# emolch/kiwi

Measured on AMD Instinct MI355X. Metric: trial-source misfit evals/s, higher is better.
Workload: dtype f32

## Files before the change

### kiwi_amd/csrc/kiwi_accum.hip

```cpp
#include "kiwi_accum_api.hpp"

#if KIWI_ARITH == 0
#define KIWI_ARITH_NS exact
#elif KIWI_ARITH == 1
#define KIWI_ARITH_NS fused
#else
#error "KIWI_ARITH: 0 (exact) or 1 (fused)"
#endif

namespace kiwi {
namespace KIWI_ARITH_NS {

#include "kiwi_accum.inc"

#define KIWI_COMMON_ARGS a.G, a.span, a.pitch, a.recs, a.cent_ofs, a.isrc0, a.nrec, a.recv, a.syn, a.syn_stride

#if KIWI_FAMILY == 1
void launch_direct(const AccumArgs &a, dim3 grid)
{
    if (a.ng == 10) hipLaunchKernelGGL(accumulate_kernel<10>, grid, dim3(256), 0, a.stream, KIWI_COMMON_ARGS, a.synrow);
    else            hipLaunchKernelGGL(accumulate_kernel<8>, grid, dim3(256), 0, a.stream, KIWI_COMMON_ARGS, a.synrow);
}
#endif

#if KIWI_FAMILY == 2
template <int NG, int T, bool COMPACT>
static void grouped_tc(const AccumArgs &a, dim3 grid, int ntiles, const int *runs, int pairsel, const int *mate, const int *mate4)
{
#define KIWI_G(FV, RV) hipLaunchKernelGGL((accumulate_grouped_kernel<NG, T, FV, RV, COMPACT>), grid, dim3(T), 0, a.stream, KIWI_COMMON_ARGS, ntiles, \
                                          a.tab, a.coefs, runs, a.fp, a.pairflag, pairsel, mate, mate4, a.synrow, a.fam_ofs, a.fam_list)
    if (a.fuse) { if (runs) KIWI_G(true, true); else KIWI_G(true, false); }
    else        { if (runs) KIWI_G(false, true); else KIWI_G(false, false); }
#undef KIWI_G
}
template <int NG, int T>
static void grouped_t(const AccumArgs &a, dim3 grid, int ntiles, const int *runs, int pairsel, const int *mate, const int *mate4)
{
    if (a.compact) grouped_tc<NG, T, true>(a, grid, ntiles, runs, pairsel, mate, mate4);
    else           grouped_tc<NG, T, false>(a, grid, ntiles, runs, pairsel, mate, mate4);
}
void launch_grouped(const AccumArgs &a, dim3 grid, int T, int ntiles, const int *runs, int pairsel, const int *mate, const int *mate4)
{
    if (a.ng == 10) {
        if (T == 64) grouped_t<10, 64>(a, grid, ntiles, runs, pairsel, mate, mate4);
        else if (T == 128) grouped_t<10, 128>(a, grid, ntiles, runs, pairsel, mate, mate4);
        else grouped_t<10, 256>(a, grid, ntiles, runs, pairsel, mate, mate4);
    } else {
        if (T == 64) grouped_t<8, 64>(a, grid, ntiles, runs, pairsel, mate, mate4);
        else if (T == 128) grouped_t<8, 128>(a, grid, ntiles, runs, pairsel, mate, mate4);
        else grouped_t<8, 256>(a, grid, ntiles, runs, pairsel, mate, mate4);
    }
}
#endif

#if KIWI_FAMILY == 3
template <int NG, int NS, bool COMPACT>
static void multi_t(const AccumArgs &a, dim3 grid, int ntiles, const int *mate, const int *wider)
{
    if (a.fuse) hipLaunchKernelGGL((accumulate_multi_kernel<NG, true, NS, COMPACT>), grid, dim3(256), 0, a.stream, KIWI_COMMON_ARGS, ntiles, a.tab, a.coefs, a.fp,
                                   a.pairflag, mate, wider);
    else        hipLaunchKernelGGL((accumulate_multi_kernel<NG, false, NS, COMPACT>), grid, dim3(256), 0, a.stream, KIWI_COMMON_ARGS, ntiles, a.tab, a.coefs, a.fp,
                                   a.pairflag, mate, wider);
}
template <int NG, int NS>
static void multi_c(const AccumArgs &a, dim3 grid, int ntiles, const int *mate, const int *wider)
{
    if (a.compact) multi_t<NG, NS, true>(a, grid, ntiles, mate, wider); else multi_t<NG, NS, false>(a, grid, ntiles, mate, wider);
}
void launch_multi(const AccumArgs &a, dim3 grid, int NS, int ntiles, const int *mate, const int *wider)
{
    if (a.ng == 10) { if (NS == 4) multi_c<10, 4>(a, grid, ntiles, mate, wider); else multi_c<10, 2>(a, grid, ntiles, mate, wider); }
    else            { if (NS == 4) multi_c<8, 4>(a, grid, ntiles, mate, wider); else multi_c<8, 2>(a, grid, ntiles, mate, wider); }
}
#endif

#if KIWI_FAMILY == 4
template <int NG, bool COMPACT>
static void cell_t(const AccumArgs &a, dim3 grid, int ntiles, bool per_wave)
{
#define KIWI_C(KERNEL) hipLaunchKernelGGL(KERNEL, grid, dim3(256), 0, a.stream, KIWI_COMMON_ARGS, ntiles, a.tab, a.coefs, a.fp, a.pairflag, a.synrow, \
                                          a.fam_ofs, a.fam_list)
    if (per_wave) { if (a.fuse) KIWI_C((accumulate_cellw_kernel<NG, true, COMPACT>)); else KIWI_C((accumulate_cellw_kernel<NG, false, COMPACT>)); }
    else          { if (a.fuse) KIWI_C((accumulate_cell_kernel<NG, 256, 2, 0, true, COMPACT>)); else KIWI_C((accumulate_cell_kernel<NG, 256, 2, 0, false, COMPACT>)); }
#undef KIWI_C
}
template <int NG>
static void cell_c(const AccumArgs &a, dim3 grid, int ntiles, bool per_wave)
{
    if (a.compact) cell_t<NG, true>(a, grid, ntiles, per_wave); else cell_t<NG, false>(a, grid, ntiles, per_wave);
}
void launch_cell(const AccumArgs &a, dim3 grid, int ntiles) { if (a.ng == 10) cell_c<10>(a, grid, ntiles, false); else cell_c<8>(a, grid, ntiles, false); }
void launch_cellw(const AccumArgs &a, dim3 grid, int ntiles) { if (a.ng == 10) cell_c<10>(a, grid, ntiles, true); else cell_c<8>(a, grid, ntiles, true); }
int cellw_range() { return kCellwRange; }
#endif

}
}
```

### kiwi_amd/csrc/kiwi_accum.inc

```


typedef float f4u __attribute__((ext_vector_type(4), aligned(4)));
typedef float f2u __attribute__((ext_vector_type(2), aligned(4)));

#if defined(KIWI_EXPLICIT_FMA)
#ifndef KIWI_CELLW_AHEAD
#define KIWI_CELLW_AHEAD 3
#endif
template <class V> __device__ __forceinline__ V kiwi_mad(V acc, float w, V v)
{
    V ws;
    for (int k = 0; k < (int)(sizeof(V) / sizeof(float)); k++) ws[k] = w;
    return __builtin_elementwise_fma(ws, v, acc);
}
template <class V> __device__ __forceinline__ V kiwi_madv(V acc, V w, V v) { return __builtin_elementwise_fma(w, v, acc); }
#else
template <class V> __device__ __forceinline__ V kiwi_mad(V acc, float w, V v) { return acc + w * v; }
template <class V> __device__ __forceinline__ V kiwi_madv(V acc, V w, V v) { return acc + w * v; }
#endif

typedef int v4i_t __attribute__((ext_vector_type(4)));
typedef int v2i_t __attribute__((ext_vector_type(2)));
__device__ __forceinline__ __amdgpu_buffer_rsrc_t gf_rsrc(const float *base)
{
// ... 195 lines not shown
    int q = kRowPad + l;
    q = min(max(q, 0), pitch - 4);
    return *(const f4u *)(rowp + q);
}


template <bool BLEND, bool FAST, int N>
__device__ __forceinline__ void build_batch(float *__restrict__ tile0, int lds_tile, const int (&igs)[N], int p, int jb,
                                            const float *__restrict__ G, int pitch, int ta, int tb, const GeoRec &g)
{
    const int j = jb + p;
    f4u v[N][BLEND ? 4 : 1];
#pragma unroll
    for (int q = 0; q < N; q++) {
#pragma unroll
        for (int k = 0; k < (BLEND ? 4 : 1); k++) {
            const int base = REC_I(ta, 4 * igs[q] + k);
            if constexpr (FAST) {
                v[q][k] = buf_load4(gf_rsrc(G), p, base + jb);
            } else {
                const int lo = REC_I(tb, 4 * igs[q] + k);
                const int idx = min(max(base + j, lo), lo + pitch - 4);
                v[q][k] = *(const f4u *)(G + (size_t)(unsigned)idx);
            }
        }
    }
#pragma unroll
    for (int q = 0; q < N; q++) {
        f4u b;
        if constexpr (BLEND) {
            b = g.w[0] * v[q][0];
            b = b + g.w[1] * v[q][1];
            b = b + g.w[2] * v[q][2];
            b = b + g.w[3] * v[q][3];
        } else {
            b = v[q][0];
        }
        *(float4 *)(tile0 + igs[q] * lds_tile + p) = make_float4(b.x, b.y, b.z, b.w);
    }
}

template <bool BLEND, bool FAST>
__device__ __forceinline__ void pair_issue(f4u (&v)[2][BLEND ? 4 : 1], int ig0, int p, int jb, const float *__restrict__ G,
                                           int pitch, int ta, int tb)
{
    const int j = jb + p;
#pragma unroll
    for (int q = 0; q < 2; q++) {
#pragma unroll
        for (int k = 0; k < (BLEND ? 4 : 1); k++) {
            const int base = REC_I(ta, 4 * (ig0 + q) + k);
            if constexpr (FAST) {
                v[q][k] = buf_load4(gf_rsrc(G), p, base + jb);
            } else {
                const int lo = REC_I(tb, 4 * (ig0 + q) + k);
                const int idx = min(max(base + j, lo), lo + pitch - 4);
                v[q][k] = *(const f4u *)(G + (size_t)(unsigned)idx);
            }
        }
    }
}

template <bool BLEND>
__device__ __forceinline__ void pair_finish(const f4u (&v)[2][BLEND ? 4 : 1], float *__restrict__ tile0, int lds_tile, int ig0, int p,
                                            const GeoRec &g)
{
#pragma unroll
    for (int q = 0; q < 2; q++) {
        f4u b;
        if constexpr (BLEND) {
            b = g.w[0] * v[q][0];
            b = b + g.w[1] * v[q][1];
            b = b + g.w[2] * v[q][2];
            b = b + g.w[3] * v[q][3];
        } else {
            b = v[q][0];
        }
        *(float4 *)(tile0 + (ig0 + q) * lds_tile + p) = make_float4(b.x, b.y, b.z, b.w);
    }
}

struct HaloRegs { f4u v[4]; };

template <bool BLEND, bool FAST>
__device__ __forceinline__ HaloRegs halo_issue(bool active, int ig, int ph, int jb, const float *__restrict__ G, int pitch,
                                               int ta, int tb)
{
    HaloRegs h;
#pragma unroll
    for (int k = 0; k < (BLEND ? 4 : 1); k++) {
        const int base = __shfl(ta, 4 * ig + k, 64);
        int idx = base + jb + ph;
        if constexpr (!FAST) {
            const int lo = __shfl(tb, 4 * ig + k, 64);
            idx = min(max(idx, lo), lo + pitch - 4);
        }
        h.v[k] = f4u{ 0.f, 0.f, 0.f, 0.f };
        if (active) h.v[k] = *(const f4u *)(G + (size_t)(unsigned)idx);
    }
    return h;
}

template <bool BLEND>
__device__ __forceinline__ void halo_finish(bool active, const HaloRegs &h, float *__restrict__ tile0, int lds_tile, int ig, int ph,
                                            const GeoRec &g)
{
    f4u b;
    if constexpr (BLEND) {
        b = g.w[0] * h.v[0];
        b = kiwi_mad(b, g.w[1], h.v[1]);
        b = kiwi_mad(b, g.w[2], h.v[2]);
        b = kiwi_mad(b, g.w[3], h.v[3]);
    } else {
        b = h.v[0];
    }
    if (active) *(float4 *)(tile0 + ig * lds_tile + ph) = make_float4(b.x, b.y, b.z, b.w);
}

struct HaloRegs2 { f2u v[4]; };

template <bool FAST>
__device__ __forceinline__ HaloRegs2 halo_issue2(bool active, int ig, int ph, int jb, const float *__restrict__ G, int pitch, int ta, int tb)
{
    HaloRegs2 h;
#pragma unroll
    for (int k = 0; k < 4; k++) {
        const int base = __shfl(ta, 4 * ig + k, 64);
        int idx = base + jb + ph;
        if constexpr (!FAST) {
            const int lo = __shfl(tb, 4 * ig + k, 64);
            idx = min(max(idx, lo), lo + pitch - 2);
        }
        h.v[k] = f2u{ 0.f, 0.f };
        if (active) h.v[k] = *(const f2u *)(G + (size_t)(unsigned)idx);
    }
    return h;
}

__device__ __forceinline__ void halo_finish2(bool active, const HaloRegs2 &h, float *__restrict__ tile0, int lds_tile, int ig, int ph,
                                             float w0, float w1, float w2, float w3)
{
    f2u b = w0 * h.v[0];
    b = kiwi_mad(b, w1, h.v[1]);
    b = kiwi_mad(b, w2, h.v[2]);
    b = kiwi_mad(b, w3, h.v[3]);
    if (active) *(float2 *)(tile0 + ig * lds_tile + ph) = make_float2(b.x, b.y);
}

typedef float f2v __attribute__((ext_vector_type(2)));
typedef const __attribute__((address_space(3))) float *lds_cfp;

template <int NP = 2> struct TileRegsN { f2v lo[NP], hi[NP]; };
typedef TileRegsN<2> TileRegs;

struct TileBase { const __attribute__((address_space(3))) float *lo, *hi; };

__device__ __forceinline__ TileBase tile_base(const float *__restrict__ p)
{
    typedef const __attribute__((address_space(3))) float *lds_fp;
    TileBase b;
    b.lo = (lds_fp)p;
    unsigned a = (unsigned)(size_t)(b.lo + 1);
    asm volatile("" : "+v"(a));
    b.hi = (lds_fp)(size_t)a;
    return b;
}

template <int NP = 2>
__device__ __forceinline__ TileRegsN<NP> tile_load(const TileBase &b, int ofs)
{
    TileRegsN<NP> t;
#pragma unroll
    for (int h = 0; h < NP; h++) {
        t.lo[h] = f2v{ b.lo[ofs + 128 * h], b.lo[ofs + 128 * h + 64] };
        t.hi[h] = f2v{ b.hi[ofs + 128 * h], b.hi[ofs + 128 * h + 64] };
    }
    return t;
}

template <bool TAIL, int NP = 2>
__device__ __forceinline__ void tile_fma(f2v (&out)[NP], const TileRegsN<NP> &t, int jl, int jend, float factor, float wl, float wr)
{
#pragma unroll
// ... 657 lines not shown
            } else {
            int eprev = 0;
            bool have = false;
#define KIWI_C2STEP(LL, HH, RV, CC) do { \
                const int e = smax - __builtin_amdgcn_readlane(ishv, (CC) - c);       \
                const int d = have ? eprev - e : 0x7fff; \
                 \
                const int dh = same ? (d == 0 ? 1 : 0x7fff) : d, dl = same ? (d == 0 ? -1 : 0x7fff) : d; \
                same = false; \
                carry2_apply<NG, RV>(ar1, ar2, dz, LL, HH, abase + 4u * (unsigned)e, dh, dl, coef_grp + (size_t)((CC) - c) * kCoefLine, gcl, gsl); \
                have = true; eprev = e; } while (0)
#define KIWI_C2SOURCES(RV) do { \
                set2_dead(X); set2_dead(Y);        \
                for (int js = s; js < s_end; js++) { \
                    if (multi) { \
                        ar1[0] = ar1[1] = ar2[0] = ar2[1] = dz[0] = dz[1] = f2v{ 0.f, 0.f }; \
                        if (synrow && synrow[js] != js) continue;        \
                    } \
                    const size_t crow = ((size_t)(cent_ofs[isrc0 + js] - cb) * nrec + (size_t)r * nc + c) * kCoefLine; \
                    const unsigned clo = __builtin_amdgcn_readfirstlane((unsigned)crow), chi = __builtin_amdgcn_readfirstlane((unsigned)(crow >> 32)); \
                    const float *__restrict__ coef_grp = coefs + (((size_t)chi << 32) | clo); \
                    int cc = c; \
                     \
                    bool same = RUNS && multi && have && ((cend - c) & 1); \
                    for (; cc + 1 < cend; cc += 2) { KIWI_C2STEP(X, Y, RV, cc); KIWI_C2STEP(Y, X, RV, cc + 1); } \
                    if (cc < cend) KIWI_C2STEP(X, Y, RV, cc); \
                    if (multi) store_family(js); \
                } } while (0)
            if (g0.flags & 2) KIWI_C2SOURCES(true); else KIWI_C2SOURCES(false);
#undef KIWI_C2SOURCES
#undef KIWI_C2STEP
            cur = cur_next;
            }
        } else
        for (int js = s; js < s_end; js++) {
        const GeoRec *__restrict__ rcj = multi ? recs + ((size_t)(cent_ofs[isrc0 + js] - cb) * nrec + (size_t)r * nc) : rc;
        int cur_next_src = 0;
        if (multi) {
            if (js + 1 < s_end) {
                int lane_o = lane;
                if constexpr (RUNS && FUSE) asm volatile("" : "+v"(lane_o));
                cur_next_src = rec_load(recs + ((size_t)(cent_ofs[isrc0 + js + 1] - cb) * nrec + (size_t)r * nc), c, nc, lane_o);
            }
            ar1[0] = ar1[1] = ar2[0] = ar2[1] = dz[0] = dz[1] = f2v{ 0.f, 0.f };
            if (synrow && synrow[js] != js) { cur = cur_next_src; continue; }
        }
        const size_t crow = ((size_t)(cent_ofs[isrc0 + js] - cb) * nrec + (size_t)r * nc + c) * kCoefLine;
        const unsigned clo = __builtin_amdgcn_readfirstlane((unsigned)crow), chi = __builtin_amdgcn_readfirstlane((unsigned)(crow >> 32));
        const float *__restrict__ coef_grp = coefs + (((size_t)chi << 32) | clo);
        for (int cc = c; cc < cend; cc++) {
            const int nxt = rec_load(rcj, cc + 1, nc, lane);
            constexpr int ro = 0;
            const int ishift = REC_I(cur, ro + 8);
            const float cl = REC_F(cur, ro + 16), sl = REC_F(cur, ro + 17);
            const int flags = REC_I(cur, ro + 18);
            const float *__restrict__ coef = coef_grp + (size_t)(cc - c) * kCoefLine;
            const int e = smax - ishift;
            const int u0 = 4 * (tid & ~63) + lane;
            const TileBase chunk0 = tile_base(&tiles[0][e + u0]);
            const int jl = jb + e + u0;
            const bool tail = (jb + e + TILE) > jend_min;
#define APPLY(TV) do { \
                if (need_h && has_d && !(flags & 8)) centroid_apply_hd<NG, LDS_TILE, TV, !(FUSE && RUNS)>(ar1, ar2, dz, chunk0, jl, jend, flags, coef, cur, sd, cl, sl); \
                else centroid_apply<NG, LDS_TILE, TV>(ar1, ar2, dz, chunk0, jl, jend, need_h, has_d, flags, \
                                                      REC_F(cur, 9), sd, REC_F(cur, 10), REC_F(cur, 11), REC_F(cur, 12), REC_F(cur, 13), \
                                                      REC_F(cur, 14), REC_F(cur, 15), cl, sl); } while (0)
            if (!tail) APPLY(false); else APPLY(true);
#undef APPLY
            cur = nxt;
        }
        if (multi) { store_family(js); cur = cur_next_src; }
        }
        stored = multi;
        c = cend;
    }
    if (!multi) store_family(s);
    else if (!stored) {
        ar1[0] = ar1[1] = ar2[0] = ar2[1] = dz[0] = dz[1] = f2v{ 0.f, 0.f };
        for (int js = s; js < s_end; js++)
            if (!(synrow && synrow[js] != js)) store_family(js);
    }
}

template <bool BLEND, bool FAST>
__device__ __forceinline__ void one_issue(f4u (&v)[BLEND ? 4 : 1], int ig, int p, int jb, const float *__restrict__ G,
                                          int pitch, int ta, int tb)
{
    const int j = jb + p;
#pragma unroll
    for (int k = 0; k < (BLEND ? 4 : 1); k++) {
        const int base = REC_I(ta, 4 * ig + k);
        if constexpr (FAST) {
            v[k] = buf_load4(gf_rsrc(G), p, base + jb);
        } else {
            const int lo = REC_I(tb, 4 * ig + k);
            const int idx = min(max(base + j, lo), lo + pitch - 4);
            v[k] = *(const f4u *)(G + (size_t)(unsigned)idx);
        }
    }
}

__device__ __forceinline__ void one_issue_hidden(f4u (&v)[4], int ig, int p, int jb, const float *__restrict__ G, int ta)
{
    const size_t gi = (size_t)G;
    const v4i_t rs = { (int)(unsigned)gi, (int)((unsigned)(gi >> 32) & 0xffffu), -1, 0x00020000 };
    const int voff = (int)(4u * (unsigned)p);
#pragma unroll
    for (int k = 0; k < 4; k++) {
        const int soff = (int)(4u * (unsigned)(REC_I(ta, 4 * ig + k) + jb));
        asm volatile("buffer_load_dwordx4 %0, %1, %2, %3 offen" : "=v"(v[k]) : "v"(voff), "s"(rs), "s"(soff));
    }
}
template <int CNT_FULL, int CNT_SHORT>
__device__ __forceinline__ void vm_wait(f4u (&v)[4], int full )
{
    if constexpr (CNT_FULL == CNT_SHORT)
        asm volatile("s_waitcnt vmcnt(%4)" : "+v"(v[0]), "+v"(v[1]), "+v"(v[2]), "+v"(v[3]) : "n"(CNT_FULL));
    else
        asm volatile("s_cmp_eq_u32 %6, 0\n\ts_cbranch_scc1 1f\n\ts_waitcnt vmcnt(%4)\n\ts_branch 2f\n1:\n\ts_waitcnt vmcnt(%5)\n2:"
                     : "+v"(v[0]), "+v"(v[1]), "+v"(v[2]), "+v"(v[3]) : "n"(CNT_FULL), "n"(CNT_SHORT), "s"(full) : "scc");
}

template <bool BLEND>
__device__ __forceinline__ void one_finish(const f4u (&v)[BLEND ? 4 : 1], float *__restrict__ tile0, int lds_tile, int ig, int p,
                                           const GeoRec &g)
{
    f4u b;
    if constexpr (BLEND) {
        b = g.w[0] * v[0];
        b = b + g.w[1] * v[1];
        b = b + g.w[2] * v[2];
        b = b + g.w[3] * v[3];
    } else {
        b = v[0];
    }
    *(float4 *)(tile0 + ig * lds_tile + p) = make_float4(b.x, b.y, b.z, b.w);
}

#ifndef KIWI_MFMA_BLEND
#define KIWI_MFMA_BLEND 0
#endif
typedef float f4m __attribute__((ext_vector_type(4)));
struct RowsDw { float r[4][4]; };

__device__ __forceinline__ void rows_issue_dw(RowsDw &v, int ig, int lane, int jb, const float *__restrict__ G, int ta)
{
    const size_t gi = (size_t)G;
    const v4i_t rs = { (int)(unsigned)gi, (int)((unsigned)(gi >> 32) & 0xffffu), -1, 0x00020000 };
    const int voff = (int)(4u * (unsigned)lane);
#pragma unroll
    for (int k = 0; k < 4; k++) {
        const int soff = (int)(4u * (unsigned)(REC_I(ta, 4 * ig + k) + jb));
        asm volatile("buffer_load_dword %0, %1, %2, %3 offen" : "=v"(v.r[k][0]) : "v"(voff), "s"(rs), "s"(soff));
        asm volatile("buffer_load_dword %0, %1, %2, %3 offen offset:256" : "=v"(v.r[k][1]) : "v"(voff), "s"(rs), "s"(soff));
        asm volatile("buffer_load_dword %0, %1, %2, %3 offen offset:512" : "=v"(v.r[k][2]) : "v"(voff), "s"(rs), "s"(soff));
        asm volatile("buffer_load_dword %0, %1, %2, %3 offen offset:768" : "=v"(v.r[k][3]) : "v"(voff), "s"(rs), "s"(soff));
    }
}
template <int CNT_FULL, int CNT_SHORT>
__device__ __forceinline__ void vm_wait16(RowsDw &v, int full )
{
#define KIWI_R16 "+v"(v.r[0][0]), "+v"(v.r[0][1]), "+v"(v.r[0][2]), "+v"(v.r[0][3]), "+v"(v.r[1][0]), "+v"(v.r[1][1]), "+v"(v.r[1][2]), "+v"(v.r[1][3]), \
                 "+v"(v.r[2][0]), "+v"(v.r[2][1]), "+v"(v.r[2][2]), "+v"(v.r[2][3]), "+v"(v.r[3][0]), "+v"(v.r[3][1]), "+v"(v.r[3][2]), "+v"(v.r[3][3])
    if constexpr (CNT_FULL == CNT_SHORT)
        asm volatile("s_waitcnt vmcnt(%16)" : KIWI_R16 : "n"(CNT_FULL));
    else
        asm volatile("s_cmp_eq_u32 %18, 0\n\ts_cbranch_scc1 1f\n\ts_waitcnt vmcnt(%16)\n\ts_branch 2f\n1:\n\ts_waitcnt vmcnt(%17)\n2:"
                     : KIWI_R16 : "n"(CNT_FULL), "n"(CNT_SHORT), "s"(full) : "scc");
#undef KIWI_R16
}
__device__ __forceinline__ void mfma_finish(const RowsDw &v, float *__restrict__ dst, const float (&w)[4], bool write)
{
    const f4m negz = { -0.f, -0.f, -0.f, -0.f };
#pragma unroll
    for (int m = 0; m < 4; m++) {
        f4m b = __builtin_amdgcn_mfma_f32_4x4x1f32(v.r[0][m], w[0], negz, 0, 0, 0);
        b = b + __builtin_amdgcn_mfma_f32_4x4x1f32(v.r[1][m], w[1], negz, 0, 0, 0);
        b = b + __builtin_amdgcn_mfma_f32_4x4x1f32(v.r[2][m], w[2], negz, 0, 0, 0);
        b = b + __builtin_amdgcn_mfma_f32_4x4x1f32(v.r[3][m], w[3], negz, 0, 0, 0);
        if (write) *(float4 *)(dst + 64 * m) = make_float4(b.x, b.y, b.z, b.w);
    }
}

template <int NG, int NS> __host__ __device__ constexpr int multi_set_stride() { return NG * (1024 / NS + kHalo) + ((NS == 4 && KIWI_MFMA_BLEND) ? 8 : 0); }

template <int NG, bool FAST, int NS, typename Shadow>
__device__ __forceinline__ void multi_build(float *__restrict__ tile0, int wv, int lane, int tid, int jb, const float *__restrict__ G,
                                            int pitch, int ta, int tb, const GeoRec (&gw)[NS], int only, bool hact, bool whalo, int hig, int hph,
                                            Shadow shadow)
{
    constexpr int TILE = 1024 / NS, LDS_TILE = TILE + kHalo, DEPTH = 3, SET = multi_set_stride<NG, NS>();
    constexpr int N = (NS == 2) ? NG / 2 : (NG + 3) / 4;
    const int p = (NS == 2) ? 4 * (64 * (wv & 1) + lane) : 4 * lane;
    auto comp = [&](int i) { return (NS == 2) ? 2 * i + (wv >> 1) : wv + 4 * i; };
    HaloRegs hv;
    if (whalo) hv = halo_issue<true, FAST>(true, hig, hph, jb, G, pitch, ta, tb);
    const bool last_ok = comp(N - 1) < NG;
    if constexpr (KIWI_MFMA_BLEND && FAST && NS == 4 && KIWI_ARITH == 0) {
        RowsDw v[N];
#pragma unroll
        for (int i = 0; i < DEPTH && i < N; i++) if (i < N - 1 || last_ok) rows_issue_dw(v[i], comp(i), lane, jb, G, ta);
        __syncthreads();
        shadow();
        const int me = lane & 3;
        float w[4];
#pragma unroll
        for (int k = 0; k < 4; k++) w[k] = me == 0 ? gw[0].w[k] : (me == 1 ? gw[1].w[k] : (me == 2 ? gw[2].w[k] : gw[3].w[k]));
        float *__restrict__ dst = tile0 + me * SET + 4 * (lane >> 2);
        const bool write = only < 0 || only == me;
#pragma unroll
        for (int i = 0; i < N; i++) {
            __builtin_amdgcn_sched_barrier(0);
            if (i < N - 1 || last_ok) {
                const int behind = (i + DEPTH < N ? i + DEPTH : N) - 1 - i;
                const bool short_ = behind > 0 && i + DEPTH >= N;
                const int lastf = __builtin_amdgcn_readfirstlane(last_ok ? 1 : 0);
                switch (behind) {
                case 0: vm_wait16<0, 0>(v[i], 1); break;
                case 1: if (short_) vm_wait16<16, 0>(v[i], lastf); else vm_wait16<16, 16>(v[i], 1); break;
                default: if (short_) vm_wait16<32, 16>(v[i], lastf); else vm_wait16<32, 32>(v[i], 1); break;
                }
                mfma_finish(v[i], dst + comp(i) * LDS_TILE, w, write);
            }
            if (i + DEPTH < N && (i + DEPTH < N - 1 || last_ok)) rows_issue_dw(v[i + DEPTH], comp(i + DEPTH), lane, jb, G, ta);
        }
        if (whalo) {
#pragma unroll
            for (int s = 0; s < NS; s++)
                if (only < 0 || only == s) halo_finish<true>(hact, hv, tile0 + s * SET, LDS_TILE, hig, hph, gw[s]);
        }
        return;
    }
    f4u v[N][4];
    auto issue = [&](int i) __attribute__((always_inline)) {
        if constexpr (FAST) one_issue_hidden(v[i], comp(i), p, jb, G, ta);
        else one_issue<true, false>(v[i], comp(i), p, jb, G, pitch, ta, tb);
    };
#pragma unroll
    for (int i = 0; i < DEPTH && i < N; i++) if (i < N - 1 || last_ok) issue(i);
    __syncthreads();
    shadow();
#pragma unroll
    for (int i = 0; i < N; i++) {
        __builtin_amdgcn_sched_barrier(0);
        if (i < N - 1 || last_ok) {
            if constexpr (FAST) {
                const int behind = (i + DEPTH < N ? i + DEPTH : N) - 1 - i;
                const bool short_ = behind > 0 && i + DEPTH >= N;
                const int lastf = __builtin_amdgcn_readfirstlane(last_ok ? 1 : 0);
                switch (behind) {
                case 0: vm_wait<0, 0>(v[i], 1); break;
                case 1: if (short_) vm_wait<4, 0>(v[i], lastf); else vm_wait<4, 4>(v[i], 1); break;
                default: if (short_) vm_wait<8, 4>(v[i], lastf); else vm_wait<8, 8>(v[i], 1); break;
                }
            }
#pragma unroll
            for (int s = 0; s < NS; s++)
                if (only < 0 || only == s) one_finish<true>(v[i], tile0 + s * SET, LDS_TILE, comp(i), p, gw[s]);
        }
        if (i + DEPTH < N && (i + DEPTH < N - 1 || last_ok)) issue(i + DEPTH);
    }
    if (whalo) {
#pragma unroll
        for (int s = 0; s < NS; s++)
            if (only < 0 || only == s) halo_finish<true>(hact, hv, tile0 + s * SET, LDS_TILE, hig, hph, gw[s]);
    }
}


__device__ __forceinline__ int smax_u(int a, int b) { int r; asm("s_max_i32 %0, %1, %2" : "=s"(r) : "s"(a), "s"(b) : "scc"); return r; }
__device__ __forceinline__ int smin_u(int a, int b) { int r; asm("s_min_i32 %0, %1, %2" : "=s"(r) : "s"(a), "s"(b) : "scc"); return r; }

template <int NS>
__device__ __forceinline__ bool multi_taken(const RecvDev &rv, const int *__restrict__ pairflag, const int *__restrict__ mate,
                                            int s, int nrec, int r)
{
    if (!mate) return false;
    const int a = s - s % NS;
    if (!mate[a / NS] || !rv.need_h || !rv.has_d) return false;
    int f = 0;
#pragma unroll
    for (int i = 0; i < NS; i++) f |= pairflag[(size_t)(a + i) * nrec + r];
    return f == 0;
}

template <int NG, bool FUSE, int NS, bool COMPACT >
__global__ __launch_bounds__(256) __attribute__((amdgpu_waves_per_eu(3))) void accumulate_multi_kernel(
    const float *__restrict__ G, const int2 *__restrict__ span, int pitch,
    const GeoRec *__restrict__ recs, const int *__restrict__ cent_ofs, int isrc0, int nrec,
    const RecvDev *__restrict__ recv, float *__restrict__ syn, size_t syn_stride, int ntiles,
    const int *__restrict__ tab, const float *__restrict__ coefs, FuseParams fp, const int *__restrict__ pairflag, const int *__restrict__ mate,
    const int *__restrict__ mate_wider )
{
    constexpr bool compact = COMPACT;
    static_assert(NS == 2 || NS == 4, "sources per workgroup");
    constexpr int TILE = 1024 / NS, LDS_TILE = TILE + kHalo, K = LDS_TILE / 64, WPS = 4 / NS;
    constexpr int SET = multi_set_stride<NG, NS>();
    __shared__ __attribute__((aligned(16))) float tiles[NS * SET];
    const int s0 = NS * (int)blockIdx.x;
    const int tile = blockIdx.y % ntiles, r = blockIdx.y / ntiles;
    const RecvDev &rv = recv[r];
    if (!rv.enabled) return;
    if (tile * TILE >= rv.wlen) return;
    if (!multi_taken<NS>(rv, pairflag, mate, s0, nrec, r)) return;
    if constexpr (NS == 2) { if (multi_taken<4>(rv, pairflag, mate_wider, s0, nrec, r)) return; }
    const int tid = threadIdx.x;
    const int lane = tid & 63;
    const int wv = __builtin_amdgcn_readfirstlane(tid >> 6);
    const int sh = wv / WPS;
    const int t_tile0 = rv.wbeg + tile * TILE;
    const int cb = cent_ofs[isrc0];
    const int nc = cent_ofs[isrc0 + s0 + 1] - cent_ofs[isrc0 + s0];
    const size_t base_me = (size_t)(cent_ofs[isrc0 + s0 + sh] - cb) * nrec + (size_t)r * nc;
    const GeoRec *__restrict__ rc = recs + base_me;
    const float sd = rv.sd;
    (void)sd;
    const int u0 = 256 * (wv % WPS) + lane;

    f2v ar1[2] = { { 0.f, 0.f }, { 0.f, 0.f } }, ar2[2] = { { 0.f, 0.f }, { 0.f, 0.f } }, dz[2] = { { 0.f, 0.f }, { 0.f, 0.f } };
    f2v xa0, xa1, xa2, xa3, xa4, xa5, xa6, xa7, xa8, xa9, xb0, xb1, xb2, xb3, xb4, xb5, xb6, xb7, xb8, xb9;
    f2v ya0, ya1, ya2, ya3, ya4, ya5, ya6, ya7, ya8, ya9, yb0, yb1, yb2, yb3, yb4, yb5, yb6, yb7, yb8, yb9;
    typedef typename Set2Sel<NG>::type SetT;
    const SetT X = make_set2<NG>(xa0, xa1, xa2, xa3, xa4, xa5, xa6, xa7, xa8, xa9, xb0, xb1, xb2, xb3, xb4, xb5, xb6, xb7, xb8, xb9);
    const SetT Y = make_set2<NG>(ya0, ya1, ya2, ya3, ya4, ya5, ya6, ya7, ya8, ya9, yb0, yb1, yb2, yb3, yb4, yb5, yb6, yb7, yb8, yb9);

    long long rbase[NS];
#pragma unroll
    for (int i = 0; i < NS; i++) {
        const long long b = (long long)(cent_ofs[isrc0 + s0 + i] - cb) * nrec + (long long)r * nc;
        rbase[i] = ((long long)__builtin_amdgcn_readfirstlane((int)(b >> 32)) << 32) | (unsigned)__builtin_amdgcn_readfirstlane((int)b);
    }
    auto recs_of = [&](int i) { return recs + (size_t)rbase[i]; };
    auto tab_of = [&](int i) { return tab + (size_t)rbase[i] * (compact ? 4 : 128); };
    int c = 0;
    int cur[NS];
#pragma unroll
    for (int i = 0; i < NS; i++) cur[i] = rec_load(recs_of(i), 0, nc, lane);
    int ta = 0, tb = 0;
    if constexpr (compact) ta = off4_load(tab_of(0), 0, lane);
    else { ta = tab_of(0)[lane]; tb = tab_of(0)[64 + lane]; }
    const int hq = 255 - tid, hch = min(hq / NG, 15), hig = hq % NG, hph = TILE + 4 * hch;
    while (c < nc) {
        GeoRec g[NS];
        int smaxs[NS], smins[NS], npos = 0;
        bool shared = true, same_rows = true;
        if constexpr (compact) desc_expand(ta, cur[0], lane, pitch, ta, tb);
#pragma unroll
        for (int i = 0; i < NS; i++) {
            g[i].ishift = REC_I(cur[i], 8);
            g[i].pad = REC_I(cur[i], 19);
            smaxs[i] = g[i].ishift + ((g[i].pad >> 8) & 0xff);
            smins[i] = g[i].ishift - ((g[i].pad >> 16) & 0xff);
            npos = max(npos, TILE + (smaxs[i] - smins[i]) + 8);
            if (i == 0) g[0].row[0] = REC_I(cur[0], 0);
            else {
                same_rows = same_rows && (__builtin_amdgcn_ballot_w64(cur[i] != cur[0]) & 0xfull) == 0ull;
                shared = shared && smaxs[i] == smaxs[0];
            }
        }
        shared = shared && same_rows;
        if (same_rows && !shared) {
            int smax_c = smaxs[0], smin_c = smins[0];
#pragma unroll
            for (int i = 1; i < NS; i++) { smax_c = smax_u(smax_c, smaxs[i]); smin_c = smin_u(smin_c, smins[i]); }
            if (TILE + (smax_c - smin_c) + 8 <= LDS_TILE) {
                shared = true;
                npos = TILE + (smax_c - smin_c) + 8;
#pragma unroll
                for (int i = 0; i < NS; i++) smaxs[i] = smax_c;
            }
        }
        const int glen = g[0].pad & 0xff;
        const int cend = c + glen;
        int smax = smaxs[0];
#pragma unroll
        for (int i = 1; i < NS; i++) if (sh == i) smax = smaxs[i];
        int flags = 0, ishv = 0, warm_ = 0;
        float gcl = 0.f, gsl = 0.f;
        const float *__restrict__ coef_grp = nullptr;
        auto shadow = [&]() {
#pragma unroll
            for (int i = 0; i < NS; i++) { g[i].w[0] = REC_F(cur[i], 4); g[i].w[1] = REC_F(cur[i], 5); g[i].w[2] = REC_F(cur[i], 6); g[i].w[3] = REC_F(cur[i], 7); }
            int curme = cur[0];
#pragma unroll
            for (int i = 1; i < NS; i++) if (sh == i) curme = cur[i];
            flags = REC_I(curme, 18);
            gcl = REC_F(curme, 16); gsl = REC_F(curme, 17);
            if (lane < glen) ishv = rc[c + lane].ishift;
            const size_t crow = (base_me + c) * kCoefLine;
            const unsigned clo = __builtin_amdgcn_readfirstlane((unsigned)crow), chi = __builtin_amdgcn_readfirstlane((unsigned)(crow >> 32));
            coef_grp = coefs + (((size_t)chi << 32) | clo);
            if constexpr (NG == 10) warm_ = coef_warm(coef_grp);
        };
        auto noshadow = []() {};
#define KIWI_MULTI_BUILD(TA, TB, I0, ONLY, NPOS, SHADOW) do { \
            const int jb_ = t_tile0 - smaxs[I0] - 1;       \
            const float *__restrict__ Gg = G + (size_t)g[I0].row[0] * (size_t)pitch; \
            const bool lane_ok = lane >= 4 * NG || ((TA) + jb_ >= (TB) && (TA) + jb_ + LDS_TILE <= (TB) + pitch); \
            const bool fast = __builtin_amdgcn_ballot_w64(lane_ok) == ~0ull; \
            const bool hact = hq < 16 * NG && hph < (NPOS); \
            const bool whalo = __builtin_amdgcn_ballot_w64(hact) != 0ull; \
            if (fast) multi_build<NG, true, NS>(&tiles[0], wv, lane, tid, jb_, Gg, pitch, TA, TB, g, ONLY, hact, whalo, hig, hph, SHADOW); \
            else      multi_build<NG, false, NS>(&tiles[0], wv, lane, tid, jb_, Gg, pitch, TA, TB, g, ONLY, hact, whalo, hig, hph, SHADOW); } while (0)
        __builtin_amdgcn_s_setprio(1);
        if (shared) KIWI_MULTI_BUILD(ta, tb, 0, -1, npos, shadow);
        else {
            KIWI_MULTI_BUILD(ta, tb, 0, 0, npos, shadow);
#pragma unroll
            for (int i = 1; i < NS; i++) {
                int tai, tbi;
                if constexpr (compact) desc_expand(off4_load(tab_of(i), c, lane), cur[i], lane, pitch, tai, tbi);
                else { tai = tab_of(i)[(size_t)c * 128 + lane]; tbi = tab_of(i)[(size_t)c * 128 + 64 + lane]; }
                g[i].row[0] = REC_I(cur[i], 0);
                KIWI_MULTI_BUILD(tai, tbi, i, i, npos, noshadow);
            }
        }
#undef KIWI_MULTI_BUILD
#pragma unroll
        for (int i = 0; i < NS; i++) cur[i] = rec_load(recs_of(i), cend, nc, lane);
        if (cend < nc) {
            if constexpr (compact) ta = off4_load(tab_of(0), cend, lane);
            else { ta = tab_of(0)[(size_t)cend * 128 + lane]; tb = tab_of(0)[(size_t)cend * 128 + 64 + lane]; }
        }
        __syncthreads();
        __builtin_amdgcn_s_setprio(0);
        {
            const unsigned abase = (unsigned)(size_t)(lds_cfp)&tiles[sh * SET + u0];
            if constexpr (NG == 10 || NG == 8) {
                asm volatile("" :: "s"(warm_));
                const float gcl_u = __int_as_float(__builtin_amdgcn_readfirstlane(__float_as_int(gcl))), gsl_u = __int_as_float(__builtin_amdgcn_readfirstlane(__float_as_int(gsl)));
                const size_t cg_ = (size_t)coef_grp;
                const float *__restrict__ coef_u = (const float *)(((size_t)(unsigned)__builtin_amdgcn_readfirstlane((int)(cg_ >> 32)) << 32) | (unsigned)__builtin_amdgcn_readfirstlane((int)cg_));
                const int n = cend - c;
#define KIWI_ASM_ARGS ar1[0], ar1[1], ar2[0], ar2[1], dz[0], dz[1], abase, ishv, smax, n, coef_u, gcl_u, gsl_u
                if constexpr (NG == 10) {
                    if (flags & 2) { if constexpr (K == 5) KIWI_APPLY_ASM(10, 5, rot)(KIWI_ASM_ARGS); else KIWI_APPLY_ASM(10, 9, rot)(KIWI_ASM_ARGS); }
                    else           { if constexpr (K == 5) KIWI_APPLY_ASM(10, 5, plain)(KIWI_ASM_ARGS); else KIWI_APPLY_ASM(10, 9, plain)(KIWI_ASM_ARGS); }
                } else {
                    if (flags & 2) { if constexpr (K == 5) KIWI_APPLY_ASM(8, 5, rot)(KIWI_ASM_ARGS); else KIWI_APPLY_ASM(8, 9, rot)(KIWI_ASM_ARGS); }
                    else           { if constexpr (K == 5) KIWI_APPLY_ASM(8, 5, plain)(KIWI_ASM_ARGS); else KIWI_APPLY_ASM(8, 9, plain)(KIWI_ASM_ARGS); }
                }
#undef KIWI_ASM_ARGS
            } else {
            int cc = c, eprev = 0;
            bool have = false;
#define KIWI_C2STEP(LL, HH, RV, CC) do { \
                const int e = smax - __builtin_amdgcn_readlane(ishv, (CC) - c);        \
                const int d = have ? eprev - e : 0x7fff; \
                carry2_apply<NG, RV, K>(ar1, ar2, dz, LL, HH, abase + 4u * (unsigned)e, d, d, coef_grp + (size_t)((CC) - c) * kCoefLine, gcl, gsl); \
                have = true; eprev = e; } while (0)
            if (flags & 2) {
                set2_dead(X); set2_dead(Y);
                for (; cc + 1 < cend; cc += 2) { KIWI_C2STEP(X, Y, true, cc); KIWI_C2STEP(Y, X, true, cc + 1); }
                if (cc < cend) KIWI_C2STEP(X, Y, true, cc);
            } else {
                set2_dead(X); set2_dead(Y);
                for (; cc + 1 < cend; cc += 2) { KIWI_C2STEP(X, Y, false, cc); KIWI_C2STEP(Y, X, false, cc + 1); }
                if (cc < cend) KIWI_C2STEP(X, Y, false, cc);
            }
#undef KIWI_C2STEP
            }
        }
        c = cend;
    }
    {
        const int js = s0 + sh;
        const int tl = tile * TILE + u0;
        if (!FUSE && tl >= rv.wlen) return;
        float *__restrict__ so = syn + (size_t)js * syn_stride + tl;
        float mom = 0.f;
        if constexpr (FUSE) mom = fp.moment[fp.isrc0 + js];
        const bool whole = tile * TILE + TILE <= rv.wlen;
        for (int k = 0; k < rv.ncomp; k++) {
            f2v o01, o23;
            out4(rv.comp[k], rv.sign[k], rv.cl0, rv.sl0, ar1, ar2, dz, o01, o23);
            if constexpr (!FUSE) {
                const float o[4] = { o01.x, o01.y, o23.x, o23.y };
#pragma unroll
                for (int i = 0; i < 4; i++)
                    if (tl + 64 * i < rv.wlen) so[rv.synofs[k] + 64 * i] = o[i];
                continue;
            }
            double acc = fused_acc4(fp, o01, o23, mom, fp.reft + rv.refofs[k] + tl, fp.tw + rv.refofs[k] + tl, tl, rv.wlen, whole);
            acc = wave_reduce_f64(acc, fp.method == 6);
            if (lane == 63)
                fp.partial[((size_t)js * fp.nmis + rv.slot0 + k) * fp.nparts + tile * WPS + (wv % WPS)] = acc;
        }
    }
}

template <int SPL> struct RawVec;
template <> struct RawVec<4> { typedef f4u type; };
template <> struct RawVec<2> { typedef f2u type; };

template <int NG, int PART> struct CellPart;
template <> struct CellPart<10, 0> { static constexpr int n = 10; static constexpr int first = 0; __device__ static constexpr int ig(int i) { return i < 3 ? i : (i == 3 ? 8 : (i < 9 ? i - 1 : 9)); } };
template <> struct CellPart<8, 0>  { static constexpr int n = 8; static constexpr int first = 0; __device__ static constexpr int ig(int i) { return i; } };
template <> struct CellPart<10, 1> { static constexpr int n = 6; static constexpr int first = 0; __device__ static constexpr int ig(int i) { return i < 3 ? i : (i == 3 ? 8 : i - 1); } };
template <> struct CellPart<10, 2> { static constexpr int n = 4; static constexpr int first = 6; __device__ static constexpr int ig(int i) { return i < 3 ? 5 + i : 9; } };
template <> struct CellPart<8, 1>  { static constexpr int n = 5; static constexpr int first = 0; __device__ static constexpr int ig(int i) { return i; } };
template <> struct CellPart<8, 2>  { static constexpr int n = 3; static constexpr int first = 5; __device__ static constexpr int ig(int i) { return 5 + i; } };

template <int NG, int PART, int SPL> using RawArr = typename RawVec<SPL>::type[CellPart<NG, PART>::n][4];

template <int NG, int PART, int SPL, bool FAST = false, bool UNI = false>
__device__ __forceinline__ void raw_issue(RawArr<NG, PART, SPL> &v, int p, int jb,
// ... 554 lines not shown
```

### kiwi_amd/csrc/kiwi_accum_api.hpp

```cpp
#pragma once
#include "kiwi_common.hpp"

namespace kiwi {

struct AccumArgs {
    hipStream_t stream;
    int ng;
    bool fuse;
    const float *G; const int2 *span; int pitch;
    const GeoRec *recs; const int *cent_ofs; int isrc0, nrec;
    const RecvDev *recv; float *syn; size_t syn_stride;
    const int *tab; const float *coefs; FuseParams fp;
    const int *pairflag, *synrow, *fam_ofs, *fam_list;
    int compact;
};

#define KIWI_ACCUM_LAUNCHERS                                                                                                      \
                                                                 \
    void launch_direct(const AccumArgs &a, dim3 grid);                                                                            \
                  \
    void launch_grouped(const AccumArgs &a, dim3 grid, int T, int ntiles, const int *runs, int pairsel, const int *mate,          \
                        const int *mate4);                                                                                        \
                                                     \
    void launch_multi(const AccumArgs &a, dim3 grid, int NS, int ntiles, const int *mate, const int *mate_wider);                \
        \
    void launch_cell(const AccumArgs &a, dim3 grid, int ntiles);                                                                  \
    void launch_cellw(const AccumArgs &a, dim3 grid, int ntiles);                                                                 \
                               \
    int cellw_range();

namespace exact { KIWI_ACCUM_LAUNCHERS }
namespace fused { KIWI_ACCUM_LAUNCHERS }
#undef KIWI_ACCUM_LAUNCHERS

}
```

### kiwi_amd/csrc/kiwi_bands.hpp

```cpp

namespace bands {

constexpr int kMaxBands = 16;
constexpr int kLg = 16;
constexpr int kMaxDynLds = 152 * 1024;

static inline bool is_spectral(int method) { return method == KIWI_AMPSPEC_L2NORM || method == KIWI_AMPSPEC_L1NORM; }

struct BandTab {
    int ntd, nfilt, nspec, nband;
    int td[kMaxBands], filt[kMaxBands], spec[kMaxBands];
    int method[kMaxBands], has_filter[kMaxBands];
};

struct BandArgs {
    SynRows sr;
    const float *reft;
    const int *ntr;
    FusedFftTables tabs;
    const BandTab *bt;
    const int2 *vtab;
    const float *normtab;
    const float *refamp, *filtw, *reffilt, *zmask;
    int nband, nmis, isrc0, dyn_bytes;
// ... 365 lines not shown
        else
            HIPCHECK(hipMemcpyAsync(st.reffilt_h.data() + f.pr.filtofs, st.reffilt_d.p + f.pr.filtofs, (size_t)cd.wlen * sizeof(float),
                                    hipMemcpyDeviceToHost, c->stream));
    }
    HIPCHECK(hipStreamSynchronize(c->stream));
    for (auto &f : fresh) {
        const CompDev &cd = c->comps[(size_t)f.pr.slot];
        const int method = c->bands[(size_t)f.b].method;
        double sum = 0.0, pk = 0.0;
        float nf;
        if (is_spectral(method)) {
            const int nb = f.pr.ntrans / 2 + 1;
            const float df = 1.f / ((float)f.pr.ntrans * dt);
            for (int k = 0; k < nb; k++) {
                const float v = st.refamp_h[(size_t)f.pr.specofs + k];
                sum += (method == KIWI_AMPSPEC_L2NORM) ? (double)v * (double)v : (double)std::fabs(v);
            }
            nf = (method == KIWI_AMPSPEC_L2NORM) ? 1.f * (float)std::sqrt((double)df * sum) : 1.f * (float)((double)df * sum);
        } else {
            for (int i = 0; i < cd.wlen; i++) {
                const float v = st.reffilt_h[(size_t)f.pr.filtofs + i];
                switch (method) {
                case KIWI_L2NORM: sum += (double)v * (double)v; break;
                case KIWI_L1NORM: sum += (double)std::fabs(v); break;
                case KIWI_SCALAR_PRODUCT: sum += (double)(v * v); break;
                default: pk = std::max(pk, (double)std::fabs(v)); break;
                }
            }
            switch (method) {
            case KIWI_L2NORM: nf = 1.f * (float)std::sqrt((double)dt * sum); break;
            case KIWI_L1NORM: nf = 1.f * (float)((double)dt * sum); break;
            case KIWI_SCALAR_PRODUCT: nf = (1.f * 1.f) * (float)sum; break;
            default: nf = 1.f * (float)pk; break;
            }
        }
        st.normtab_h[((size_t)f.b * nmis + f.pr.slot) * kLg + lg_of(f.pr.ntrans)] = nf;
    }
    HIPCHECK(hipMemcpyAsync(st.refamp_d.p, st.refamp_h.data(), st.refamp_h.size() * sizeof(float), hipMemcpyHostToDevice, c->stream));
    HIPCHECK(hipMemcpyAsync(st.reffilt_d.p, st.reffilt_h.data(), st.reffilt_h.size() * sizeof(float), hipMemcpyHostToDevice, c->stream));
    HIPCHECK(hipMemcpyAsync(st.vtab_d.p, st.vtab_h.data(), st.vtab_h.size() * sizeof(int2), hipMemcpyHostToDevice, c->stream));
    HIPCHECK(hipMemcpyAsync(st.normtab_d.p, st.normtab_h.data(), st.normtab_h.size() * sizeof(float), hipMemcpyHostToDevice, c->stream));
    HIPCHECK(hipStreamSynchronize(c->stream));
}

static void run(kiwi_hip_ctx *c, int isrc0, int nsrc, const Out &out)
{
    check_setup(c);
    if (isrc0 < 0 || nsrc < 0 || (long long)isrc0 + nsrc > (long long)c->nsrc)
        throw std::runtime_error("band_misfits: sources " + std::to_string(isrc0) + " .. " + std::to_string((long long)isrc0 + nsrc) +
                                 " are not inside the uploaded batch of " + std::to_string(c->nsrc));
    if (nsrc == 0) return;
    BandState &st = c->band_state;
    if (!st.valid || st.prepare_gen != c->prepare_gen) reset_cache(c);
    const int nrec = (int)c->recv.size(), nband = (int)c->bands.size(), nmis = c->nmis;
    if (st.need_spec && !c->fused_fft)
        throw std::runtime_error("band_misfits: bands with a frequency filter or an amplitude-spectrum method go through the in-LDS transforms, "
                                 "which KIWI_HIP_FUSED_FFT=0 switches off");
    int wlen_pow2 = 1 << kFusedFftMinLog2;
    while (wlen_pow2 < c->max_wlen) wlen_pow2 <<= 1;
    if (wlen_pow2 > (1 << kFusedFftMaxLog2))
        throw std::runtime_error("band_misfits: a misfit window of " + std::to_string(c->max_wlen) + " samples does not fit the in-LDS row of " +
                                 std::to_string(1 << kFusedFftMaxLog2) + " samples");
    c->misfit_d.ensure((size_t)c->nsrc * c->nmis, &c->dev_bytes);
    c->global_d.ensure((size_t)c->nsrc, &c->dev_bytes);
    if (c->fft_needed && !c->fft_ready) prepare_fft(c, c->reft_h);
    c->fuse_now = false;
    struct Restore { kiwi_hip_ctx *c; bool want; ~Restore() { c->want_spansrc = want; } } restore{ c, c->want_spansrc };
    c->want_spansrc = true;
    if (!st.attr) {
        HIPCHECK(hipFuncSetAttribute(reinterpret_cast<const void *>(&band_kernel), hipFuncAttributeMaxDynamicSharedMemorySize, kMaxDynLds));
        st.attr = true;
    }

    hipEvent_t ev[4];
    for (int i = 0; i < 4; i++) ev[i] = c->get_event();
    struct Return { kiwi_hip_ctx *c; hipEvent_t *ev; ~Return() { for (int i = 0; i < 4; i++) c->event_pool.push_back(ev[i]); } } ret{ c, ev };
    std::vector<int> ntr_h;
    int s = isrc0;
    while (s < isrc0 + nsrc) {
        size_t bytes = 0;
        int n = 0;
        while (s + n < isrc0 + nsrc) {
            const size_t nc = (size_t)(c->cent_ofs[s + n + 1] - c->cent_ofs[s + n]);
            const size_t add = nc * nrec * (sizeof(GeoRec) + (c->accum_mode == 0 ? 512 + kCoefLine * sizeof(float) : 0)) + c->syn_stride * sizeof(float) +
                               (size_t)nband * nmis * 2 * sizeof(float);
            if (n > 0 && (bytes + add > c->chunk_bytes_limit || n >= 65535)) break;
            if (c->fft_needed && n >= c->fft_cap) break;
            bytes += add; n++;
        }
        HIPCHECK(hipEventRecord(ev[0], c->stream));
        run_chunk(c, s, n, 0);
        HIPCHECK(hipEventRecord(ev[1], c->stream));
        const size_t np = (size_t)n * nmis;
        int longest = wlen_pow2;
        if (st.need_spec) {
            st.ntr_d.ensure(np, &c->dev_bytes);
            hipLaunchKernelGGL(fft_size_kernel, dim3((unsigned)((np + 255) / 256)), dim3(256), 0, c->stream, c->spansrc_d.p, c->comps_d.p, nmis, n, nrec,
                               c->risetime_d.p + s, c->gm.dt, st.ntr_d.p, (const int *)nullptr);
            ntr_h.resize(np);
            HIPCHECK(hipMemcpyAsync(ntr_h.data(), st.ntr_d.p, np * sizeof(int), hipMemcpyDeviceToHost, c->stream));
            HIPCHECK(hipStreamSynchronize(c->stream));
            std::vector<std::pair<int, int>> want;
            std::vector<int> seen((size_t)nmis, 0);
            longest = 0;
            for (size_t i = 0; i < np; i++) {
                const int m = (int)(i % (size_t)nmis), nt = ntr_h[i];
                if (nt < (1 << kFusedFftMinLog2) || nt > (1 << kFusedFftMaxLog2))
                    throw std::runtime_error("band_misfits: source " + std::to_string(s + (int)(i / (size_t)nmis) + 1) + ", misfit slot " + std::to_string(m + 1) +
                                             " needs a transform of " + std::to_string(nt) + " samples; the in-LDS transforms take " +
                                             std::to_string(1 << kFusedFftMinLog2) + " to " + std::to_string(1 << kFusedFftMaxLog2));
                longest = std::max(longest, nt);
                if (seen[(size_t)m] != nt) { seen[(size_t)m] = nt; want.emplace_back(m, nt); }
            }
            std::sort(want.begin(), want.end());
            want.erase(std::unique(want.begin(), want.end()), want.end());
            make_variants(c, want);
        }
        const size_t nout = (size_t)n * nband * nmis;
        st.mis_d.ensure(nout, &c->dev_bytes); st.norm_d.ensure(nout, &c->dev_bytes); st.glob_d.ensure((size_t)n * nband, &c->dev_bytes);
        const int dyn = st.nfilt >= 2 ? std::max(4 * longest, std::min(8 * longest, kMaxDynLds)) : 4 * longest;
        BandArgs a;
        a.sr = SynRows{ c->syn_d.p, c->syn_stride, c->comps_d.p, c->tw_d.p, c->moment_d.p, c->risetime_d.p, nullptr };
        a.reft = c->reft_d.p;
        a.ntr = st.need_spec ? st.ntr_d.p : nullptr;
        a.tabs = fused_fft_tables(c);
        a.bt = reinterpret_cast<const BandTab *>(st.bt_d.p);
        a.vtab = st.vtab_d.p; a.normtab = st.normtab_d.p;
        a.refamp = st.refamp_d.p; a.filtw = st.filtw_d.p; a.reffilt = st.reffilt_d.p; a.zmask = st.zmask_d.p;
        a.nband = nband; a.nmis = nmis; a.isrc0 = s; a.dyn_bytes = dyn;
        a.dt = c->gm.dt; a.syn_factor = c->syn_factor;
        a.mis_out = st.mis_d.p; a.norm_out = st.norm_d.p;
        hipLaunchKernelGGL(band_kernel, dim3((unsigned)n, (unsigned)nmis), dim3(256), (size_t)dyn, c->stream, a);
        hipLaunchKernelGGL(band_global_kernel, dim3((unsigned)(((size_t)n * nband + 127) / 128)), dim3(128), 0, c->stream, st.mis_d.p, st.norm_d.p,
                           c->recfirst_d.p, c->nrec_en, nmis, nband, s, n, st.glob_d.p, c->any_failed ? c->status_d.p : (const int *)nullptr);
        HIPCHECK(hipGetLastError());
        HIPCHECK(hipEventRecord(ev[2], c->stream));
        const Out o = out.at((size_t)(s - isrc0), (size_t)nband, (size_t)nmis);
        if (o.misfit) HIPCHECK(hipMemcpyAsync(o.misfit, st.mis_d.p, nout * sizeof(float), hipMemcpyDeviceToHost, c->stream));
        if (o.norm) HIPCHECK(hipMemcpyAsync(o.norm, st.norm_d.p, nout * sizeof(float), hipMemcpyDeviceToHost, c->stream));
        if (o.global) HIPCHECK(hipMemcpyAsync(o.global, st.glob_d.p, (size_t)n * nband * sizeof(float), hipMemcpyDeviceToHost, c->stream));
        HIPCHECK(hipEventRecord(ev[3], c->stream));
        HIPCHECK(hipStreamSynchronize(c->stream));
        for (int i = 0; i < 3; i++) {
            float t = 0.f;
            HIPCHECK(hipEventElapsedTime(&t, ev[i], ev[i + 1]));
            c->bands_ms[i] += t;
        }
        s += n;
    }
    c->last_isrc0 = isrc0; c->last_nsrc = nsrc; c->last_proc_which = 0;
    c->evaluated.resize((size_t)c->nsrc, 0);
    std::fill(c->evaluated.begin() + isrc0, c->evaluated.begin() + isrc0 + nsrc, 1);
}

}
```

### kiwi_amd/csrc/kiwi_common.hpp

```cpp
#pragma once
#include <hip/hip_runtime.h>
#include <type_traits>

namespace kiwi {

constexpr int kRowPad = 32;
constexpr int kTile = 1024;
constexpr int kMaxComp = 5;
constexpr int kHalo = 64;
constexpr int kMaxGroup = 64;

struct GeoRec {
    int   row[4];
    float w[4];
    int   ishift;
    float wfrac;
    float f[6];
    float cl, sl;
    int   flags;
    int   pad;
};
static_assert(sizeof(GeoRec) == 80, "GeoRec layout");

struct GfMeta {
    int nx, nz, ng;
    int pitch;
    float dt, dx, dz, firstx, firstz;
};

struct RecvDev {
    double azi0, bazi0, dist0;
    float depth;
    float cl0, sl0;
    int   enabled;
    int   ncomp;
    int   comp[kMaxComp];
    float sign[kMaxComp];
    int   need_h, has_d;
    float sd;
    int   wbeg, wlen;
    int   synofs[kMaxComp];
    int   slot0;
    int   refofs[kMaxComp];
};

struct FuseParams {
    const float *reft, *tw, *moment;
    double *partial;
    int method;
    float syn_factor;
    int nmis, nparts, isrc0;
};

struct CompDev {
    int synofs;
    int halo;
    int w0, wlen;
    int refofs;
    int rec;
    int has_filter;
    int ntrans_max;
    int fl_lo, fl_ns, refxofs;
    int untapered, rf0, rf1, vertical;
    int spankind;
};

struct FftPair {
    long long fft_ofs;
    long long spec_ofs;
    int ntrans;
    int specofs;
    int filtofs;
    int slot;
};
static_assert(sizeof(FftPair) == 32, "FftPair layout");

struct ShakeRec {
    int slot[3];
    int np;
    int untapered;
    int rec;
};

constexpr int kCoefLine = 20;
template <int NG> __host__ __device__ constexpr int coef_wl(int a) { return 2 * a; }
template <int NG> __host__ __device__ constexpr int coef_wr(int a) { return 2 * a + 1; }

constexpr int kSpanInts = 8;
__device__ __forceinline__ void strip_span(const int *__restrict__ sp, int kind, int &lo, int &hi)
{
    if (kind == 3) { lo = sp[4]; hi = sp[5]; return; }
    if (kind == 0) { lo = sp[0]; hi = sp[1]; return; }
    if (kind == 1) { lo = sp[2]; hi = sp[3]; return; }
    lo = min(sp[0], sp[2]); hi = max(sp[1], sp[3]);
}

struct EvalParams {
    int bilinear, xus, zus;
    int nrec;
    int isrc0;
    int cellmode;
    int nogaps;
};

__device__ __forceinline__ bool cell_pair(const RecvDev &rv, const int *__restrict__ pairflag, int s, int nrec, int r)
{
    return rv.need_h && rv.has_d && !(pairflag[(size_t)s * nrec + r] & 3);
}

template <int NS>
__device__ __forceinline__ bool multi_taken_fwd(const RecvDev &rv, const int *__restrict__ pairflag, const int *__restrict__ mate,
                                                int s, int nrec, int r)
{
    if (!mate) return false;
    const int a = s - s % NS;
    if (!mate[a / NS] || !rv.need_h || !rv.has_d) return false;
    int f = 0;
#pragma unroll
    for (int i = 0; i < NS; i++) f |= pairflag[(size_t)(a + i) * nrec + r];
    return f == 0;
}

__device__ __forceinline__ double sq_acc(double acc, float d) { return fma((double)d, (double)d, acc); }

template <int CTRL, int ROW_MASK>
__device__ __forceinline__ double dpp_f64(double v)
{
    const int lo = __builtin_amdgcn_update_dpp(0, __double2loint(v), CTRL, ROW_MASK, 0xf, true);
    const int hi = __builtin_amdgcn_update_dpp(0, __double2hiint(v), CTRL, ROW_MASK, 0xf, true);
    return __hiloint2double(hi, lo);
}

template <bool IS_MAX>
__device__ __forceinline__ double wave_reduce_f64_t(double v)
{
#define KIWI_STEP(CTRL, MASK) do { const double o = dpp_f64<CTRL, MASK>(v); v = IS_MAX ? fmax(v, o) : v + o; } while (0)
    KIWI_STEP(0x111, 0xf);
    KIWI_STEP(0x112, 0xf);
    KIWI_STEP(0x114, 0xf);
    KIWI_STEP(0x118, 0xf);
    KIWI_STEP(0x142, 0xa);
    KIWI_STEP(0x143, 0xc);
#undef KIWI_STEP
    return v;
}
__device__ __forceinline__ double wave_reduce_f64(double v, bool is_max)
{
    return is_max ? wave_reduce_f64_t<true>(v) : wave_reduce_f64_t<false>(v);
}

}
```

### kiwi_amd/csrc/kiwi_hip.hip

```cpp
#include "../../include/kiwi_hip.h"
#include "kiwi_host.hpp"
#include "kiwi_host_eikonal.hpp"
#include "kiwi_host_lm.hpp"
#include "kiwi_geometry.hpp"
#include "kiwi_misfit.hpp"
#include "kiwi_accum_api.hpp"
#include "kiwi_fmm_device.hpp"

#include <hip/hip_runtime.h>
#include <hipfft/hipfft.h>
#include <algorithm>
#include <array>
#include <map>
#include <tuple>
#include <cstdio>
#include <cstdlib>
#include <cstring>
#include <string>
#include <vector>
#include <stdexcept>
#include <omp.h>
#include <chrono>
#include <condition_variable>
#include <deque>
// ... 82 lines not shown
};

struct BandDef { int method; Plf filter; };

struct BandState {
    bool valid = false, need_spec = false, attr = false;
    unsigned prepare_gen = 0;
    int nfilt = 0;
    std::vector<float> refamp_h, filtw_h, reffilt_h, normtab_h;
    std::vector<int2> vtab_h;
    DevBuf<CompDev> comps_d;
    DevBuf<float> zmask_d, rows_d, refamp_d, filtw_d, reffilt_d, normtab_d, mis_d, norm_d, glob_d;
    DevBuf<int2> vtab_d;
    DevBuf<int> bt_d, ntr_d;
    DevBuf<FftPair> prs_d;
};

struct TimeScanState {
    bool attr = false;
    DevBuf<float> mis_d, norm_d, glob_d;
    DevBuf<int> best_d;
};

}

struct kiwi_hip_ctx {
    int device = 0;
    hipStream_t stream = nullptr;
    std::string err;
    long long dev_bytes = 0;

    GfMeta gm{};
    bool have_db = false;
    DevBuf<float> G;
    DevBuf<int2> span;
    DevBuf<unsigned char> endz;
    int db_lmax = 0;

    int bilinear = 0, xus = 1, zus = 1;
    float effective_dt = 1.f;
    GeoCoords src_origin; bool have_origin = false; double ref_time = 0;
    std::vector<Receiver> recv;
    int method = KIWI_L2NORM;
    float syn_factor = 1.f;
    bool have_crust = false;
    CrustProfile rupture_profile{}, origin_profile{};
    float crustal_thickness_limit = 0.f;
    std::vector<HalfSpace> constraints;

    bool prepared = false;
    bool synth_only = false;
    bool any_untapered = false;
    DevBuf<int> spansrc_d;
    bool want_spansrc = false;
    int nmis = 0, nrec_en = 0;
    int halo = 0;
    size_t syn_stride = 0;
    std::vector<CompDev> comps;
    std::vector<RecvDev> recv_h;
    std::vector<float> norm_h;
    std::vector<float> reft_h;
    DevBuf<RecvDev> recv_d;
    DevBuf<CompDev> comps_d;
    DevBuf<float> reft_d, tw_d, norm_d;
    DevBuf<int> recfirst_d;
    int max_wlen = 0;

    int nsrc = 0;
    std::vector<int> cent_ofs;
    float max_risetime = 0.f;
    DevBuf<float> cent_d, moment_d, risetime_d;
    DevBuf<int> centofs_d;
    std::vector<int> src_status;
    bool any_failed = false;
    DevBuf<int> status_d;
    std::vector<int> same_as;
    bool any_same = false;
    DevBuf<int> synrow_d, famofs_d, famlist_d;
    int dedupe_enabled = 1;
    std::vector<unsigned long long> geo_hash;
    std::vector<kiwi_hip_ctx *> mates;
    int cpu_share = 1;
    std::vector<unsigned long long> struct_hash;
    std::vector<unsigned char> group_lens;
    std::vector<int> first_shift;
    std::vector<float> src_ends;
    DevBuf<int> mate_d, mate4_d;
    int duo = 4;
    std::vector<char> single_group;
    DevBuf<int> runfirst_d;
    int share_runs = 1, max_run = 64;
    int fuse_enabled = 1;
    bool fuse_now = false;
    DevBuf<double> fusepart_d;

    DevBuf<float> misfit_d, global_d;
    DevBuf<GeoRec> recs_d;
    DevBuf<int> tab_d;
    DevBuf<int> off4_d;
    DevBuf<float> coef_d;
    DevBuf<int> pairflag_d;
    DevBuf<float> syn_d, proc_d;
    bool floating = false;
    int max_ns = 1;
    DevBuf<float> refx_d, vt_d, partial_d;
    DevBuf<int> fshift_d;
    int last_isrc0 = 0, last_nsrc = 0, last_chunk0 = 0, last_chunkn = 0;
    std::vector<char> evaluated;
    int last_proc_which = 0;
    int group_threads_env = 0;
    int group_threads = 128;
    int accum_mode = 0;
    int cell_mode = -1;
    int cell_wave = 1;
    int arith = KIWI_ARITH_EXACT;
    double points_per_centroid = 0.0;
    int keep_which = 0;
    int proc_chunk0 = 0, proc_chunkn = 0, proc_which_held = 0;
    size_t chunk_bytes_limit = (size_t)16 << 30;
    float outer_ms[3] = { 0.f, 0.f, 0.f };
    float linfit_wide_ms[2] = { 0.f, 0.f };
    float linfit_ms[4] = { 0.f, 0.f, 0.f, 0.f };
    std::vector<BandDef> bands;
    BandState band_state;
    float bands_ms[3] = { 0.f, 0.f, 0.f };
    TimeScanState timescan_state;
    float timescan_ms[3] = { 0.f, 0.f, 0.f };
    float linfit_timescan_ms[4] = { 0.f, 0.f, 0.f, 0.f };
    unsigned linfit_timescan_attr = 0;
    unsigned prepare_gen = 0;
    int eik_solver = 0;
    mutable FmmDev fmm;

    bool fft_needed = false, fft_ready = false, any_filter = false;
    int fft_cap = 0;
    size_t fft_floats_per_src = 0, spec_cplx_per_src = 0;
    struct FftVariant { int ntrans, specofs, filtofs; float norm; };
    std::map<std::pair<int, int>, FftVariant> variants;
    std::vector<float> refamp_h, filtw_h, reffilt_h;
    std::vector<int> slot_has_filter;
    DevBuf<int> spanbuf_d, ntr_d;
    DevBuf<float> fft_d, refamp_d, filtw_d, reffilt_d, zmask_d, normsrc_d;
    DevBuf<int> lmax_d;
    bool db_gaps = false;
    bool db_simple = false;
    int compact = 1;
    DevBuf<int> synspan_d;
    DevBuf<float> refpair_d, reffiltpair_d;
    bool untapered_fft = false;
    DevBuf<float2> spec_d;
    DevBuf<FftPair> pairs_d;
    int *ntr_pin = nullptr; size_t ntr_pin_n = 0;
    int *mate_pin = nullptr; size_t mate_pin_n = 0;
    hipEvent_t mate_event = nullptr;
    FftPair *pairs_pin = nullptr; size_t pairs_pin_n = 0;
    std::vector<FftPair> last_pairs;
    std::vector<float> norm_src_h;
    struct FftBucket { int ntrans; long long count, fft_base, spec_base; };
    std::vector<FftBucket> buckets;
    hipEvent_t size_event = nullptr;
    std::map<std::tuple<int, int, int>, hipfftHandle> plans;
    DevBuf<float2> fused_tab[kFusedFftMaxLog2 + 1];
    bool fused_fft = true;
    bool fused_fft_attr = false;

    std::vector<EventPair> events;
    std::vector<hipEvent_t> event_pool;

    hipEvent_t get_event()
    {
// ... 575 lines not shown
                case KIWI_SCALAR_PRODUCT: sum += (double)(a * a); break;
                default: pk = std::max(pk, (double)std::fabs(a)); break;
                }
            }
            switch (c->method) {
            case KIWI_L2NORM: nf = 1.f * (float)std::sqrt((double)dt * sum); break;
            case KIWI_L1NORM: nf = 1.f * (float)((double)dt * sum); break;
            case KIWI_SCALAR_PRODUCT: nf = (1.f * 1.f) * (float)sum; break;
            default: nf = 1.f * (float)pk; break;
            }
        }
        c->variants[std::make_pair(pr.slot, pr.ntrans)] = kiwi_hip_ctx::FftVariant{ pr.ntrans, pr.specofs, pr.filtofs, nf };
    }
}

void layout_fft_chunk(kiwi_hip_ctx *c, int isrc0, int nsrc)
{
    HIPCHECK(hipEventSynchronize(c->size_event));
    const size_t np = (size_t)nsrc * c->nmis;
    const int *ntr = c->ntr_pin;
    std::map<int, long long> count;
    std::vector<std::pair<int, int>> want;
    {
        std::vector<int> seen((size_t)c->nmis, 0);
        for (size_t i = 0; i < np; i++) {
            const int m = (int)(i % c->nmis);
            count[ntr[i]]++;
            if (seen[m] != ntr[i]) { seen[m] = ntr[i]; want.emplace_back(m, ntr[i]); }
        }
        std::sort(want.begin(), want.end());
        want.erase(std::unique(want.begin(), want.end()), want.end());
    }
    make_variants(c, want);
    c->buckets.clear();
    std::map<int, size_t> bucket_of;
    long long fb = 0, sbase = 0;
    for (auto &kv : count) {
        bucket_of[kv.first] = c->buckets.size();
        c->buckets.push_back({ kv.first, 0, fb, sbase });
        fb += kv.second * kv.first;
        sbase += kv.second * (kv.first / 2 + 1);
    }
    c->fft_d.ensure((size_t)fb, &c->dev_bytes);
    c->spec_d.ensure((size_t)sbase, &c->dev_bytes);
    if (c->untapered_fft) {
        c->refpair_d.ensure((size_t)sbase, &c->dev_bytes);
        c->reffiltpair_d.ensure((size_t)fb, &c->dev_bytes);
    }
    pin_ensure(c->pairs_pin, c->pairs_pin_n, np);
    c->norm_src_h.resize((size_t)c->nsrc * c->nmis, 0.f);
    int last_ntr = -1; size_t last_b = 0;
    for (size_t i = 0; i < np; i++) {
        const int m = (int)(i % c->nmis);
        if (ntr[i] != last_ntr) { last_ntr = ntr[i]; last_b = bucket_of[last_ntr]; }
        auto &b = c->buckets[last_b];
        const auto &v = c->variants[std::make_pair(m, ntr[i])];
        FftPair &pr = c->pairs_pin[i];
        pr.fft_ofs = b.fft_base + b.count * b.ntrans;
        pr.spec_ofs = b.spec_base + b.count * (b.ntrans / 2 + 1);
        pr.ntrans = b.ntrans; pr.specofs = v.specofs; pr.filtofs = v.filtofs; pr.slot = m;
        b.count++;
        c->norm_src_h[(size_t)isrc0 * c->nmis + i] = v.norm;
    }
    c->pairs_d.ensure(np, &c->dev_bytes);
    HIPCHECK(hipMemcpyAsync(c->pairs_d.p, c->pairs_pin, np * sizeof(FftPair), hipMemcpyHostToDevice, c->stream));
    HIPCHECK(hipMemcpyAsync(c->normsrc_d.p + (size_t)isrc0 * c->nmis, c->norm_src_h.data() + (size_t)isrc0 * c->nmis, np * sizeof(float),
                            hipMemcpyHostToDevice, c->stream));
    c->last_pairs.assign(c->pairs_pin, c->pairs_pin + np);
}

bool can_fuse(const kiwi_hip_ctx *c, int proc_which, int isrc0, int nsrc)
{
    (void)isrc0; (void)nsrc;
    return c->fuse_enabled && c->accum_mode == 0 && proc_which == 0 && !c->fft_needed && !c->floating && !c->synth_only && !c->any_untapered &&
           c->halo == 0 && (c->method == KIWI_L2NORM || c->method == KIWI_L1NORM || c->method == KIWI_SCALAR_PRODUCT || c->method == KIWI_PEAK);
}

static int kiwi_quad_shift_span()
{
    static const int v = [] { const char *m = std::getenv("KIWI_HIP_QUAD_SPAN"); return m ? std::atoi(m) : 16; }();
    return v;
}

void run_chunk(kiwi_hip_ctx *c, int isrc0, int nsrc, int proc_which)
{
    const int nrec = (int)c->recv.size();
    const int cbeg = c->cent_ofs[isrc0], cend = c->cent_ofs[isrc0 + nsrc];
    int maxnc = 0;
    for (int s = isrc0; s < isrc0 + nsrc; s++) maxnc = std::max(maxnc, c->cent_ofs[s + 1] - c->cent_ofs[s]);
    c->recs_d.ensure((size_t)(cend - cbeg) * nrec, &c->dev_bytes);
    int *tab = nullptr;
    int *off4 = nullptr;
    if (c->accum_mode == 0) {
        c->tab_d.ensure((size_t)(cend - cbeg) * nrec * 128, &c->dev_bytes); tab = c->tab_d.p;
        if (c->db_simple && c->compact) {
            c->off4_d.ensure((size_t)(cend - cbeg) * nrec * 4, &c->dev_bytes); off4 = c->off4_d.p;
            if (std::getenv("KIWI_HIP_POISON")) HIPCHECK(hipMemsetAsync(off4, 0x7f, (size_t)(cend - cbeg) * nrec * 4 * sizeof(int), c->stream));
        }
        if (std::getenv("KIWI_HIP_POISON")) HIPCHECK(hipMemsetAsync(tab, 0x7f, (size_t)(cend - cbeg) * nrec * 128 * sizeof(int), c->stream));
        c->coef_d.ensure((size_t)(cend - cbeg) * nrec * kCoefLine + 160, &c->dev_bytes);
    }
    const int *synrow = nullptr, *famofs = nullptr, *famlist = nullptr;
    const bool heavy = c->dedupe_enabled == 2 || (size_t)(cend - cbeg) >= (size_t)8 * (size_t)nsrc;
    if (c->dedupe_enabled && heavy && c->any_same && !c->fft_needed && !c->floating && !c->any_untapered && !c->want_spansrc && !c->synth_only &&
        proc_which == 0) {
        std::vector<int> sr((size_t)nsrc);
        int ndup = 0;
        for (int s = 0; s < nsrc; s++) {
            const int f = c->same_as[(size_t)isrc0 + s];
            sr[s] = (f >= isrc0 && f != isrc0 + s) ? f - isrc0 : s;
            ndup += sr[s] != s;
        }
        const bool any = c->dedupe_enabled == 2 ? ndup > 0 : 2 * ndup >= nsrc;
        if (any) {
            c->synrow_d.ensure((size_t)nsrc, &c->dev_bytes);
            HIPCHECK(hipMemcpyAsync(c->synrow_d.p, sr.data(), (size_t)nsrc * sizeof(int), hipMemcpyHostToDevice, c->stream));
            synrow = c->synrow_d.p;
            if (c->fuse_now) {
                std::vector<int> ofs((size_t)nsrc + 1, 0), lst;
                for (int s = 0; s < nsrc; s++) if (sr[s] != s) ofs[(size_t)sr[s] + 1]++;
                for (int s = 0; s < nsrc; s++) ofs[(size_t)s + 1] += ofs[s];
                lst.resize((size_t)ofs[nsrc]);
                std::vector<int> fill(ofs.begin(), ofs.end() - 1);
                for (int s = 0; s < nsrc; s++) if (sr[s] != s) lst[(size_t)fill[sr[s]]++] = s;
                c->famofs_d.ensure(ofs.size(), &c->dev_bytes);
                c->famlist_d.ensure(std::max<size_t>(lst.size(), 1), &c->dev_bytes);
                HIPCHECK(hipMemcpyAsync(c->famofs_d.p, ofs.data(), ofs.size() * sizeof(int), hipMemcpyHostToDevice, c->stream));
                HIPCHECK(hipMemcpyAsync(c->famlist_d.p, lst.data(), lst.size() * sizeof(int), hipMemcpyHostToDevice, c->stream));
                HIPCHECK(hipStreamSynchronize(c->stream));
                famofs = c->famofs_d.p; famlist = c->famlist_d.p;
            }
            HIPCHECK(hipStreamSynchronize(c->stream));
        }
    }
    const bool fuse = c->fuse_now;
    if (!fuse) c->syn_d.ensure((size_t)nsrc * c->syn_stride, &c->dev_bytes);
    float *proc = nullptr;
    if (proc_which) { c->proc_d.ensure((size_t)nsrc * c->syn_stride, &c->dev_bytes); proc = c->proc_d.p; }

    const bool cell = c->accum_mode == 0 && (c->cell_mode == 1 || (c->cell_mode < 0 && c->bilinear && c->points_per_centroid > 0.5));
    const bool duo_maybe = c->accum_mode == 0 && c->duo && !cell && c->max_wlen >= 128 && !c->group_threads_env && nsrc >= 2;
    EvalParams ep{ c->bilinear, c->xus, c->zus, nrec, isrc0, cell ? 1 : 0, c->db_gaps ? 0 : 1 };
    int *spansrc = nullptr;
    if (c->any_untapered || c->want_spansrc || c->fft_needed) {
        const size_t n = (size_t)nsrc * nrec;
        c->spansrc_d.ensure(n * kSpanInts, &c->dev_bytes);
        hipLaunchKernelGGL(span_init_kernel, dim3((unsigned)((2 * n + 255) / 256)), dim3(256), 0, c->stream, c->spansrc_d.p, 2 * n);
        spansrc = c->spansrc_d.p;
    }
    hipEvent_t e0, e1, e2, e3;
    record(c, 0, e0);
    if (maxnc > 0) {
        dim3 grid((unsigned)((maxnc * nrec + 255) / 256), (unsigned)nsrc);
        if (cell || duo_maybe) {
            c->pairflag_d.ensure((size_t)nsrc * nrec, &c->dev_bytes);
            HIPCHECK(hipMemsetAsync(c->pairflag_d.p, 0, (size_t)nsrc * nrec * sizeof(int), c->stream));
        }
        int *lmax = nullptr;
        if (c->db_gaps && spansrc) {
            c->lmax_d.ensure((size_t)nsrc * nrec, &c->dev_bytes);
            HIPCHECK(hipMemsetAsync(c->lmax_d.p, 0xff, (size_t)nsrc * nrec * sizeof(int), c->stream));
            lmax = c->lmax_d.p;
            hipLaunchKernelGGL(geometry_kernel, grid, dim3(256), 0, c->stream, c->cent_d.p, c->centofs_d.p, ep, c->gm,
                               c->span.p, c->recv_d.p, (GeoRec *)nullptr, (int *)nullptr, (float *)nullptr, (int *)nullptr, (int *)nullptr, (int *)nullptr, c->endz.p, (const int *)nullptr,
                               lmax, (const int *)nullptr, (int4 *)nullptr);
        }
        hipLaunchKernelGGL(geometry_kernel, grid, dim3(256), 0, c->stream, c->cent_d.p, c->centofs_d.p, ep, c->gm,
                           c->span.p, c->recv_d.p, c->recs_d.p, tab, c->coef_d.p, (int *)nullptr, spansrc, (cell || duo_maybe) ? c->pairflag_d.p : (int *)nullptr, c->endz.p, (const int *)nullptr,
                           (int *)nullptr, (const int *)lmax, (int4 *)off4);
        if (cell)
            hipLaunchKernelGGL(cellgroup_kernel, grid, dim3(256), 0, c->stream, c->centofs_d.p, ep, c->gm, c->span.p, c->recv_d.p,
                               c->recs_d.p, tab, c->coef_d.p, c->pairflag_d.p, c->endz.p, (const int *)nullptr,
                               c->cell_wave ? exact::cellw_range() : kHalo - 10, off4 ? 1 : 0);
    }
    if (c->fft_needed && !c->untapered_fft) {
        const size_t np = (size_t)nsrc * c->nmis;
        c->ntr_d.ensure(np, &c->dev_bytes);
        pin_ensure(c->ntr_pin, c->ntr_pin_n, np);
        hipLaunchKernelGGL(fft_size_kernel, dim3((unsigned)((np + 255) / 256)), dim3(256), 0, c->stream, spansrc, c->comps_d.p, c->nmis,
                           nsrc, nrec, c->risetime_d.p + isrc0, c->gm.dt, c->ntr_d.p, (const int *)nullptr);
        HIPCHECK(hipMemcpyAsync(c->ntr_pin, c->ntr_d.p, np * sizeof(int), hipMemcpyDeviceToHost, c->stream));
        HIPCHECK(hipEventRecord(c->size_event, c->stream));
    }
    record(c, 0, e1);
    int fuse_T = 0, fuse_tile = 0, fuse_ntiles = 0, fuse_nparts = 0;
    bool fuse_all = false;
    {
        dim3 grid((unsigned)((c->max_wlen + kTile - 1) / kTile), (unsigned)nrec, (unsigned)nsrc);
        const bool fusedar = c->arith == KIWI_ARITH_FUSED;
        AccumArgs aa{ c->stream, c->gm.ng, c->fuse_now, c->G.p, c->span.p, c->gm.pitch, c->recs_d.p, c->centofs_d.p, isrc0, nrec, c->recv_d.p,
                      c->syn_d.p, c->syn_stride, off4 ? off4 : c->tab_d.p, c->coef_d.p, FuseParams{ nullptr, nullptr, nullptr, nullptr, 0, 1.f, 0, 0, 0 },
                      nullptr, synrow, famofs, famlist, off4 ? 1 : 0 };
        if (c->accum_mode == 1) {
            if (fusedar) fused::launch_direct(aa, grid); else exact::launch_direct(aa, grid);
        } else {
            const int T = c->group_threads_env ? c->group_threads : (c->max_wlen >= 2048 ? 256 : (c->max_wlen >= 384 ? 128 : 64));
            const int ntiles = (c->max_wlen + 4 * T - 1) / (4 * T);
            const int ntiles_p = (c->max_wlen + 511) / 512;
            const int spl = 2, Tc = 256;
            const int ntiles_c = (c->max_wlen + spl * Tc - 1) / (spl * Tc);
            int *runs = nullptr;
            unsigned gx = (unsigned)nsrc;
            if (c->share_runs && !cell && (!synrow || fuse)) {
                std::vector<int> rf;
                const int cap = std::max(1, std::min(c->max_run, (nsrc * ntiles * nrec) / 8192));
                int s = 0;
                while (s < nsrc) {
                    int e = s + 1;
                    const int g = isrc0 + s;
                    if (c->single_group[g])
                        while (e < nsrc && e - s < cap && c->single_group[isrc0 + e] && c->geo_hash[isrc0 + e] == c->geo_hash[g] &&
                               c->cent_ofs[isrc0 + e + 1] - c->cent_ofs[isrc0 + e] == c->cent_ofs[g + 1] - c->cent_ofs[g]) e++;
                    rf.push_back(s);
                    s = e;
                }
                if ((int)rf.size() < nsrc) {
                    rf.push_back(nsrc);
                    c->runfirst_d.ensure(rf.size(), &c->dev_bytes);
                    HIPCHECK(hipMemcpyAsync(c->runfirst_d.p, rf.data(), rf.size() * sizeof(int), hipMemcpyHostToDevice, c->stream));
                    HIPCHECK(hipStreamSynchronize(c->stream));
                    runs = c->runfirst_d.p;
                    gx = (unsigned)rf.size() - 1;
                }
            }
            bool duo = duo_maybe && !runs && !synrow && maxnc > 0;
            bool any4 = false, any2 = false;
            if (duo) {
                const size_t n4 = (size_t)(nsrc + 3) / 4, n2 = (size_t)(nsrc + 1) / 2;
                pin_ensure(c->mate_pin, c->mate_pin_n, n4 + n2);
                if (!c->mate_event) HIPCHECK(hipEventCreateWithFlags(&c->mate_event, hipEventDisableTiming));
                else HIPCHECK(hipEventSynchronize(c->mate_event));
                int *m4 = c->mate_pin, *m2 = c->mate_pin + n4;
                std::fill(m4, m4 + n4 + n2, 0);
                const float near_h = 0.25f * c->gm.dx * (float)c->xus, near_z = 0.25f * c->gm.dz * (float)c->zus;
                auto same = [&](int a, int b, bool shifts) {
                    const int na = c->cent_ofs[a + 1] - c->cent_ofs[a], nb = c->cent_ofs[b + 1] - c->cent_ofs[b];
                    if (!(na > 0 && na == nb && c->struct_hash[a] == c->struct_hash[b] && (!shifts || std::abs(c->first_shift[a] - c->first_shift[b]) <= kiwi_quad_shift_span()))) return false;
                    if (std::memcmp(c->group_lens.data() + c->cent_ofs[a], c->group_lens.data() + c->cent_ofs[b], (size_t)na) != 0) return false;
                    const float *p = c->src_ends.data() + (size_t)a * 6, *q = c->src_ends.data() + (size_t)b * 6;
                    for (int k = 0; k < 6; k++)
                        if (std::fabs(p[k] - q[k]) > (k % 3 == 2 ? near_z : near_h)) return false;
                    return true;
                };
                if (c->duo >= 4)
                    for (int k = 0; 4 * k + 3 < nsrc; k++) {
                        const int a = isrc0 + 4 * k;
                        m4[k] = (same(a, a + 1, true) && same(a, a + 2, true) && same(a, a + 3, true)) ? 1 : 0;
                        any4 = any4 || m4[k];
                    }
                for (int k = 0; c->max_wlen > 256 && 2 * k + 1 < nsrc; k++) {
                    const int a = isrc0 + 2 * k;
                    m2[k] = (!m4[(size_t)k / 2] && same(a, a + 1, false)) ? 1 : 0;
                    any2 = any2 || m2[k];
                }
                duo = any4 || any2;
                if (std::getenv("KIWI_HIP_DEBUG")) {
                    int c4 = 0, c2 = 0; for (size_t i = 0; i < n4; i++) c4 += m4[i]; for (size_t i = 0; i < n2; i++) c2 += m2[i];
                    std::fprintf(stderr, "[kiwi_hip] chunk of %d sources: %d groups of four, %d pairs of equal structure\n", nsrc, c4, c2);
                }
                if (duo) {
                    c->mate4_d.ensure(n4, &c->dev_bytes);
                    c->mate_d.ensure(n2, &c->dev_bytes);
                    HIPCHECK(hipMemcpyAsync(c->mate4_d.p, m4, n4 * sizeof(int), hipMemcpyHostToDevice, c->stream));
                    HIPCHECK(hipMemcpyAsync(c->mate_d.p, m2, n2 * sizeof(int), hipMemcpyHostToDevice, c->stream));
                    HIPCHECK(hipEventRecord(c->mate_event, c->stream));
                }
            }
            const int ntiles_q = (c->max_wlen + 255) / 256;
            dim3 ggrid(gx, (unsigned)(ntiles * nrec));
            dim3 dgrid((unsigned)((nsrc + 1) / 2), (unsigned)(ntiles_p * nrec)), qgrid((unsigned)((nsrc + 3) / 4), (unsigned)(ntiles_q * nrec));
            dim3 cgrid((unsigned)nsrc, (unsigned)(ntiles_c * nrec));
            if (fuse) {
                const int nparts = cell ? std::max(ntiles * (T / 64), ntiles_c * (Tc / 64)) : (duo ? std::max({ ntiles * (T / 64), ntiles_p * 2, ntiles_q }) : ntiles * (T / 64));
                c->fusepart_d.ensure((size_t)nsrc * c->nmis * nparts, &c->dev_bytes);
                if (cell || duo) HIPCHECK(hipMemsetAsync(c->fusepart_d.p, 0, (size_t)nsrc * c->nmis * nparts * sizeof(double), c->stream));
                aa.fp = FuseParams{ c->reft_d.p, c->tw_d.p, c->moment_d.p, c->fusepart_d.p, c->method, c->syn_factor, c->nmis, nparts, isrc0 };
                fuse_nparts = nparts;
            }
            fuse_T = T; fuse_tile = 4 * T; fuse_ntiles = ntiles; fuse_all = cell || duo;
            aa.pairflag = (cell || duo) ? c->pairflag_d.p : (const int *)nullptr;
            if (cell) {
                static const bool cell_fused = [] { const char *e = std::getenv("KIWI_HIP_CELL_FUSED"); return !e || std::atoi(e) != 0; }();
                if (c->cell_wave) { if (fusedar && cell_fused) fused::launch_cellw(aa, cgrid, ntiles_c); else exact::launch_cellw(aa, cgrid, ntiles_c); }
                else exact::launch_cell(aa, cgrid, ntiles_c);
            }
            const int *m2p = any2 ? c->mate_d.p : (const int *)nullptr, *m4p = any4 ? c->mate4_d.p : (const int *)nullptr;
            if (any4) { if (fusedar) fused::launch_multi(aa, qgrid, 4, ntiles_q, m4p, nullptr); else exact::launch_multi(aa, qgrid, 4, ntiles_q, m4p, nullptr); }
            if (any2) { if (fusedar) fused::launch_multi(aa, dgrid, 2, ntiles_p, m2p, m4p); else exact::launch_multi(aa, dgrid, 2, ntiles_p, m2p, m4p); }
            const int pairsel = cell ? 1 : (duo ? 3 : 0);
            if (fusedar) fused::launch_grouped(aa, ggrid, T, ntiles, runs, pairsel, m2p, m4p);
            else         exact::launch_grouped(aa, ggrid, T, ntiles, runs, pairsel, m2p, m4p);
        }
    }
    record(c, 1, e2);
    if (c->any_untapered) {
        c->synspan_d.ensure((size_t)nsrc * c->nmis * 2, &c->dev_bytes);
        hipLaunchKernelGGL(synspan_kernel, dim3((unsigned)c->nmis, (unsigned)nsrc), dim3(256), 0, c->stream, c->syn_d.p, c->syn_stride, c->comps_d.p,
                           c->risetime_d.p + isrc0, c->gm.dt, c->nmis, spansrc, nrec, synrow, c->synspan_d.p);
    }
    if (c->untapered_fft) {
        const size_t np = (size_t)nsrc * c->nmis;
        c->ntr_d.ensure(np, &c->dev_bytes);
        pin_ensure(c->ntr_pin, c->ntr_pin_n, np);
        hipLaunchKernelGGL(fft_size_kernel, dim3((unsigned)((np + 255) / 256)), dim3(256), 0, c->stream, spansrc, c->comps_d.p, c->nmis,
                           nsrc, nrec, c->risetime_d.p + isrc0, c->gm.dt, c->ntr_d.p, (const int *)c->synspan_d.p);
        HIPCHECK(hipMemcpyAsync(c->ntr_pin, c->ntr_d.p, np * sizeof(int), hipMemcpyDeviceToHost, c->stream));
        HIPCHECK(hipEventRecord(c->size_event, c->stream));
    }
    if (c->fft_needed) layout_fft_chunk(c, isrc0, nsrc);
    {
        const bool spectral = (c->method == KIWI_AMPSPEC_L2NORM || c->method == KIWI_AMPSPEC_L1NORM);
        const int fl_method = c->method == KIWI_FLOATING_L2NORM ? KIWI_L2NORM : KIWI_L1NORM;
        const int td_method = spectral ? KIWI_L2NORM : (c->floating ? fl_method : c->method);
        const int fft_mode = !c->fft_needed ? 0 : (spectral ? 3 : 1);
        MisfitParams mp{ td_method, c->gm.dt, c->syn_factor, c->nmis, isrc0, proc_which == 3 ? 2 : proc_which, fft_mode, nsrc,
                         c->floating ? 1 : 0 };
        if (c->floating) {
            c->vt_d.ensure((size_t)nsrc * c->syn_stride, &c->dev_bytes);
            c->partial_d.ensure((size_t)nsrc * c->nmis * c->max_ns, &c->dev_bytes);
            c->fshift_d.ensure((size_t)c->nsrc * c->nrec_en, &c->dev_bytes);
        }
        if (fuse) {
            const int nth = nsrc * c->nmis;
            hipLaunchKernelGGL(misfit_finish_kernel, dim3((unsigned)((nth + 255) / 256)), dim3(256), 0, c->stream,
                               c->fusepart_d.p, c->comps_d.p, c->nmis, fuse_all ? fuse_nparts : fuse_ntiles * (fuse_T / 64), fuse_T / 64,
                               fuse_all ? 0 : fuse_tile,
                               c->method, c->gm.dt, isrc0, nsrc, c->misfit_d.p);
        }
        int lds_lo = 1, lds_hi = 0;
        if (c->fft_needed) lds_fft_range(c, lds_lo, lds_hi);
        const bool direct_ok = !proc && !fuse;
        if (!spectral && !direct_ok) { lds_lo = 1; lds_hi = 0; }
        bool any_lds = false, any_lib = false;
        int lds_longest = 0;
        if (c->fft_needed)
            for (auto &b : c->buckets) { if (b.ntrans >= lds_lo && b.ntrans <= lds_hi) { any_lds = true; lds_longest = std::max(lds_longest, b.ntrans); } else any_lib = true; }
        const bool spec_direct_all = spectral && c->fft_needed && direct_ok && !any_lib;
        if (c->fft_needed && direct_ok) { mp.fft_mode |= 4; mp.lds_lo = lds_lo; mp.lds_hi = lds_hi; }
        SpecParams sp{ c->method, c->gm.dt, c->syn_factor, c->nmis, isrc0, c->any_filter ? 1 : 0 };
        sp.lds_lo = lds_lo; sp.lds_hi = lds_hi;
        if (c->untapered_fft) {
            sp.refpair = c->refpair_d.p; sp.reffiltpair = c->reffiltpair_d.p;
            const dim3 pg((unsigned)c->nmis, (unsigned)nsrc);
            hipLaunchKernelGGL(untapered_rows_kernel<true>, pg, dim3(256), 0, c->stream, c->syn_d.p, c->syn_stride, c->comps_d.p, c->reft_d.p,
                               c->moment_d.p, c->risetime_d.p, isrc0, c->gm.dt, c->nmis, spansrc, nrec, c->synspan_d.p, c->pairs_d.p, c->fft_d.p);
            fft_buckets(c, true);
            if (spectral) {
                hipLaunchKernelGGL(pair_refamp_kernel, pg, dim3(256), 0, c->stream, c->spec_d.p, c->pairs_d.p, c->comps_d.p, c->filtw_d.p, sp,
                                   c->refpair_d.p, c->normsrc_d.p);
            } else {
                hipLaunchKernelGGL(spec_filter_kernel, dim3((unsigned)(c->nmis * nsrc)), dim3(256), 0, c->stream,
                                   c->spec_d.p, c->pairs_d.p, c->comps_d.p, c->filtw_d.p, 1, 0);
                fft_buckets(c, false);
                hipLaunchKernelGGL(pair_reffilt_kernel, pg, dim3(256), 0, c->stream, c->fft_d.p, c->pairs_d.p, c->comps_d.p, sp, c->synspan_d.p,
                                   c->reffiltpair_d.p, c->normsrc_d.p, c->reffilt_d.p);
            }
        }
        if (!fuse && !spec_direct_all)
        hipLaunchKernelGGL(misfit_kernel, dim3((unsigned)c->nmis, (unsigned)nsrc), dim3(256), 0, c->stream,
                           c->syn_d.p, c->syn_stride, c->comps_d.p, c->reft_d.p, c->tw_d.p, c->moment_d.p,
                           c->risetime_d.p, mp, c->misfit_d.p, proc, c->fft_d.p, c->vt_d.p,
                           c->synspan_d.p, c->pairs_d.p, synrow);
        if (c->floating) {
            hipLaunchKernelGGL(floating_norm_kernel, dim3((unsigned)c->nmis, (unsigned)nsrc), dim3(256), 0, c->stream,
                               c->vt_d.p, c->syn_stride, c->comps_d.p, c->refx_d.p, c->tw_d.p, fl_method, c->gm.dt,
                               c->syn_factor, c->nmis, c->max_ns, c->partial_d.p, c->synspan_d.p);
            const int nth = nsrc * c->nrec_en;
            hipLaunchKernelGGL(floating_select_kernel, dim3((unsigned)((nth + 127) / 128)), dim3(128), 0, c->stream,
                               c->partial_d.p, c->comps_d.p, c->recfirst_d.p, c->nrec_en, c->nmis, c->max_ns, fl_method,
                               isrc0, nsrc, c->misfit_d.p, c->fshift_d.p);
        }
        if (c->fft_needed) {
            if (c->untapered_fft) {
                const dim3 pg((unsigned)c->nmis, (unsigned)nsrc);
                hipLaunchKernelGGL(untapered_rows_kernel<false>, pg, dim3(256), 0, c->stream, c->syn_d.p, c->syn_stride, c->comps_d.p, c->reft_d.p,
                                   c->moment_d.p, c->risetime_d.p, isrc0, c->gm.dt, c->nmis, spansrc, nrec, c->synspan_d.p, c->pairs_d.p, c->fft_d.p);
            }
            const SynRows sr{ c->syn_d.p, c->syn_stride, c->comps_d.p, c->tw_d.p, c->moment_d.p, c->risetime_d.p, synrow };
            if (any_lds) for (auto &b : c->buckets) if (sp.in_lds(b.ntrans)) fused_fft_table(c, b.ntrans);
            if (spectral) {
                if (any_lds) {
                    if (direct_ok)
                        hipLaunchKernelGGL(spec_fft_norm_kernel<2>, dim3((unsigned)nsrc, (unsigned)c->nmis), dim3(256), (size_t)lds_longest * 4, c->stream,
                                           (const float *)nullptr, c->pairs_d.p, fused_fft_tables(c), c->refamp_d.p, c->filtw_d.p, sp, c->misfit_d.p, (float *)nullptr, sr);
                    else
                        hipLaunchKernelGGL(spec_fft_norm_kernel<0>, dim3((unsigned)nsrc, (unsigned)c->nmis), dim3(256), (size_t)lds_longest * 4, c->stream,
                                           c->fft_d.p, c->pairs_d.p, fused_fft_tables(c), c->refamp_d.p, c->filtw_d.p, sp, c->misfit_d.p, (float *)nullptr, sr);
                }
                if (any_lib) {
                    fft_buckets(c, true, lds_lo, lds_hi);
                    hipLaunchKernelGGL(spec_norm_kernel, dim3((unsigned)c->nmis, (unsigned)nsrc), dim3(256), 0, c->stream,
                                       c->spec_d.p, c->pairs_d.p, c->refamp_d.p, c->filtw_d.p, sp, c->misfit_d.p, c->comps_d.p);
                }
            } else {
                if (any_lds)
                    hipLaunchKernelGGL(spec_fft_filter_norm_kernel<0>, dim3((unsigned)nsrc, (unsigned)c->nmis), dim3(256), (size_t)lds_longest * 4, c->stream,
                                       (const float *)nullptr, c->pairs_d.p, fused_fft_tables(c), c->comps_d.p, c->filtw_d.p, c->reffilt_d.p, c->zmask_d.p, sp,
                                       c->misfit_d.p, (float *)nullptr, sr);
                if (any_lib) {
                    fft_buckets(c, true, lds_lo, lds_hi);
                    hipLaunchKernelGGL(spec_filter_kernel, dim3((unsigned)(c->nmis * nsrc)), dim3(256), 0, c->stream,
                                       c->spec_d.p, c->pairs_d.p, c->comps_d.p, c->filtw_d.p, lds_lo, lds_hi);
                    fft_buckets(c, false, lds_lo, lds_hi);
                    hipLaunchKernelGGL(filtered_norm_kernel, dim3((unsigned)c->nmis, (unsigned)nsrc), dim3(256), 0, c->stream,
                                       c->fft_d.p, c->comps_d.p, c->pairs_d.p, c->reffilt_d.p, c->zmask_d.p, sp, c->misfit_d.p,
                                       proc_which == 3 ? proc : nullptr, c->syn_stride, c->synspan_d.p);
                }
            }
        }
        hipLaunchKernelGGL(global_kernel, dim3((unsigned)((nsrc + 127) / 128)), dim3(128), 0, c->stream,
                           c->misfit_d.p, c->norm_d.p, c->recfirst_d.p, c->nrec_en, c->nmis, isrc0, nsrc, c->global_d.p,
                           c->any_failed ? c->status_d.p : (const int *)nullptr,
                           c->fft_needed ? c->normsrc_d.p : (const float *)nullptr);
    }
    record(c, 2, e3);
    HIPCHECK(hipGetLastError());
    if (c->events.size() >= 3 * 2048) {
        HIPCHECK(hipStreamSynchronize(c->stream));
        for (auto &ev : c->events) { if (ev.kind == 0) c->event_pool.push_back(ev.a); c->event_pool.push_back(ev.b); }
        c->events.clear();
    }
    c->events.push_back({ e0, e1, 0 });
    c->events.push_back({ e1, e2, 1 });
    c->events.push_back({ e2, e3, 2 });
    c->last_chunk0 = isrc0; c->last_chunkn = nsrc;
    if (proc_which) { c->proc_chunk0 = isrc0; c->proc_chunkn = nsrc; c->proc_which_held = proc_which; }
    else c->proc_which_held = c->proc_which_held;
}

int eval_impl(kiwi_hip_ctx *c, int isrc0, int nsrc, int proc_which)
{
    if (isrc0 < 0 || nsrc < 0 || isrc0 + nsrc > c->nsrc) throw std::runtime_error("source range out of bounds");
    HIPCHECK(hipSetDevice(c->device));
    prepare(c);
    c->misfit_d.ensure((size_t)c->nsrc * c->nmis, &c->dev_bytes);
    c->global_d.ensure((size_t)c->nsrc, &c->dev_bytes);
    if (c->fft_needed && !c->fft_ready) prepare_fft(c, c->reft_h);
    const int nrec = (int)c->recv.size();
    c->fuse_now = can_fuse(c, proc_which, isrc0, nsrc);
    int s = isrc0;
    while (s < isrc0 + nsrc) {
        size_t bytes = 0;
        int n = 0;
        while (s + n < isrc0 + nsrc) {
            const size_t nc = (size_t)(c->cent_ofs[s + n + 1] - c->cent_ofs[s + n]);
            const size_t syn_bytes = c->fuse_now ? (size_t)c->nmis * 64 * sizeof(double)
                                                             : c->syn_stride * sizeof(float) * ((proc_which ? 2 : 1) + (c->floating ? 1 : 0));
            const size_t add = nc * nrec * (sizeof(GeoRec) + (c->accum_mode == 0 ? 512 + kCoefLine * sizeof(float) : 0)) + syn_bytes;
            if (n > 0 && (bytes + add > c->chunk_bytes_limit || n >= 65535)) break;
            if (c->fft_needed && n >= c->fft_cap) break;
            bytes += add; n++;
        }
        run_chunk(c, s, n, proc_which);
        s += n;
    }
    c->last_isrc0 = isrc0; c->last_nsrc = nsrc; c->last_proc_which = proc_which;
    c->evaluated.resize((size_t)c->nsrc, 0);
    std::fill(c->evaluated.begin() + isrc0, c->evaluated.begin() + isrc0 + nsrc, 1);
    return 0;
}

}

#include "kiwi_gfk.hpp"
#include "kiwi_outer.hpp"
#include "kiwi_linfit.hpp"
#include "kiwi_linfit_robust.hpp"
#include "kiwi_linfit_wide.hpp"
#include "kiwi_linfit_candidates.hpp"
#include "kiwi_bands.hpp"
#include "kiwi_timescan.hpp"
#include "kiwi_linfit_timescan.hpp"

typedef unsigned int read_u4 __attribute__((ext_vector_type(4)));
__global__ __launch_bounds__(256) void read_fill_kernel(read_u4 *p, size_t n16)
{
    for (size_t i = (size_t)blockIdx.x * 256 + threadIdx.x; i < n16; i += (size_t)gridDim.x * 256)
        p[i] = read_u4{ (unsigned)i, 1u, 2u, 3u };
}
__global__ __launch_bounds__(256) void read_in_order_kernel(const read_u4 *__restrict__ p, size_t n16, unsigned *__restrict__ sink)
{
    const size_t per = (n16 + gridDim.x - 1) / gridDim.x;
    const size_t a = per * blockIdx.x, b = a + per < n16 ? a + per : n16;
    unsigned x = 0u, y = 0u, z = 0u, w = 0u;
    size_t i = a + threadIdx.x;
    for (; i + 7 * 256 < b; i += 8 * 256) {
        read_u4 v[8];
#pragma unroll
        for (int k = 0; k < 8; k++) v[k] = __builtin_nontemporal_load(p + i + 256 * k);
#pragma unroll
        for (int k = 0; k < 8; k++) { x ^= v[k].x; y ^= v[k].y; z ^= v[k].z; w ^= v[k].w; }
    }
    for (; i < b; i += 256) { const read_u4 v = p[i]; x ^= v.x; y ^= v.y; z ^= v.z; w ^= v.w; }
    if ((x ^ y ^ z ^ w) == 0x9e3779b9u) sink[blockIdx.x] = x;
}

extern "C" {

int kiwi_hip_init(int device, kiwi_hip_ctx **out)
{
    kmp_set_blocktime(0);
    kiwi_hip_ctx *c = nullptr;
    try {
        int ndev = 0;
        hipError_t e = hipGetDeviceCount(&ndev);
        if (e != hipSuccess || ndev <= 0)
            return fail(nullptr, std::string("no HIP device available: ") + hipGetErrorString(e));
        if (device < 0 || device >= ndev) return fail(nullptr, "device index out of range");
        HIPCHECK(hipSetDevice(device));
        c = new kiwi_hip_ctx();
        c->device = device;
        HIPCHECK(hipStreamCreateWithFlags(&c->stream, hipStreamNonBlocking));
        if (const char *m = std::getenv("KIWI_HIP_GROUP_THREADS")) {
            const int v = std::atoi(m);
            if (v == 64 || v == 128 || v == 256) { c->group_threads = v; c->group_threads_env = 1; }
        }
        if (const char *m = std::getenv("KIWI_HIP_ACCUM")) c->accum_mode = (std::strcmp(m, "direct") == 0) ? 1 : 0;
        if (const char *m = std::getenv("KIWI_HIP_FUSE")) c->fuse_enabled = std::atoi(m);
        if (const char *m = std::getenv("KIWI_HIP_DUO")) { const int v = std::atoi(m); c->duo = v >= 4 ? 4 : (v >= 1 ? 2 : 0); }
        if (const char *m = std::getenv("KIWI_HIP_CELL")) c->cell_mode = std::atoi(m) ? 1 : 0;
        if (const char *m = std::getenv("KIWI_HIP_DEDUPE")) c->dedupe_enabled = std::atoi(m);
        if (const char *m = std::getenv("KIWI_HIP_FUSED_FFT")) c->fused_fft = std::atoi(m) != 0;
        if (const char *m = std::getenv("KIWI_HIP_ARITH")) {
            if (std::strcmp(m, "fused") == 0 || std::strcmp(m, "fma") == 0) c->arith = KIWI_ARITH_FUSED;
            else if (std::strcmp(m, "exact") != 0) throw std::runtime_error("KIWI_HIP_ARITH: exact or fused");
        }
        if (const char *m = std::getenv("KIWI_HIP_CELL_WAVE")) c->cell_wave = std::atoi(m) ? 1 : 0;
        if (const char *m = std::getenv("KIWI_HIP_COMPACT")) c->compact = std::atoi(m) ? 1 : 0;
        if (const char *m = std::getenv("KIWI_HIP_CHUNK_MB")) {
            const long v = std::atol(m);
            if (v > 0) c->chunk_bytes_limit = (size_t)v << 20;
        }
        if (const char *m = std::getenv("KIWI_HIP_EIK_DEVICE")) c->eik_solver = std::atoi(m) ? 1 : 0;
        if (const char *m = std::getenv("KIWI_HIP_RUNS")) {
            const int v = std::atoi(m);
            c->share_runs = v != 0;
            if (v > 1) c->max_run = v;
        }
        *out = c;
        return 0;
    } catch (const std::exception &e) {
        delete c;
        return fail(nullptr, e.what());
    }
}

int kiwi_hip_init_multi(int ndev_wanted, kiwi_hip_ctx **out)
{
    if (!out) return fail(nullptr, "null argument");
    *out = nullptr;
    int ndev = 0;
    hipError_t e = hipGetDeviceCount(&ndev);
    if (e != hipSuccess || ndev <= 0) return fail(nullptr, std::string("no HIP device available: ") + hipGetErrorString(e));
    int n = ndev_wanted <= 0 ? ndev : ndev_wanted;
    const char *over = std::getenv("KIWI_HIP_MULTI_OVERSUBSCRIBE");
    if (n > ndev && !(over && std::atoi(over) != 0))
        return fail(nullptr, "kiwi_hip_init_multi: " + std::to_string(n) + " devices wanted, " + std::to_string(ndev) + " visible");
    kiwi_hip_ctx *c = nullptr;
    if (int rc = kiwi_hip_init(0, &c)) return rc;
    for (int i = 1; i < n; i++) {
        kiwi_hip_ctx *m = nullptr;
        if (int rc = kiwi_hip_init(i % ndev, &m)) { kiwi_hip_destroy(c); return rc; }
        c->mates.push_back(m);
    }
    c->cpu_share = n;
    for (kiwi_hip_ctx *m : c->mates) m->cpu_share = n;
    if (hipSetDevice(c->device) != hipSuccess) { kiwi_hip_destroy(c); return fail(nullptr, "hipSetDevice failed"); }
    *out = c;
    return 0;
}

int kiwi_hip_ndevices(kiwi_hip_ctx *c, int *n)
{
    if (!c || !n) return fail(c, "null argument");
    *n = 1 + (int)c->mates.size();
    return 0;
}

int kiwi_hip_destroy(kiwi_hip_ctx *c)
{
    if (!c) return 0;
    for (kiwi_hip_ctx *m : c->mates) kiwi_hip_destroy(m);
    c->mates.clear();
    (void)hipSetDevice(c->device);
    (void)hipStreamSynchronize(c->stream);
    for (auto &ev : c->events) {
        if (ev.kind == 0) (void)hipEventDestroy(ev.a);
        (void)hipEventDestroy(ev.b);
    }
    for (auto e : c->event_pool) (void)hipEventDestroy(e);
    for (auto &kv : c->plans) (void)hipfftDestroy(kv.second);
    if (c->ntr_pin) (void)hipHostFree(c->ntr_pin);
    if (c->mate_pin) (void)hipHostFree(c->mate_pin);
    if (c->mate_event) (void)hipEventDestroy(c->mate_event);
    if (c->pairs_pin) (void)hipHostFree(c->pairs_pin);
    if (c->size_event) (void)hipEventDestroy(c->size_event);
    c->fmm.release();
    (void)hipStreamDestroy(c->stream);
    delete c;
    return 0;
}

// ... 335 lines not shown
    return 0;
    GUARD_END(c)
}

int kiwi_hip_set_source_constraints(kiwi_hip_ctx *c, int n, const float *points, const float *normals)
{
    GUARD_BEGIN
    if (n < 0) throw std::runtime_error("negative number of constraints");
    c->constraints.resize((size_t)n);
    for (int i = 0; i < n; i++)
        for (int k = 0; k < 3; k++) { c->constraints[i].point[k] = points[3 * i + k]; c->constraints[i].normal[k] = normals[3 * i + k]; }
    return forward(c, [&](kiwi_hip_ctx *m) { return kiwi_hip_set_source_constraints(m, n, points, normals); });
    GUARD_END(c)
}

static bool eik_staged_env();
static void eikonal_staged(const kiwi_hip_ctx *c, int where, int sourcetype, const std::vector<int> &idx, const float *params, int np, float edt,
                           const CrustProfile &prof, const std::vector<HalfSpace> &cons, int nthreads, DiscreteSource *ds,
                           std::vector<std::string> &errs, double *solve_ms, int *nsolved);

int kiwi_hip_discretize_eikonal(int sourcetype, const float *params, int nparams, float effective_dt,
                                const float *rupture_profile, int ncon, const float *points, const float *normals,
                                float *cent, int maxcent, int *ncent, float *moment, float *risetime)
{
    try {
        if (source_nparams_eikonal(sourcetype) != nparams) return 2;
        std::vector<HalfSpace> cons((size_t)std::max(ncon, 0));
        for (int i = 0; i < ncon; i++)
            for (int k = 0; k < 3; k++) { cons[i].point[k] = points[3 * i + k]; cons[i].normal[k] = normals[3 * i + k]; }
        DiscreteSource ds;
        std::string err;
        if (eik_staged_env()) {
            std::vector<std::string> errs;
            eikonal_staged(nullptr, 0, sourcetype, std::vector<int>{ 0 }, params, nparams, effective_dt, unpack_profile(rupture_profile), cons, 1, &ds, errs, nullptr, nullptr);
            err = errs[0];
        } else err = discretize_eikonal(sourcetype, params, effective_dt, unpack_profile(rupture_profile), cons, ds);
        if (!err.empty()) return err[0] == 'E' ? 5 : 6;
        *ncent = (int)ds.centroids.size();
        if (moment) *moment = ds.moment;
        if (risetime) *risetime = ds.risetime;
        if (cent) {
            if (*ncent > maxcent) return 4;
            std::memcpy(cent, ds.centroids.data(), ds.centroids.size() * sizeof(Centroid));
        }
        return 0;
    } catch (...) { return 1; }
}

int kiwi_hip_discretize(int sourcetype, const float *params, int nparams, float effective_dt,
                        float *cent, int maxcent, int *ncent, float *moment, float *risetime)
{
    try {
        if (source_nparams(sourcetype) != nparams) return 2;
        DiscreteSource ds;
        if (!discretize(sourcetype, params, effective_dt, ds)) return 3;
        *ncent = (int)ds.centroids.size();
        if (moment) *moment = ds.moment;
        if (risetime) *risetime = ds.risetime;
        if (cent) {
            if (*ncent > maxcent) return 4;
            std::memcpy(cent, ds.centroids.data(), ds.centroids.size() * sizeof(Centroid));
        }
        return 0;
    } catch (...) { return 1; }
}

int kiwi_hip_set_sources(kiwi_hip_ctx *c, int nsrc, const int *cent_ofs, const float *cent,
                         const float *moment, const float *risetime)
{
    GUARD_BEGIN
    if (nsrc < 1) throw std::runtime_error("need at least one source");
    if (!c->have_db) throw std::runtime_error("set the database before the sources");
    HIPCHECK(hipSetDevice(c->device));
    if (cent_ofs[0] != 0) throw std::runtime_error("cent_ofs[0] must be 0");
    for (int s = 0; s < nsrc; s++) if (cent_ofs[s + 1] < cent_ofs[s]) throw std::runtime_error("cent_ofs not monotone");
    const size_t ntot = (size_t)cent_ofs[nsrc];
    float maxrise = 0.f;
    for (int s = 0; s < nsrc; s++) maxrise = std::max(maxrise, risetime[s]);
    if (2 * fold_halfwidth(maxrise, c->gm.dt) + 1 > kMaxFold) throw std::runtime_error("rise time too long for the fold kernel");
    c->cent_ofs.assign(cent_ofs, cent_ofs + nsrc + 1);
    c->geo_hash.assign((size_t)nsrc, 0ull);
    c->struct_hash.assign((size_t)nsrc, 0ull);
    c->group_lens.assign(ntot, 0);
    c->first_shift.assign((size_t)nsrc, 0);
    c->src_ends.assign((size_t)nsrc * 6, 0.f);
    c->single_group.assign((size_t)nsrc, 0);
    {
        const float dt = c->gm.dt;
#pragma omp parallel for schedule(static) num_threads(std::max(1, std::min(8, nsrc / 512)))
        for (int s = 0; s < nsrc; s++) {
            const float *ce = cent + (size_t)cent_ofs[s] * 10;
            const int nc = cent_ofs[s + 1] - cent_ofs[s];
            unsigned long long h = 1469598103934665603ull ^ (unsigned long long)nc;
            unsigned long long hs = 1469598103934665603ull ^ (unsigned long long)nc;
            bool one = nc >= 1 && nc <= kMaxGroup;
            int smin = 0, smax = 0;
            for (int k = 0; k < nc; k++) {
                unsigned int w[4];
                std::memcpy(w, ce + (size_t)k * 10, sizeof(w));
                for (int q = 0; q < 4; q++) { h ^= w[q]; h *= 1099511628211ull; }

                if (one) {
                    const float *p = ce + (size_t)k * 10;
                    if (!(p[0] == ce[0] && p[1] == ce[1] && p[2] == ce[2])) one = false;
                    const int sh = (int)std::floor(p[3] / dt);
                    if (k == 0) smin = smax = sh; else { smin = std::min(smin, sh); smax = std::max(smax, sh); }
                    if (smax - smin > kHalo - 10) one = false;
                }
            }
            for (int k = 0; k < nc;) {
                const float *g0 = ce + (size_t)k * 10;
                int len = 1, lo = (int)std::floor(g0[3] / dt), hi = lo;
                for (int q = k + 1; q < nc && len < kMaxGroup; q++) {
                    const float *p = ce + (size_t)q * 10;
                    if (!(p[0] == g0[0] && p[1] == g0[1] && p[2] == g0[2])) break;
                    const int sh = (int)std::floor(p[3] / dt);
                    const int nlo = std::min(lo, sh), nhi = std::max(hi, sh);
                    if (nhi - nlo > kHalo - 10) break;
                    lo = nlo; hi = nhi; len++;
                }
                hs ^= (unsigned)len; hs *= 1099511628211ull;
                c->group_lens[(size_t)cent_ofs[s] + k] = (unsigned char)len;
                k += len;
            }
            c->geo_hash[s] = h;
            c->struct_hash[s] = hs;
            c->first_shift[s] = nc > 0 ? (int)std::floor(ce[3] / dt) : 0;
            if (nc > 0)
                for (int q = 0; q < 3; q++) { c->src_ends[(size_t)s * 6 + q] = ce[q]; c->src_ends[(size_t)s * 6 + 3 + q] = ce[(size_t)(nc - 1) * 10 + q]; }
            c->single_group[s] = one ? 1 : 0;
        }
        c->same_as.assign((size_t)nsrc, 0);
        c->any_same = false;
        {
            std::vector<unsigned long long> th((size_t)nsrc);
#pragma omp parallel for schedule(static) num_threads(std::max(1, std::min(8, nsrc / 512)))
            for (int s = 0; s < nsrc; s++) {
                const unsigned int *w = reinterpret_cast<const unsigned int *>(cent + (size_t)cent_ofs[s] * 10);
                const size_t n = (size_t)(cent_ofs[s + 1] - cent_ofs[s]) * 10;
                unsigned long long h = 1469598103934665603ull ^ (unsigned long long)n;
                for (size_t q = 0; q < n; q++) { h ^= w[q]; h *= 1099511628211ull; }
                th[s] = h;
            }
            std::map<unsigned long long, int> first_of;
            for (int s = 0; s < nsrc; s++) {
                c->same_as[s] = s;
                const int nc = cent_ofs[s + 1] - cent_ofs[s];
                if (nc == 0) continue;
                auto it = first_of.find(th[s]);
                if (it == first_of.end()) { first_of[th[s]] = s; continue; }
                const int f = it->second;
                if (cent_ofs[f + 1] - cent_ofs[f] == nc &&
                    std::memcmp(cent + (size_t)cent_ofs[f] * 10, cent + (size_t)cent_ofs[s] * 10, (size_t)nc * 10 * sizeof(float)) == 0) {
                    c->same_as[s] = f;
                    c->any_same = true;
                }
            }
        }
        long long npts = 0, ncen = 0;
        const int stride = std::max(1, nsrc / 64);
        for (int s = 0; s < nsrc; s += stride) {
            const float *ce = cent + (size_t)cent_ofs[s] * 10;
            const int nc = cent_ofs[s + 1] - cent_ofs[s];
            for (int k = 0; k < nc; k++) {
                const float *p = ce + (size_t)k * 10, *q = p - 10;
                if (k == 0 || !(p[0] == q[0] && p[1] == q[1] && p[2] == q[2])) npts++;
            }
            ncen += nc;
        }
        c->points_per_centroid = ncen > 0 ? (double)npts / (double)ncen : 0.0;
    }
    c->cent_d.ensure(std::max<size_t>(ntot, 1) * 10, &c->dev_bytes);
    c->centofs_d.ensure((size_t)nsrc + 1, &c->dev_bytes);
    c->moment_d.ensure((size_t)nsrc, &c->dev_bytes);
    c->risetime_d.ensure((size_t)nsrc, &c->dev_bytes);
    HIPCHECK(hipMemcpy(c->cent_d.p, cent, ntot * 10 * sizeof(float), hipMemcpyHostToDevice));
    HIPCHECK(hipMemcpy(c->centofs_d.p, cent_ofs, ((size_t)nsrc + 1) * sizeof(int), hipMemcpyHostToDevice));
    HIPCHECK(hipMemcpy(c->moment_d.p, moment, (size_t)nsrc * sizeof(float), hipMemcpyHostToDevice));
    HIPCHECK(hipMemcpy(c->risetime_d.p, risetime, (size_t)nsrc * sizeof(float), hipMemcpyHostToDevice));
    c->nsrc = nsrc;
    c->src_status.assign((size_t)nsrc, 0);
    c->any_failed = false;
    c->evaluated.assign((size_t)nsrc, 0);
    if (c->prepared) {
        c->misfit_d.ensure((size_t)nsrc * c->nmis, &c->dev_bytes);
        c->global_d.ensure((size_t)nsrc, &c->dev_bytes);
    }
    if (fold_halfwidth(maxrise, c->gm.dt) != fold_halfwidth(c->max_risetime, c->gm.dt)) c->prepared = false;
    c->max_risetime = maxrise;
    if (c->synth_only || c->any_untapered) c->prepared = false;
    c->last_nsrc = 0;
    c->proc_which_held = 0;
    c->fft_ready = false;
    return 0;
    GUARD_END(c)
}

static int effective_cpus()
{
    static const int n = [] {
        int hw = std::max(1, omp_get_num_procs());
        double quota = 0.0;
        if (FILE *f = std::fopen("/sys/fs/cgroup/cpu.max", "r")) {
            char q[64]; long long per = 0;
            if (std::fscanf(f, "%63s %lld", q, &per) == 2 && std::strcmp(q, "max") != 0 && per > 0) quota = std::atof(q) / (double)per;
// ... 1628 lines not shown
```

### kiwi_amd/csrc/kiwi_linfit.hpp

```cpp

namespace linfit {

constexpr int kMaxBasis = 8;
constexpr int kThreads = 256;

__host__ __device__ constexpr int nn_of(int K) { return K * (K + 1) / 2 + K + 1; }
__host__ __device__ constexpr int tri(int K, int i, int j) { return i * K - i * (i - 1) / 2 + (j - i); }

template <int K>
__global__ __launch_bounds__(kThreads) void linfit_gram_kernel(const float *__restrict__ proc, size_t syn_stride,
                                                               const RecvDev *__restrict__ recv, const CompDev *__restrict__ comps,
                                                               const float *__restrict__ reft, const float *__restrict__ reffilt,
                                                               const FftPair *__restrict__ pairs, int nmis, int nrec, float syn_factor,
                                                               float dt, double *__restrict__ nbr)
{
    constexpr int NG = K * (K + 1) / 2, NN = NG + K + 1;
    __shared__ double part[kThreads / 64][NN];
    const int r = (int)blockIdx.x, g = (int)blockIdx.y, tid = (int)threadIdx.x;
    const RecvDev rd = recv[r];
    if (!rd.enabled) return;
    const bool unit = (syn_factor == 1.f);
    const float *__restrict__ src0 = proc + (size_t)g * K * syn_stride;
    double acc[NN];
#pragma unroll
// ... 253 lines not shown
    DevBuf<double> x, misfit, scale, tile_v, best_misfit;
    DevBuf<float> rmis, rnorm;
    DevBuf<int> tile_i, best_index, status;
};
static void check_candidates(const Candidates &cd, int K);
static size_t cand_bytes(const Candidates &cd, int nrec);
static void cand_chunk(kiwi_hip_ctx *c, int K, int g0, int ng, const double *w_d, int anarchy, const double *nbr, const double *normal,
                       const Candidates &cd, CandBufs &b, hipEvent_t after_kernels);
static void cand_fill_failed(int ngroup, int nrec, const Candidates &cd);

static void check_setup(kiwi_hip_ctx *c, int K, const Out &out, const Robust *rb = nullptr, const Wide *wd = nullptr)
{
    const int kmax = wd ? kWideMaxBasis : kMaxBasis;
    if (K < 1 || K > kmax)
        throw std::runtime_error("linear_fit: K = " + std::to_string(K) + " basis sources per group; 1 to " + std::to_string(kmax) + " are supported");
    if (wd) {
        if (wd->nonneg != 0 && wd->nonneg != 1) throw std::runtime_error("linear_fit_wide: nonneg = " + std::to_string(wd->nonneg) + " must be 0 or 1");
        if (wd->penalty)
            for (int p = 0; p < K * (K + 1) / 2; p++)
                if (!std::isfinite(wd->penalty[p])) throw std::runtime_error("linear_fit_wide: penalty entry " + std::to_string(p) + " is not finite");
    }
    if (!out.coef || !out.misfit || !out.status) throw std::runtime_error("linear_fit: null coef, misfit or status array");
    if (c->method == KIWI_FLOATING_L2NORM || c->method == KIWI_FLOATING_L1NORM)
        throw std::runtime_error("linear_fit: floating shift ranges make the misfit a minimum over shifts, which is not quadratic in the coefficients; set l2norm");
    if (c->method != KIWI_L2NORM && !(rb && rb->mode == 1 && c->method == KIWI_L1NORM))
        throw std::runtime_error("linear_fit: the misfit method must be l2norm (the only inner norm that is quadratic in the coefficients)");
    prepare(c);
    if (c->synth_only) throw std::runtime_error("linear_fit: every enabled receiver component needs a reference seismogram");
    if (c->any_untapered)
        throw std::runtime_error("linear_fit: an enabled receiver has no misfit taper (its comparison span follows the source, so the basis traces have no common span)");
}

static void run(kiwi_hip_ctx *c, int isrc0, int ngroup, int K, const double *receiver_weight, int anarchy, const Out &out,
                const Robust *rb = nullptr, const Wide *wd = nullptr, const Candidates *cd = nullptr)
{
    if (cd) check_candidates(*cd, K);
    check_setup(c, K, out, rb, wd);
    if (isrc0 < 0 || ngroup < 0 || (long long)isrc0 + (long long)ngroup * K > (long long)c->nsrc)
        throw std::runtime_error("linear_fit: sources " + std::to_string(isrc0) + " .. " + std::to_string((long long)isrc0 + (long long)ngroup * K) +
                                 " are not inside the uploaded batch of " + std::to_string(c->nsrc));
    if (ngroup == 0) return;
    const int nrec = (int)c->recv.size(), NN = nn_of(K);
    struct Restore {
        kiwi_hip_ctx *c; bool fused, touched;
        static void drop_variants(kiwi_hip_ctx *c) { c->variants.clear(); c->refamp_h.clear(); c->filtw_h.clear(); c->reffilt_h.clear(); }
        ~Restore() { if (touched) { c->fused_fft = fused; drop_variants(c); } }
    } restore{ c, c->fused_fft, false };
    if (c->fft_needed && c->fused_fft) { c->fused_fft = false; Restore::drop_variants(c); restore.touched = true; }
    c->misfit_d.ensure((size_t)c->nsrc * c->nmis, &c->dev_bytes);
    c->global_d.ensure((size_t)c->nsrc, &c->dev_bytes);
    if (c->fft_needed && !c->fft_ready) prepare_fft(c, c->reft_h);
    const int proc_which = c->any_filter ? 3 : 2;
    c->fuse_now = can_fuse(c, proc_which, isrc0, ngroup * K);
    if (c->fft_needed && c->fft_cap < K) throw std::runtime_error("linear_fit: the transform workspace (KIWI_HIP_CHUNK_MB) does not hold one group");

    std::vector<double> w((size_t)nrec, 0.0);
    for (int r = 0; r < nrec; r++)
        if (c->recv[r].enabled && c->recv[r].ncomp > 0) w[r] = receiver_weight ? receiver_weight[r] : 1.0;
    DevBuf<double> w_d, nbr_d, coef_d, mis_d, piv_d, normal_d, wbr_d, trace_d;
    const size_t trace_len = rb ? (size_t)(rb->niter + 1) * 2 : 0;
    DevBuf<int> st_d, npos_d, nsol_d;
    DevBuf<double> penalty_d;
    CandBufs cand;
    w_d.alloc((size_t)nrec, &c->dev_bytes);
    HIPCHECK(hipMemcpyAsync(w_d.p, w.data(), (size_t)nrec * sizeof(double), hipMemcpyHostToDevice, c->stream));
    if (wd && wd->penalty) {
        penalty_d.alloc((size_t)(K * (K + 1) / 2), &c->dev_bytes);
        HIPCHECK(hipMemcpyAsync(penalty_d.p, wd->penalty, (size_t)(K * (K + 1) / 2) * sizeof(double), hipMemcpyHostToDevice, c->stream));
    }
    HIPCHECK(hipStreamSynchronize(c->stream));

    hipEvent_t ev[6];
    for (int i = 0; i < 6; i++) ev[i] = c->get_event();
    struct Return { kiwi_hip_ctx *c; hipEvent_t *ev; ~Return() { for (int i = 0; i < 6; i++) c->event_pool.push_back(ev[i]); } } ret{ c, ev };
    std::vector<double> piv_h;
    int g0 = 0;
    while (g0 < ngroup) {
        size_t bytes = 0;
        int ng = 0;
        while (g0 + ng < ngroup) {
            size_t add = 0;
            for (int s = isrc0 + (g0 + ng) * K; s < isrc0 + (g0 + ng + 1) * K; s++) {
                const size_t nc = (size_t)(c->cent_ofs[s + 1] - c->cent_ofs[s]);
                add += nc * nrec * (sizeof(GeoRec) + (c->accum_mode == 0 ? 512 + kCoefLine * sizeof(float) : 0)) + c->syn_stride * sizeof(float) * 2;
            }
            add += (size_t)nrec * (NN + (rb && rb->mode == 1 ? NN + 2 : 0)) * sizeof(double);
            if (cd) add += cand_bytes(*cd, nrec);
            if (ng > 0 && (bytes + add > c->chunk_bytes_limit || (ng + 1) * K > 65535)) break;
            if (c->fft_needed && (ng + 1) * K > c->fft_cap) break;
            bytes += add; ng++;
        }
        const int s0 = isrc0 + g0 * K;
        HIPCHECK(hipEventRecord(ev[0], c->stream));
        run_chunk(c, s0, ng * K, proc_which);
        HIPCHECK(hipEventRecord(ev[1], c->stream));
        nbr_d.ensure((size_t)ng * nrec * NN, &c->dev_bytes);
        coef_d.ensure((size_t)ng * K, &c->dev_bytes); mis_d.ensure((size_t)ng, &c->dev_bytes); piv_d.ensure((size_t)ng, &c->dev_bytes);
        st_d.ensure((size_t)ng, &c->dev_bytes);
        if (out.normal || cd) normal_d.ensure((size_t)ng * NN, &c->dev_bytes);
        HIPCHECK(hipMemsetAsync(nbr_d.p, 0, (size_t)ng * nrec * NN * sizeof(double), c->stream));
        if (wd) {
            npos_d.ensure((size_t)ng, &c->dev_bytes); nsol_d.ensure((size_t)ng, &c->dev_bytes);
            wide_launch(c, K, ng, c->fft_needed ? c->pairs_d.p : (const FftPair *)nullptr, w_d.p, anarchy ? 1 : 0, *wd, penalty_d.p, nbr_d.p,
                        coef_d.p, mis_d.p, st_d.p, piv_d.p, npos_d.p, nsol_d.p, out.normal ? normal_d.p : (double *)nullptr, ev[5]);
        } else
            launch_any(c, K, ng, c->fft_needed ? c->pairs_d.p : (const FftPair *)nullptr, w_d.p, anarchy ? 1 : 0, nbr_d.p, coef_d.p, mis_d.p,
                       st_d.p, piv_d.p, out.normal || cd ? normal_d.p : (double *)nullptr);
        HIPCHECK(hipEventRecord(ev[2], c->stream));
        if (rb) {
            if (rb->mode == 1) wbr_d.ensure((size_t)ng * nrec * (NN + 2), &c->dev_bytes);
            trace_d.ensure((size_t)ng * trace_len, &c->dev_bytes);
            robust_launch_any(c, K, ng, c->fft_needed ? c->pairs_d.p : (const FftPair *)nullptr, w_d.p, anarchy ? 1 : 0, nbr_d.p, *rb, wbr_d.p,
                              coef_d.p, mis_d.p, st_d.p, trace_d.p);
        }
        if (cd) cand_chunk(c, K, g0, ng, w_d.p, anarchy ? 1 : 0, nbr_d.p, normal_d.p, *cd, cand, ev[3]);
        else HIPCHECK(hipEventRecord(ev[3], c->stream));
        piv_h.resize((size_t)ng);
        HIPCHECK(hipMemcpyAsync(out.coef + (size_t)g0 * K, coef_d.p, (size_t)ng * K * sizeof(double), hipMemcpyDeviceToHost, c->stream));
        HIPCHECK(hipMemcpyAsync(out.misfit + g0, mis_d.p, (size_t)ng * sizeof(double), hipMemcpyDeviceToHost, c->stream));
        HIPCHECK(hipMemcpyAsync(out.status + g0, st_d.p, (size_t)ng * sizeof(int), hipMemcpyDeviceToHost, c->stream));
        HIPCHECK(hipMemcpyAsync(out.pivot_min ? out.pivot_min + g0 : piv_h.data(), piv_d.p, (size_t)ng * sizeof(double), hipMemcpyDeviceToHost, c->stream));
        if (out.normal)
            HIPCHECK(hipMemcpyAsync(out.normal + (size_t)g0 * NN, normal_d.p, (size_t)ng * NN * sizeof(double), hipMemcpyDeviceToHost, c->stream));
        if (out.by_receiver)
            HIPCHECK(hipMemcpyAsync(out.by_receiver + (size_t)g0 * nrec * NN, nbr_d.p, (size_t)ng * nrec * NN * sizeof(double), hipMemcpyDeviceToHost, c->stream));
        if (wd && out.npositive)
            HIPCHECK(hipMemcpyAsync(out.npositive + g0, npos_d.p, (size_t)ng * sizeof(int), hipMemcpyDeviceToHost, c->stream));
        if (wd && out.nsolves)
            HIPCHECK(hipMemcpyAsync(out.nsolves + g0, nsol_d.p, (size_t)ng * sizeof(int), hipMemcpyDeviceToHost, c->stream));
        if (rb && out.trace)
            HIPCHECK(hipMemcpyAsync(out.trace + (size_t)g0 * trace_len, trace_d.p, (size_t)ng * trace_len * sizeof(double), hipMemcpyDeviceToHost, c->stream));
        HIPCHECK(hipEventRecord(ev[4], c->stream));
        HIPCHECK(hipStreamSynchronize(c->stream));
        for (int i = 0; i < 4; i++) {
            float t = 0.f;
            HIPCHECK(hipEventElapsedTime(&t, ev[i], ev[i + 1]));
            c->linfit_ms[i] += t;
        }
        if (wd) {
            float t = 0.f;
            HIPCHECK(hipEventElapsedTime(&t, ev[1], ev[5]));
            c->linfit_wide_ms[0] += t;
            HIPCHECK(hipEventElapsedTime(&t, ev[5], ev[2]));
            c->linfit_wide_ms[1] += t;
        }
        g0 += ng;
    }
    c->last_isrc0 = isrc0; c->last_nsrc = ngroup * K; c->last_proc_which = proc_which;
    c->evaluated.resize((size_t)c->nsrc, 0);
    std::fill(c->evaluated.begin() + isrc0, c->evaluated.begin() + isrc0 + ngroup * K, 1);
    const double nan = std::numeric_limits<double>::quiet_NaN();
    for (int g = 0; g < ngroup; g++) {
        bool bad = false;
        for (int i = 0; i < K; i++) if (c->src_status[(size_t)isrc0 + (size_t)g * K + i]) bad = true;
        if (!bad) continue;
        out.status[g] = 2;
        out.misfit[g] = nan;
        for (int i = 0; i < K; i++) out.coef[(size_t)g * K + i] = nan;
        if (out.trace) std::fill(out.trace + (size_t)g * out.trace_rows * 2, out.trace + (size_t)(g + 1) * out.trace_rows * 2, nan);
        if (out.npositive) out.npositive[g] = 0;
        if (out.nsolves) out.nsolves[g] = 0;
        if (cd) cand_fill_failed(1, nrec, cd->at(g, nrec));
    }
}

static void fill_failed(int ngroup, int K, int nrec, const Out &out)
{
// ... 16 lines not shown
```

### kiwi_amd/csrc/kiwi_linfit_timescan.hpp

```cpp

namespace linfit_timescan {

constexpr int kThreads = 256;
constexpr int kTile = 512;
constexpr int kPerPass[linfit::kMaxBasis + 1] = { 0, 8, 8, 8, 6, 4, 4, 2, 2 };
static_assert(kTile % kThreads == 0, "a thread's samples and their order must not depend on the tiling");

struct GramArgs {
    SynRows sr;
    const RecvDev *recv;
    const float *reft;
    int isrc0;
    int nrec, k0, kstep, nk;
    int lds_row;
    float dt, syn_factor;
    double *nbr;
};

template <int K, int J>
__global__ __launch_bounds__(kThreads) void linfit_scan_gram_kernel(GramArgs a)
{
    constexpr int NG = K * (K + 1) / 2, NP = NG + K, NN = NP + 1, NACC = J * NP + 1;
    extern __shared__ __attribute__((aligned(16))) float rows[];
    __shared__ double part[kThreads / 64][NACC];
// ... 139 lines not shown
    double *pivot_min;
    int *best;
    double *normal;
    Out at(size_t g, size_t K, size_t nk) const
    {
        const size_t nn = (size_t)linfit::nn_of((int)K);
        return Out{ coef + g * nk * K, misfit + g * nk, status + g * nk, pivot_min ? pivot_min + g * nk : nullptr, best ? best + g : nullptr,
                    normal ? normal + g * nk * nn : nullptr };
    }
};

static void mark_failed(size_t g, size_t K, size_t nk, const Out &out)
{
    const double nan = std::numeric_limits<double>::quiet_NaN();
    std::fill(out.status + g * nk, out.status + (g + 1) * nk, 2);
    std::fill(out.misfit + g * nk, out.misfit + (g + 1) * nk, nan);
    std::fill(out.coef + g * nk * K, out.coef + (g + 1) * nk * K, nan);
    if (out.best) out.best[g] = -1;
}

static void fill_failed(size_t ngroup, size_t K, size_t nk, const Out &out)
{
    for (size_t g = 0; g < ngroup; g++) mark_failed(g, K, nk, out);
    if (out.pivot_min) std::fill(out.pivot_min, out.pivot_min + ngroup * nk, 0.0);
    if (out.normal) std::memset(out.normal, 0, ngroup * nk * (size_t)linfit::nn_of((int)K) * sizeof(double));
}

static void check_setup(kiwi_hip_ctx *c, int K, const timescan::Offsets &of, const Out &out)
{
    linfit::check_setup(c, K, linfit::Out{ out.coef, out.misfit, out.status });
    timescan::check_setup(c, of.k0, of.kstep, of.nk);
    if (c->any_filter)
        throw std::runtime_error("linear_fit_time_scan: an enabled receiver has a misfit filter; the taper sits in front of the filter, so every "
                                     "basis source and offset would need a transform of its own, which is not supported");
}

static void run(kiwi_hip_ctx *c, int isrc0, int ngroup, int K, const timescan::Offsets &of, const double *receiver_weight, int anarchy, const Out &out)
{
    check_setup(c, K, of, out);
    if (isrc0 < 0 || ngroup < 0 || (long long)isrc0 + (long long)ngroup * K > (long long)c->nsrc)
        throw std::runtime_error("linear_fit_time_scan: sources " + std::to_string(isrc0) + " .. " +
                                 std::to_string((long long)isrc0 + (long long)ngroup * K) + " are not inside the uploaded batch of " +
                                 std::to_string(c->nsrc));
    if (ngroup == 0) return;
    const int nrec = (int)c->recv.size(), NN = linfit::nn_of(K), nk = of.nk;
    c->misfit_d.ensure((size_t)c->nsrc * c->nmis, &c->dev_bytes);
    c->global_d.ensure((size_t)c->nsrc, &c->dev_bytes);
    const int base = c->halo, shalo = of.max_abs();
    c->fuse_now = false;
    struct Restore {
        kiwi_hip_ctx *c; bool want; int halo;
        ~Restore()
        {
            c->want_spansrc = want;
            try { HIPCHECK(hipSetDevice(c->device)); timescan::set_halo(c, halo); }
            catch (...) { c->prepared = false; }
        }
    } restore{ c, c->want_spansrc, base };
    c->want_spansrc = true;
    timescan::set_halo(c, base + shalo);

    std::vector<double> w((size_t)nrec, 0.0);
    for (int r = 0; r < nrec; r++)
        if (c->recv[r].enabled && c->recv[r].ncomp > 0) w[r] = receiver_weight ? receiver_weight[r] : 1.0;
    DevBuf<double> w_d, nbr_d, coef_d, mis_d, piv_d, normal_d;
    DevBuf<int> st_d, best_d;
    w_d.alloc((size_t)nrec, &c->dev_bytes);
    HIPCHECK(hipMemcpyAsync(w_d.p, w.data(), (size_t)nrec * sizeof(double), hipMemcpyHostToDevice, c->stream));
    HIPCHECK(hipStreamSynchronize(c->stream));

    hipEvent_t ev[5];
    for (int i = 0; i < 5; i++) ev[i] = c->get_event();
    struct Return { kiwi_hip_ctx *c; hipEvent_t *ev; ~Return() { for (int i = 0; i < 5; i++) c->event_pool.push_back(ev[i]); } } ret{ c, ev };
    std::vector<double> piv_h;
    std::vector<int> best_h;
    int g0 = 0;
    while (g0 < ngroup) {
        size_t bytes = 0;
        int ng = 0;
        while (g0 + ng < ngroup) {
            size_t add = 0;
            for (int s = isrc0 + (g0 + ng) * K; s < isrc0 + (g0 + ng + 1) * K; s++) {
                const size_t nc = (size_t)(c->cent_ofs[s + 1] - c->cent_ofs[s]);
                add += nc * nrec * (sizeof(GeoRec) + (c->accum_mode == 0 ? 512 + kCoefLine * sizeof(float) : 0)) + c->syn_stride * sizeof(float);
            }
            add += (size_t)nk * nrec * NN * sizeof(double);
            if (ng > 0 && (bytes + add > c->chunk_bytes_limit || (ng + 1) * K > 65535)) break;
            bytes += add; ng++;
        }
        const int s0 = isrc0 + g0 * K;
        const size_t nsolve = (size_t)ng * nk;
        HIPCHECK(hipEventRecord(ev[0], c->stream));
        run_chunk(c, s0, ng * K, 0);
        HIPCHECK(hipEventRecord(ev[1], c->stream));
        nbr_d.ensure(nsolve * nrec * NN, &c->dev_bytes);
        coef_d.ensure(nsolve * K, &c->dev_bytes); mis_d.ensure(nsolve, &c->dev_bytes); piv_d.ensure(nsolve, &c->dev_bytes);
        st_d.ensure(nsolve, &c->dev_bytes); best_d.ensure((size_t)ng, &c->dev_bytes);
        if (out.normal) normal_d.ensure(nsolve * NN, &c->dev_bytes);
        HIPCHECK(hipMemsetAsync(nbr_d.p, 0, nsolve * nrec * NN * sizeof(double), c->stream));
        GramArgs a;
        a.sr = SynRows{ c->syn_d.p, c->syn_stride, c->comps_d.p, c->tw_d.p, c->moment_d.p, c->risetime_d.p, nullptr };
        a.recv = c->recv_d.p;
        a.reft = c->reft_d.p;
        a.isrc0 = s0; a.nrec = nrec; a.k0 = of.k0; a.kstep = of.kstep; a.nk = nk;
        a.lds_row = kTile + (std::min(kPerPass[K], nk) - 1) * of.kstep;
        a.dt = c->gm.dt; a.syn_factor = c->syn_factor;
        a.nbr = nbr_d.p;
        launch_any(c, K, a, ng, w_d.p, anarchy ? 1 : 0, coef_d.p, mis_d.p, st_d.p, piv_d.p, out.normal ? normal_d.p : (double *)nullptr, best_d.p, ev[2]);
        HIPCHECK(hipEventRecord(ev[3], c->stream));
        piv_h.resize(nsolve); best_h.resize((size_t)ng);
        const size_t o = (size_t)g0 * nk;
        HIPCHECK(hipMemcpyAsync(out.coef + o * K, coef_d.p, nsolve * K * sizeof(double), hipMemcpyDeviceToHost, c->stream));
        HIPCHECK(hipMemcpyAsync(out.misfit + o, mis_d.p, nsolve * sizeof(double), hipMemcpyDeviceToHost, c->stream));
        HIPCHECK(hipMemcpyAsync(out.status + o, st_d.p, nsolve * sizeof(int), hipMemcpyDeviceToHost, c->stream));
        HIPCHECK(hipMemcpyAsync(out.pivot_min ? out.pivot_min + o : piv_h.data(), piv_d.p, nsolve * sizeof(double), hipMemcpyDeviceToHost, c->stream));
        HIPCHECK(hipMemcpyAsync(out.best ? out.best + g0 : best_h.data(), best_d.p, (size_t)ng * sizeof(int), hipMemcpyDeviceToHost, c->stream));
        if (out.normal) HIPCHECK(hipMemcpyAsync(out.normal + o * NN, normal_d.p, nsolve * NN * sizeof(double), hipMemcpyDeviceToHost, c->stream));
        HIPCHECK(hipEventRecord(ev[4], c->stream));
        HIPCHECK(hipStreamSynchronize(c->stream));
        for (int i = 0; i < 4; i++) {
            float t = 0.f;
            HIPCHECK(hipEventElapsedTime(&t, ev[i], ev[i + 1]));
            c->linfit_timescan_ms[i] += t;
        }
        g0 += ng;
    }
    c->last_isrc0 = isrc0; c->last_nsrc = ngroup * K; c->last_proc_which = 0;
    c->evaluated.resize((size_t)c->nsrc, 0);
    std::fill(c->evaluated.begin() + isrc0, c->evaluated.begin() + isrc0 + ngroup * K, 1);
    for (int g = 0; g < ngroup; g++) {
        bool bad = false;
        for (int i = 0; i < K; i++) if (c->src_status[(size_t)isrc0 + (size_t)g * K + i]) bad = true;
        if (bad) mark_failed((size_t)g, (size_t)K, (size_t)nk, out);
    }
}

}
```

### kiwi_amd/csrc/kiwi_timescan.hpp

```cpp

namespace timescan {

constexpr int kMaxShift = 1024;
constexpr int kMaxOffsets = 256;
constexpr int kPerPass = 4;
constexpr int kMaxDynLds = 148 * 1024;

struct ScanArgs {
    SynRows sr;
    const float *reft;
    const float *norm_slot;
    const float *norm_src;
    const FftPair *pairs;
    FusedFftTables tabs;
    const float *refamp, *filtw, *reffilt, *zmask;
    const int *status;
    int method, spectral, any_filter;
    int nmis, isrc0, k0, kstep, nk, shalo;
    int zf_floats;
    float dt, syn_factor;
    float *mis_out;
    float *norm_out;
};

// ... 230 lines not shown
    prepare(c);
    if (c->synth_only) throw std::runtime_error("time_scan: every enabled receiver component needs a reference seismogram");
    if (c->any_untapered)
        throw std::runtime_error("time_scan: an enabled receiver has no misfit taper (its comparison span follows the source, which the scan moves)");
}

static void set_halo(kiwi_hip_ctx *c, int halo)
{
    size_t synofs = 0;
    c->max_wlen = 0;
    for (RecvDev &d : c->recv_h) {
        if (!d.enabled) continue;
        d.wbeg = c->comps[(size_t)d.slot0].w0 - halo;
        d.wlen = c->comps[(size_t)d.slot0].wlen + 2 * halo;
        c->max_wlen = std::max(c->max_wlen, d.wlen);
        for (int k = 0; k < d.ncomp; k++) {
            CompDev &cd = c->comps[(size_t)d.slot0 + k];
            cd.synofs = (int)synofs; cd.halo = halo;
            d.synofs[k] = (int)synofs;
            synofs += ((size_t)d.wlen + 3) / 4 * 4;
        }
    }
    c->halo = halo;
    c->syn_stride = synofs;
    HIPCHECK(hipMemcpyAsync(c->recv_d.p, c->recv_h.data(), c->recv_h.size() * sizeof(RecvDev), hipMemcpyHostToDevice, c->stream));
    HIPCHECK(hipMemcpyAsync(c->comps_d.p, c->comps.data(), c->comps.size() * sizeof(CompDev), hipMemcpyHostToDevice, c->stream));
    HIPCHECK(hipStreamSynchronize(c->stream));
}

static void run(kiwi_hip_ctx *c, int isrc0, int nsrc, const Offsets &of, const Out &out)
{
    check_setup(c, of.k0, of.kstep, of.nk);
    if (isrc0 < 0 || nsrc < 0 || (long long)isrc0 + nsrc > (long long)c->nsrc)
        throw std::runtime_error("time_scan: sources " + std::to_string(isrc0) + " .. " + std::to_string((long long)isrc0 + nsrc) +
                                 " are not inside the uploaded batch of " + std::to_string(c->nsrc));
    if (nsrc == 0) return;
    TimeScanState &st = c->timescan_state;
    const int nrec = (int)c->recv.size(), nmis = c->nmis, nk = of.nk;
    const bool spectral = c->method == KIWI_AMPSPEC_L2NORM || c->method == KIWI_AMPSPEC_L1NORM;
    if (c->fft_needed && !c->fused_fft)
        throw std::runtime_error("time_scan: slots with a frequency filter or an amplitude-spectrum method go through the in-LDS transforms, "
                                 "which KIWI_HIP_FUSED_FFT=0 switches off");
    c->misfit_d.ensure((size_t)c->nsrc * c->nmis, &c->dev_bytes);
    c->global_d.ensure((size_t)c->nsrc, &c->dev_bytes);
    if (c->fft_needed && !c->fft_ready) prepare_fft(c, c->reft_h);
    const int base = c->halo, shalo = of.max_abs();
    int max_w = 0, ntr_bound = 0;
    for (const CompDev &cd : c->comps) {
        max_w = std::max(max_w, cd.wlen);
        if (c->fft_needed && (spectral || cd.has_filter)) ntr_bound = std::max(ntr_bound, std::min(cd.ntrans_max, 1 << kFusedFftMaxLog2));
    }
    const int row_len = max_w + 2 * (base + shalo), row_limit = kMaxDynLds / 4 - ntr_bound;
    if (row_len > row_limit)
        throw std::runtime_error("time_scan: a row of " + std::to_string(row_len) + " samples (window " + std::to_string(max_w) + " + 2 x halo " +
                                 std::to_string(base + shalo) + ") does not fit in LDS" +
                                 (ntr_bound ? " beside a transform of " + std::to_string(ntr_bound) + " samples" : std::string()) + "; the limit is " +
                                 std::to_string(row_limit));
    c->fuse_now = false;
    struct Restore {
        kiwi_hip_ctx *c; bool want; int halo;
        ~Restore()
        {
            c->want_spansrc = want;
            try { HIPCHECK(hipSetDevice(c->device)); set_halo(c, halo); }
            catch (...) { c->prepared = false; }
        }
    } restore{ c, c->want_spansrc, base };
    c->want_spansrc = true;
    set_halo(c, base + shalo);
    if (!st.attr) {
        HIPCHECK(hipFuncSetAttribute(reinterpret_cast<const void *>(&time_scan_kernel), hipFuncAttributeMaxDynamicSharedMemorySize, kMaxDynLds));
        st.attr = true;
    }

    hipEvent_t ev[4];
    for (int i = 0; i < 4; i++) ev[i] = c->get_event();
    struct Return { kiwi_hip_ctx *c; hipEvent_t *ev; ~Return() { for (int i = 0; i < 4; i++) c->event_pool.push_back(ev[i]); } } ret{ c, ev };
    int s = isrc0;
    while (s < isrc0 + nsrc) {
        size_t bytes = 0;
        int n = 0;
        while (s + n < isrc0 + nsrc) {
            const size_t nc = (size_t)(c->cent_ofs[s + n + 1] - c->cent_ofs[s + n]);
            const size_t add = nc * nrec * (sizeof(GeoRec) + (c->accum_mode == 0 ? 512 + kCoefLine * sizeof(float) : 0)) + c->syn_stride * sizeof(float) +
                               ((size_t)nk * nmis + nmis + nk + 1) * sizeof(float);
            if (n > 0 && (bytes + add > c->chunk_bytes_limit || n >= 65535)) break;
            if (c->fft_needed && n >= c->fft_cap) break;
            bytes += add; n++;
        }
        HIPCHECK(hipEventRecord(ev[0], c->stream));
        run_chunk(c, s, n, 0);
        HIPCHECK(hipEventRecord(ev[1], c->stream));
        int longest = 0;
        if (c->fft_needed) {
            for (size_t i = 0; i < (size_t)n * nmis; i++) {
                const int m = (int)(i % (size_t)nmis), nt = c->ntr_pin[i];
                if (!spectral && !c->comps[(size_t)m].has_filter) continue;
                if (nt < (1 << kFusedFftMinLog2) || nt > (1 << kFusedFftMaxLog2))
                    throw std::runtime_error("time_scan: source " + std::to_string(s + (int)(i / (size_t)nmis) + 1) + ", misfit slot " + std::to_string(m + 1) +
                                             " needs a transform of " + std::to_string(nt) + " samples; the in-LDS transforms take " +
                                             std::to_string(1 << kFusedFftMinLog2) + " to " + std::to_string(1 << kFusedFftMaxLog2));
                longest = std::max(longest, nt);
            }
        }
        const size_t nout = (size_t)n * nk * nmis;
        st.mis_d.ensure(nout, &c->dev_bytes); st.norm_d.ensure((size_t)n * nmis, &c->dev_bytes);
        st.glob_d.ensure((size_t)n * nk, &c->dev_bytes); st.best_d.ensure((size_t)n, &c->dev_bytes);
        ScanArgs a;
        a.sr = SynRows{ c->syn_d.p, c->syn_stride, c->comps_d.p, c->tw_d.p, c->moment_d.p, c->risetime_d.p, nullptr };
        a.reft = c->reft_d.p;
        a.norm_slot = c->norm_d.p;
        a.norm_src = c->fft_needed ? c->normsrc_d.p : nullptr;
        a.pairs = c->fft_needed ? c->pairs_d.p : nullptr;
        a.tabs = c->fft_needed ? fused_fft_tables(c) : FusedFftTables{};
        a.refamp = c->refamp_d.p; a.filtw = c->filtw_d.p; a.reffilt = c->reffilt_d.p; a.zmask = c->zmask_d.p;
        a.status = c->any_failed ? c->status_d.p : nullptr;
        a.method = c->method; a.spectral = spectral ? 1 : 0; a.any_filter = c->any_filter ? 1 : 0;
        a.nmis = nmis; a.isrc0 = s; a.k0 = of.k0; a.kstep = of.kstep; a.nk = nk; a.shalo = shalo;
        a.zf_floats = longest;
        a.dt = c->gm.dt; a.syn_factor = c->syn_factor;
        a.mis_out = st.mis_d.p; a.norm_out = st.norm_d.p;
        const size_t dyn = ((size_t)longest + (size_t)max_w + 2 * (size_t)shalo) * sizeof(float);
        hipLaunchKernelGGL(time_scan_kernel, dim3((unsigned)n, (unsigned)nmis), dim3(256), dyn, c->stream, a);
        hipLaunchKernelGGL(time_scan_global_kernel, dim3((unsigned)n), dim3(kMaxOffsets), 0, c->stream, st.mis_d.p, st.norm_d.p, c->recfirst_d.p,
                           c->nrec_en, nmis, nk, s, st.glob_d.p, st.best_d.p, c->any_failed ? c->status_d.p : (const int *)nullptr);
        HIPCHECK(hipGetLastError());
        HIPCHECK(hipEventRecord(ev[2], c->stream));
        const Out o = out.at((size_t)(s - isrc0), (size_t)nk, (size_t)nmis);
        if (o.misfit) HIPCHECK(hipMemcpyAsync(o.misfit, st.mis_d.p, nout * sizeof(float), hipMemcpyDeviceToHost, c->stream));
        if (o.norm) HIPCHECK(hipMemcpyAsync(o.norm, st.norm_d.p, (size_t)n * nmis * sizeof(float), hipMemcpyDeviceToHost, c->stream));
        if (o.global) HIPCHECK(hipMemcpyAsync(o.global, st.glob_d.p, (size_t)n * nk * sizeof(float), hipMemcpyDeviceToHost, c->stream));
        if (o.best) HIPCHECK(hipMemcpyAsync(o.best, st.best_d.p, (size_t)n * sizeof(int), hipMemcpyDeviceToHost, c->stream));
        HIPCHECK(hipEventRecord(ev[3], c->stream));
        HIPCHECK(hipStreamSynchronize(c->stream));
        for (int i = 0; i < 3; i++) {
            float t = 0.f;
            HIPCHECK(hipEventElapsedTime(&t, ev[i], ev[i + 1]));
            c->timescan_ms[i] += t;
        }
        s += n;
    }
    c->last_isrc0 = isrc0; c->last_nsrc = nsrc; c->last_proc_which = 0;
    c->evaluated.resize((size_t)c->nsrc, 0);
    std::fill(c->evaluated.begin() + isrc0, c->evaluated.begin() + isrc0 + nsrc, 1);
}

}
```

Before: 34950.

## Precompute per-group descriptor plans for multi-source accumulate kernel

Adds a small pre-pass kernel that builds, for each group and receiver, a packed plan record holding the row bases, offsets, weights, shift bounds and sharing flags. The multi-source accumulate kernel can then read these descriptors with scalar loads instead of doing per-lane record loads, shuffles and ballot checks. A descriptor abstraction (lane-based or plan-based) is threaded through the halo and row issue helpers. This costs an extra kernel launch, extra device memory and host bookkeeping, and it is gated on an environment/context flag.

```diff
diff --git a/kiwi_amd/csrc/kiwi_accum.hip b/kiwi_amd/csrc/kiwi_accum.hip
--- a/kiwi_amd/csrc/kiwi_accum.hip
+++ b/kiwi_amd/csrc/kiwi_accum.hip
@@ -54,23 +54,33 @@
 #endif
 
 #if KIWI_FAMILY == 3
-template <int NG, int NS, bool COMPACT>
+template <int NG, int NS, bool COMPACT, bool PLAN>
 static void multi_t(const AccumArgs &a, dim3 grid, int ntiles, const int *mate, const int *wider)
 {
-    if (a.fuse) hipLaunchKernelGGL((accumulate_multi_kernel<NG, true, NS, COMPACT>), grid, dim3(256), 0, a.stream, KIWI_COMMON_ARGS, ntiles, a.tab, a.coefs, a.fp,
-                                   a.pairflag, mate, wider);
-    else        hipLaunchKernelGGL((accumulate_multi_kernel<NG, false, NS, COMPACT>), grid, dim3(256), 0, a.stream, KIWI_COMMON_ARGS, ntiles, a.tab, a.coefs, a.fp,
-                                   a.pairflag, mate, wider);
+    if (a.fuse) hipLaunchKernelGGL((accumulate_multi_kernel<NG, true, NS, COMPACT, PLAN>), grid, dim3(256), 0, a.stream, KIWI_COMMON_ARGS, ntiles, a.tab, a.coefs, a.fp,
+                                   a.pairflag, mate, wider, a.plan, a.plan_ofs);
+    else        hipLaunchKernelGGL((accumulate_multi_kernel<NG, false, NS, COMPACT, PLAN>), grid, dim3(256), 0, a.stream, KIWI_COMMON_ARGS, ntiles, a.tab, a.coefs, a.fp,
+                                   a.pairflag, mate, wider, a.plan, a.plan_ofs);
 }
 template <int NG, int NS>
 static void multi_c(const AccumArgs &a, dim3 grid, int ntiles, const int *mate, const int *wider)
 {
-    if (a.compact) multi_t<NG, NS, true>(a, grid, ntiles, mate, wider); else multi_t<NG, NS, false>(a, grid, ntiles, mate, wider);
+    if (a.compact && a.plan) multi_t<NG, NS, true, true>(a, grid, ntiles, mate, wider);
+    else if (a.compact) multi_t<NG, NS, true, false>(a, grid, ntiles, mate, wider);
+    else multi_t<NG, NS, false, false>(a, grid, ntiles, mate, wider);
 }
 void launch_multi(const AccumArgs &a, dim3 grid, int NS, int ntiles, const int *mate, const int *wider)
 {
     if (a.ng == 10) { if (NS == 4) multi_c<10, 4>(a, grid, ntiles, mate, wider); else multi_c<10, 2>(a, grid, ntiles, mate, wider); }
     else            { if (NS == 4) multi_c<8, 4>(a, grid, ntiles, mate, wider); else multi_c<8, 2>(a, grid, ntiles, mate, wider); }
+}
+void launch_multi_plan(const AccumArgs &a, int NS, int ngroups, const int *mate, const int *wider, PlanSrc *plan)
+{
+    const dim3 grid((unsigned)ngroups, (unsigned)((a.nrec + 63) / 64));
+    if (NS == 4) hipLaunchKernelGGL(multi_plan_kernel<4>, grid, dim3(64), 0, a.stream, a.recs, a.cent_ofs, a.isrc0, a.nrec, a.recv, a.tab, a.pairflag, mate, wider,
+                                    a.plan_ofs, (int4 *)plan);
+    else         hipLaunchKernelGGL(multi_plan_kernel<2>, grid, dim3(64), 0, a.stream, a.recs, a.cent_ofs, a.isrc0, a.nrec, a.recv, a.tab, a.pairflag, mate, wider,
+                                    a.plan_ofs, (int4 *)plan);
 }
 #endif
 
diff --git a/kiwi_amd/csrc/kiwi_accum.inc b/kiwi_amd/csrc/kiwi_accum.inc
--- a/kiwi_amd/csrc/kiwi_accum.inc
+++ b/kiwi_amd/csrc/kiwi_accum.inc
@@ -301,23 +301,53 @@
 
 struct HaloRegs { f4u v[4]; };
 
+struct DescLanes {
+    int ta, tb;
+    __device__ __forceinline__ int a(int ig, int k) const { return REC_I(ta, 4 * ig + k); }
+    __device__ __forceinline__ int b(int ig, int k) const { return REC_I(tb, 4 * ig + k); }
+    __device__ __forceinline__ int ha(int hig, int k) const { return __shfl(ta, 4 * hig + k, 64); }
+    __device__ __forceinline__ int hb(int hig, int k) const { return __shfl(tb, 4 * hig + k, 64); }
+    __device__ __forceinline__ bool fast(int jb, int lds_tile, int pitch, int lane, int ng) const
+    {
+        const bool lane_ok = lane >= 4 * ng || (ta + jb >= tb && ta + jb + lds_tile <= tb + pitch);
+        return __builtin_amdgcn_ballot_w64(lane_ok) == ~0ull;
+    }
+};
+struct DescPlan {
+    int b0[4], o[4], pitch, hoff;
+    __device__ __forceinline__ int b(int ig, int k) const { return b0[k] + ig * pitch; }
+    __device__ __forceinline__ int a(int ig, int k) const { return b0[k] + ig * pitch + o[k]; }
+    __device__ __forceinline__ int hb(int, int k) const { return b0[k] + hoff; }
+    __device__ __forceinline__ int ha(int, int k) const { return b0[k] + hoff + o[k]; }
+    __device__ __forceinline__ bool fast(int jb, int lds_tile, int pitch_, int, int) const
+    {
+        const int omin = min(min(o[0], o[1]), min(o[2], o[3])), omax = max(max(o[0], o[1]), max(o[2], o[3]));
+        return omin + jb >= 0 && omax + jb + lds_tile <= pitch_;
+    }
+};
+
+template <bool BLEND, bool FAST, typename D>
+__device__ __forceinline__ HaloRegs halo_issue(bool active, int ig, int ph, int jb, const float *__restrict__ G, int pitch, const D &d)
+{
+    HaloRegs h;
+#pragma unroll
+    for (int k = 0; k < (BLEND ? 4 : 1); k++) {
+        const int base = d.ha(ig, k);
+        int idx = base + jb + ph;
+        if constexpr (!FAST) {
+            const int lo = d.hb(ig, k);
+            idx = min(max(idx, lo), lo + pitch - 4);
+        }
+        h.v[k] = f4u{ 0.f, 0.f, 0.f, 0.f };
+        if (active) h.v[k] = *(const f4u *)(G + (size_t)(unsigned)idx);
+    }
+    return h;
+}
 template <bool BLEND, bool FAST>
 __device__ __forceinline__ HaloRegs halo_issue(bool active, int ig, int ph, int jb, const float *__restrict__ G, int pitch,
                                                int ta, int tb)
 {
-    HaloRegs h;
-#pragma unroll
-    for (int k = 0; k < (BLEND ? 4 : 1); k++) {
-        const int base = __shfl(ta, 4 * ig + k, 64);
-        int idx = base + jb + ph;
-        if constexpr (!FAST) {
-            const int lo = __shfl(tb, 4 * ig + k, 64);
-            idx = min(max(idx, lo), lo + pitch - 4);
-        }
-        h.v[k] = f4u{ 0.f, 0.f, 0.f, 0.f };
-        if (active) h.v[k] = *(const f4u *)(G + (size_t)(unsigned)idx);
-    }
-    return h;
+    return halo_issue<BLEND, FAST>(active, ig, ph, jb, G, pitch, DescLanes{ ta, tb });
 }
 
 template <bool BLEND>
@@ -1141,32 +1171,33 @@
     }
 }
 
-template <bool BLEND, bool FAST>
+template <bool BLEND, bool FAST, typename D>
 __device__ __forceinline__ void one_issue(f4u (&v)[BLEND ? 4 : 1], int ig, int p, int jb, const float *__restrict__ G,
-                                          int pitch, int ta, int tb)
+                                          int pitch, const D &d)
 {
     const int j = jb + p;
 #pragma unroll
     for (int k = 0; k < (BLEND ? 4 : 1); k++) {
-        const int base = REC_I(ta, 4 * ig + k);
+        const int base = d.a(ig, k);
         if constexpr (FAST) {
             v[k] = buf_load4(gf_rsrc(G), p, base + jb);
         } else {
-            const int lo = REC_I(tb, 4 * ig + k);
+            const int lo = d.b(ig, k);
             const int idx = min(max(base + j, lo), lo + pitch - 4);
             v[k] = *(const f4u *)(G + (size_t)(unsigned)idx);
         }
     }
 }
 
-__device__ __forceinline__ void one_issue_hidden(f4u (&v)[4], int ig, int p, int jb, const float *__restrict__ G, int ta)
+template <typename D>
+__device__ __forceinline__ void one_issue_hidden(f4u (&v)[4], int ig, int p, int jb, const float *__restrict__ G, const D &d)
 {
     const size_t gi = (size_t)G;
     const v4i_t rs = { (int)(unsigned)gi, (int)((unsigned)(gi >> 32) & 0xffffu), -1, 0x00020000 };
     const int voff = (int)(4u * (unsigned)p);
 #pragma unroll
     for (int k = 0; k < 4; k++) {
-        const int soff = (int)(4u * (unsigned)(REC_I(ta, 4 * ig + k) + jb));
+        const int soff = (int)(4u * (unsigned)(d.a(ig, k) + jb));
         asm volatile("buffer_load_dwordx4 %0, %1, %2, %3 offen" : "=v"(v[k]) : "v"(voff), "s"(rs), "s"(soff));
     }
 }
@@ -1202,14 +1233,15 @@
 typedef float f4m __attribute__((ext_vector_type(4)));
 struct RowsDw { float r[4][4]; };
 
-__device__ __forceinline__ void rows_issue_dw(RowsDw &v, int ig, int lane, int jb, const float *__restrict__ G, int ta)
+template <typename D>
+__device__ __forceinline__ void rows_issue_dw(RowsDw &v, int ig, int lane, int jb, const float *__restrict__ G, const D &d)
 {
     const size_t gi = (size_t)G;
     const v4i_t rs = { (int)(unsigned)gi, (int)((unsigned)(gi >> 32) & 0xffffu), -1, 0x00020000 };
     const int voff = (int)(4u * (unsigned)lane);
 #pragma unroll
     for (int k = 0; k < 4; k++) {
-        const int soff = (int)(4u * (unsigned)(REC_I(ta, 4 * ig + k) + jb));
+        const int soff = (int)(4u * (unsigned)(d.a(ig, k) + jb));
         asm volatile("buffer_load_dword %0, %1, %2, %3 offen" : "=v"(v.r[k][0]) : "v"(voff), "s"(rs), "s"(soff));
         asm volatile("buffer_load_dword %0, %1, %2, %3 offen offset:256" : "=v"(v.r[k][1]) : "v"(voff), "s"(rs), "s"(soff));
         asm volatile("buffer_load_dword %0, %1, %2, %3 offen offset:512" : "=v"(v.r[k][2]) : "v"(voff), "s"(rs), "s"(soff));
@@ -1243,9 +1275,9 @@
 
 template <int NG, int NS> __host__ __device__ constexpr int multi_set_stride() { return NG * (1024 / NS + kHalo) + ((NS == 4 && KIWI_MFMA_BLEND) ? 8 : 0); }
 
-template <int NG, bool FAST, int NS, typename Shadow>
+template <int NG, bool FAST, int NS, typename D, typename Shadow>
 __device__ __forceinline__ void multi_build(float *__restrict__ tile0, int wv, int lane, int tid, int jb, const float *__restrict__ G,
-                                            int pitch, int ta, int tb, const GeoRec (&gw)[NS], int only, bool hact, bool whalo, int hig, int hph,
+                                            int pitch, const D &d, const GeoRec (&gw)[NS], int only, bool hact, bool whalo, int hig, int hph,
                                             Shadow shadow)
 {
     constexpr int TILE = 1024 / NS, LDS_TILE = TILE + kHalo, DEPTH = 3, SET = multi_set_stride<NG, NS>();
@@ -1253,12 +1285,12 @@
     const int p = (NS == 2) ? 4 * (64 * (wv & 1) + lane) : 4 * lane;
     auto comp = [&](int i) { return (NS == 2) ? 2 * i + (wv >> 1) : wv + 4 * i; };
     HaloRegs hv;
-    if (whalo) hv = halo_issue<true, FAST>(true, hig, hph, jb, G, pitch, ta, tb);
+    if (whalo) hv = halo_issue<true, FAST>(true, hig, hph, jb, G, pitch, d);
     const bool last_ok = comp(N - 1) < NG;
     if constexpr (KIWI_MFMA_BLEND && FAST && NS == 4 && KIWI_ARITH == 0) {
         RowsDw v[N];
 #pragma unroll
-        for (int i = 0; i < DEPTH && i < N; i++) if (i < N - 1 || last_ok) rows_issue_dw(v[i], comp(i), lane, jb, G, ta);
+        for (int i = 0; i < DEPTH && i < N; i++) if (i < N - 1 || last_ok) rows_issue_dw(v[i], comp(i), lane, jb, G, d);
         __syncthreads();
         shadow();
         const int me = lane & 3;
@@ -1281,7 +1313,7 @@
                 }
                 mfma_finish(v[i], dst + comp(i) * LDS_TILE, w, write);
             }
-            if (i + DEPTH < N && (i + DEPTH < N - 1 || last_ok)) rows_issue_dw(v[i + DEPTH], comp(i + DEPTH), lane, jb, G, ta);
+            if (i + DEPTH < N && (i + DEPTH < N - 1 || last_ok)) rows_issue_dw(v[i + DEPTH], comp(i + DEPTH), lane, jb, G, d);
         }
         if (whalo) {
 #pragma unroll
@@ -1292,8 +1324,8 @@
     }
     f4u v[N][4];
     auto issue = [&](int i) __attribute__((always_inline)) {
-        if constexpr (FAST) one_issue_hidden(v[i], comp(i), p, jb, G, ta);
-        else one_issue<true, false>(v[i], comp(i), p, jb, G, pitch, ta, tb);
+        if constexpr (FAST) one_issue_hidden(v[i], comp(i), p, jb, G, d);
+        else one_issue<true, false>(v[i], comp(i), p, jb, G, pitch, d);
     };
 #pragma unroll
     for (int i = 0; i < DEPTH && i < N; i++) if (i < N - 1 || last_ok) issue(i);
@@ -1343,16 +1375,90 @@
     return f == 0;
 }
 
-template <int NG, bool FUSE, int NS, bool COMPACT >
+template <int NS>
+__global__ __launch_bounds__(64) void multi_plan_kernel(const GeoRec *__restrict__ recs, const int *__restrict__ cent_ofs, int isrc0, int nrec,
+    const RecvDev *__restrict__ recv, const int *__restrict__ off4, const int *__restrict__ pairflag, const int *__restrict__ mate,
+    const int *__restrict__ mate_wider, const int *__restrict__ plan_ofs, int4 *__restrict__ plan)
+{
+    constexpr int TILE = 1024 / NS, LDS_TILE = TILE + kHalo;
+    const int k = (int)blockIdx.x, s0 = NS * k, r = (int)(blockIdx.y * 64 + threadIdx.x);
+    if (r >= nrec) return;
+    const RecvDev &rv = recv[r];
+    if (!rv.enabled) return;
+    if (!multi_taken<NS>(rv, pairflag, mate, s0, nrec, r)) return;
+    if constexpr (NS == 2) { if (multi_taken<4>(rv, pairflag, mate_wider, s0, nrec, r)) return; }
+    const int cb = cent_ofs[isrc0];
+    const int nc = cent_ofs[isrc0 + s0 + 1] - cent_ofs[isrc0 + s0];
+    const size_t pbeg = (size_t)plan_ofs[k], pend = (size_t)plan_ofs[k + 1];
+    size_t pi = pbeg + (size_t)r;
+    for (int c = 0; c < nc && pi < pend; pi += (size_t)nrec) {
+        const GeoRec *h[NS];
+        int smaxs[NS], smins[NS], npos = 0;
+        bool shared = true, same_rows = true;
+#pragma unroll
+        for (int i = 0; i < NS; i++) {
+            h[i] = recs + ((size_t)(cent_ofs[isrc0 + s0 + i] - cb) * nrec + (size_t)r * nc + c);
+            smaxs[i] = h[i]->ishift + ((h[i]->pad >> 8) & 0xff);
+            smins[i] = h[i]->ishift - ((h[i]->pad >> 16) & 0xff);
+            npos = max(npos, TILE + (smaxs[i] - smins[i]) + 8);
+            if (i > 0) {
+                same_rows = same_rows && h[i]->row[0] == h[0]->row[0] && h[i]->row[1] == h[0]->row[1] && h[i]->row[2] == h[0]->row[2] && h[i]->row[3] == h[0]->row[3];
+                shared = shared && smaxs[i] == smaxs[0];
+            }
+        }
+        shared = shared && same_rows;
+        if (same_rows && !shared) {
+            int smax_c = smaxs[0], smin_c = smins[0];
+#pragma unroll
+            for (int i = 1; i < NS; i++) { smax_c = max(smax_c, smaxs[i]); smin_c = min(smin_c, smins[i]); }
+            if (TILE + (smax_c - smin_c) + 8 <= LDS_TILE) {
+                shared = true;
+                npos = TILE + (smax_c - smin_c) + 8;
+#pragma unroll
+                for (int i = 0; i < NS; i++) smaxs[i] = smax_c;
+            }
+        }
+        const int glen = h[0]->pad & 0xff;
+        int4 *__restrict__ out = plan + pi * (kPlanStride / 16);
+#pragma unroll
+        for (int i = 0; i < NS; i++) {
+            const int4 o = *(const int4 *)(off4 + ((size_t)(cent_ofs[isrc0 + s0 + i] - cb) * nrec + (size_t)r * nc + c) * 4);
+            const int head = (h[i]->flags & 0xffff) | (glen << 16) | ((shared ? 1 : 0) << 23) | ((npos - TILE) << 24);
+            out[4 * i + 0] = make_int4(h[i]->row[0], h[i]->row[1], h[i]->row[2], h[i]->row[3]);
+            out[4 * i + 1] = o;
+            out[4 * i + 2] = make_int4(__float_as_int(h[i]->w[0]), __float_as_int(h[i]->w[1]), __float_as_int(h[i]->w[2]), __float_as_int(h[i]->w[3]));
+            out[4 * i + 3] = make_int4(smaxs[i], head, __float_as_int(h[i]->cl), __float_as_int(h[i]->sl));
+        }
+        if (glen < 1) break;
+        c += glen;
+    }
+}
+
+typedef const __attribute__((address_space(4))) v4i_t *plan_cptr;
+template <int NS>
+__device__ __forceinline__ int plan_warm(size_t p)
+{
+    int d;
+    if constexpr (NS == 4)
+        asm volatile("s_load_dword %0, %1, 0x0\n\ts_load_dword %0, %1, 0x40\n\ts_load_dword %0, %1, 0x80\n\ts_load_dword %0, %1, 0xc0" : "=&s"(d) : "s"(p) : "memory");
+    else
+        asm volatile("s_load_dword %0, %1, 0x0\n\ts_load_dword %0, %1, 0x40" : "=&s"(d) : "s"(p) : "memory");
+    return d;
+}
+
+template <int NG, bool FUSE, int NS, bool COMPACT ,
+          bool PLAN >
 __global__ __launch_bounds__(256) __attribute__((amdgpu_waves_per_eu(3))) void accumulate_multi_kernel(
     const float *__restrict__ G, const int2 *__restrict__ span, int pitch,
     const GeoRec *__restrict__ recs, const int *__restrict__ cent_ofs, int isrc0, int nrec,
     const RecvDev *__restrict__ recv, float *__restrict__ syn, size_t syn_stride, int ntiles,
     const int *__restrict__ tab, const float *__restrict__ coefs, FuseParams fp, const int *__restrict__ pairflag, const int *__restrict__ mate,
-    const int *__restrict__ mate_wider )
+    const int *__restrict__ mate_wider ,
+    const PlanSrc *__restrict__ plan, const int *__restrict__ plan_ofs )
 {
     constexpr bool compact = COMPACT;
     static_assert(NS == 2 || NS == 4, "sources per workgroup");
+    static_assert(!PLAN || COMPACT, "plans hold compact descriptors");
     constexpr int TILE = 1024 / NS, LDS_TILE = TILE + kHalo, K = LDS_TILE / 64, WPS = 4 / NS;
     constexpr int SET = multi_set_stride<NG, NS>();
     __shared__ __attribute__((aligned(16))) float tiles[NS * SET];
@@ -1393,17 +1499,40 @@
     auto tab_of = [&](int i) { return tab + (size_t)rbase[i] * (compact ? 4 : 128); };
     int c = 0;
     int cur[NS];
-#pragma unroll
-    for (int i = 0; i < NS; i++) cur[i] = rec_load(recs_of(i), 0, nc, lane);
     int ta = 0, tb = 0;
-    if constexpr (compact) ta = off4_load(tab_of(0), 0, lane);
-    else { ta = tab_of(0)[lane]; tb = tab_of(0)[64 + lane]; }
+    if constexpr (!PLAN) {
+#pragma unroll
+        for (int i = 0; i < NS; i++) cur[i] = rec_load(recs_of(i), 0, nc, lane);
+        if constexpr (compact) ta = off4_load(tab_of(0), 0, lane);
+        else { ta = tab_of(0)[lane]; tb = tab_of(0)[64 + lane]; }
+    }
     const int hq = 255 - tid, hch = min(hq / NG, 15), hig = hq % NG, hph = TILE + 4 * hch;
+    size_t pcur = 0;
+    if constexpr (PLAN) {
+        const size_t a = (size_t)plan + ((size_t)plan_ofs[blockIdx.x] + (size_t)r) * kPlanStride;
+        pcur = ((size_t)(unsigned)__builtin_amdgcn_readfirstlane((int)(a >> 32)) << 32) | (unsigned)__builtin_amdgcn_readfirstlane((int)a);
+    }
+    const int pstep = nrec * kPlanStride;
+    const int hoff = PLAN ? hig * pitch : 0;
+    auto plan4 = [&](int byte) { return *(plan_cptr)(pcur + (size_t)(unsigned)byte); };
     while (c < nc) {
         GeoRec g[NS];
         int smaxs[NS], smins[NS], npos = 0;
         bool shared = true, same_rows = true;
-        if constexpr (compact) desc_expand(ta, cur[0], lane, pitch, ta, tb);
+        int glen_p = 0;
+        DescPlan dp;
+        if constexpr (PLAN) {
+            const v4i_t rw = plan4(0), of = plan4(16), tl = plan4(48);
+            g[0].row[0] = rw.x;
+            dp = DescPlan{ { 0, (rw.y - rw.x) * pitch, (rw.z - rw.x) * pitch, (rw.w - rw.x) * pitch }, { of.x, of.y, of.z, of.w }, pitch, hoff };
+            const unsigned head = (unsigned)tl.y;
+            glen_p = (int)((head >> 16) & 0x7fu);
+            shared = ((head >> 23) & 1u) != 0u;
+            npos = TILE + (int)(head >> 24);
+            smaxs[0] = tl.x;
+        }
+        if constexpr (compact && !PLAN) desc_expand(ta, cur[0], lane, pitch, ta, tb);
+        if constexpr (!PLAN) {
 #pragma unroll
         for (int i = 0; i < NS; i++) {
             g[i].ishift = REC_I(cur[i], 8);
@@ -1429,15 +1558,29 @@
                 for (int i = 0; i < NS; i++) smaxs[i] = smax_c;
             }
         }
-        const int glen = g[0].pad & 0xff;
+        }
+        const int glen = PLAN ? glen_p : (g[0].pad & 0xff);
         const int cend = c + glen;
         int smax = smaxs[0];
-#pragma unroll
-        for (int i = 1; i < NS; i++) if (sh == i) smax = smaxs[i];
-        int flags = 0, ishv = 0, warm_ = 0;
+        if constexpr (PLAN) smax = plan4(64 * sh + 48).x;
+        else {
+#pragma unroll
+            for (int i = 1; i < NS; i++) if (sh == i) smax = smaxs[i];
+        }
+        int flags = 0, ishv = 0, warm_ = 0, pwarm_ = 0;
         float gcl = 0.f, gsl = 0.f;
         const float *__restrict__ coef_grp = nullptr;
         auto shadow = [&]() {
+            if constexpr (PLAN) {
+#pragma unroll
+                for (int i = 0; i < NS; i++) {
+                    const v4i_t w = plan4(64 * i + 32);
+                    g[i].w[0] = __int_as_float(w.x); g[i].w[1] = __int_as_float(w.y); g[i].w[2] = __int_as_float(w.z); g[i].w[3] = __int_as_float(w.w);
+                }
+                const v4i_t me = plan4(64 * sh + 48);
+                flags = me.y & 0xffff; gcl = __int_as_float(me.z); gsl = __int_as_float(me.w);
+                if (c + glen < nc) pwarm_ = plan_warm<NS>(pcur + (size_t)(unsigned)pstep);
+            } else {
 #pragma unroll
             for (int i = 0; i < NS; i++) { g[i].w[0] = REC_F(cur[i], 4); g[i].w[1] = REC_F(cur[i], 5); g[i].w[2] = REC_F(cur[i], 6); g[i].w[3] = REC_F(cur[i], 7); }
             int curme = cur[0];
@@ -1445,6 +1588,7 @@
             for (int i = 1; i < NS; i++) if (sh == i) curme = cur[i];
             flags = REC_I(curme, 18);
             gcl = REC_F(curme, 16); gsl = REC_F(curme, 17);
+            }
             if (lane < glen) ishv = rc[c + lane].ishift;
             const size_t crow = (base_me + c) * kCoefLine;
             const unsigned clo = __builtin_amdgcn_readfirstlane((unsigned)crow), chi = __builtin_amdgcn_readfirstlane((unsigned)(crow >> 32));
@@ -1452,35 +1596,51 @@
             if constexpr (NG == 10) warm_ = coef_warm(coef_grp);
         };
         auto noshadow = []() {};
-#define KIWI_MULTI_BUILD(TA, TB, I0, ONLY, NPOS, SHADOW) do { \
+#define KIWI_MULTI_BUILD(DESC, I0, ONLY, NPOS, SHADOW) do { \
             const int jb_ = t_tile0 - smaxs[I0] - 1;       \
             const float *__restrict__ Gg = G + (size_t)g[I0].row[0] * (size_t)pitch; \
-            const bool lane_ok = lane >= 4 * NG || ((TA) + jb_ >= (TB) && (TA) + jb_ + LDS_TILE <= (TB) + pitch); \
-            const bool fast = __builtin_amdgcn_ballot_w64(lane_ok) == ~0ull; \
+            const bool fast = (DESC).fast(jb_, LDS_TILE, pitch, lane, NG); \
             const bool hact = hq < 16 * NG && hph < (NPOS); \
             const bool whalo = __builtin_amdgcn_ballot_w64(hact) != 0ull; \
-            if (fast) multi_build<NG, true, NS>(&tiles[0], wv, lane, tid, jb_, Gg, pitch, TA, TB, g, ONLY, hact, whalo, hig, hph, SHADOW); \
-            else      multi_build<NG, false, NS>(&tiles[0], wv, lane, tid, jb_, Gg, pitch, TA, TB, g, ONLY, hact, whalo, hig, hph, SHADOW); } while (0)
+            if (fast) multi_build<NG, true, NS>(&tiles[0], wv, lane, tid, jb_, Gg, pitch, DESC, g, ONLY, hact, whalo, hig, hph, SHADOW); \
+            else      multi_build<NG, false, NS>(&tiles[0], wv, lane, tid, jb_, Gg, pitch, DESC, g, ONLY, hact, whalo, hig, hph, SHADOW); } while (0)
         __builtin_amdgcn_s_setprio(1);
-        if (shared) KIWI_MULTI_BUILD(ta, tb, 0, -1, npos, shadow);
+        if constexpr (PLAN) {
+            if (shared) KIWI_MULTI_BUILD(dp, 0, -1, npos, shadow);
+            else {
+                KIWI_MULTI_BUILD(dp, 0, 0, npos, shadow);
+#pragma unroll
+                for (int i = 1; i < NS; i++) {
+                    const v4i_t rw = plan4(64 * i), of = plan4(64 * i + 16);
+                    smaxs[i] = plan4(64 * i + 48).x;
+                    g[i].row[0] = rw.x;
+                    const DescPlan di{ { 0, (rw.y - rw.x) * pitch, (rw.z - rw.x) * pitch, (rw.w - rw.x) * pitch }, { of.x, of.y, of.z, of.w }, pitch, hoff };
+                    KIWI_MULTI_BUILD(di, i, i, npos, noshadow);
+                }
+            }
+            asm volatile("" :: "s"(pwarm_));
+            pcur += (size_t)(unsigned)pstep;
+        } else {
+        if (shared) KIWI_MULTI_BUILD((DescLanes{ ta, tb }), 0, -1, npos, shadow);
         else {
-            KIWI_MULTI_BUILD(ta, tb, 0, 0, npos, shadow);
+            KIWI_MULTI_BUILD((DescLanes{ ta, tb }), 0, 0, npos, shadow);
 #pragma unroll
             for (int i = 1; i < NS; i++) {
                 int tai, tbi;
                 if constexpr (compact) desc_expand(off4_load(tab_of(i), c, lane), cur[i], lane, pitch, tai, tbi);
                 else { tai = tab_of(i)[(size_t)c * 128 + lane]; tbi = tab_of(i)[(size_t)c * 128 + 64 + lane]; }
                 g[i].row[0] = REC_I(cur[i], 0);
-                KIWI_MULTI_BUILD(tai, tbi, i, i, npos, noshadow);
-            }
-        }
-#undef KIWI_MULTI_BUILD
+                KIWI_MULTI_BUILD((DescLanes{ tai, tbi }), i, i, npos, noshadow);
+            }
+        }
 #pragma unroll
         for (int i = 0; i < NS; i++) cur[i] = rec_load(recs_of(i), cend, nc, lane);
         if (cend < nc) {
             if constexpr (compact) ta = off4_load(tab_of(0), cend, lane);
             else { ta = tab_of(0)[(size_t)cend * 128 + lane]; tb = tab_of(0)[(size_t)cend * 128 + 64 + lane]; }
         }
+        }
+#undef KIWI_MULTI_BUILD
         __syncthreads();
         __builtin_amdgcn_s_setprio(0);
         {
diff --git a/kiwi_amd/csrc/kiwi_accum_api.hpp b/kiwi_amd/csrc/kiwi_accum_api.hpp
--- a/kiwi_amd/csrc/kiwi_accum_api.hpp
+++ b/kiwi_amd/csrc/kiwi_accum_api.hpp
@@ -13,6 +13,8 @@
     const int *tab; const float *coefs; FuseParams fp;
     const int *pairflag, *synrow, *fam_ofs, *fam_list;
     int compact;
+    const PlanSrc *plan = nullptr;
+    const int *plan_ofs = nullptr;
 };
 
 #define KIWI_ACCUM_LAUNCHERS                                                                                                      \
@@ -23,6 +25,8 @@
                         const int *mate4);                                                                                        \
                                                      \
     void launch_multi(const AccumArgs &a, dim3 grid, int NS, int ntiles, const int *mate, const int *mate_wider);                \
+                \
+    void launch_multi_plan(const AccumArgs &a, int NS, int ngroups, const int *mate, const int *mate_wider, PlanSrc *plan);      \
         \
     void launch_cell(const AccumArgs &a, dim3 grid, int ntiles);                                                                  \
     void launch_cellw(const AccumArgs &a, dim3 grid, int ntiles);                                                                 \
diff --git a/kiwi_amd/csrc/kiwi_bands.hpp b/kiwi_amd/csrc/kiwi_bands.hpp
--- a/kiwi_amd/csrc/kiwi_bands.hpp
+++ b/kiwi_amd/csrc/kiwi_bands.hpp
@@ -471,7 +471,7 @@
         int n = 0;
         while (s + n < isrc0 + nsrc) {
             const size_t nc = (size_t)(c->cent_ofs[s + n + 1] - c->cent_ofs[s + n]);
-            const size_t add = nc * nrec * (sizeof(GeoRec) + (c->accum_mode == 0 ? 512 + kCoefLine * sizeof(float) : 0)) + c->syn_stride * sizeof(float) +
+            const size_t add = nc * nrec * (sizeof(GeoRec) + (c->accum_mode == 0 ? 512 + kCoefLine * sizeof(float) : 0)) + plan_bytes(c, s + n, (size_t)nrec) + c->syn_stride * sizeof(float) +
                                (size_t)nband * nmis * 2 * sizeof(float);
             if (n > 0 && (bytes + add > c->chunk_bytes_limit || n >= 65535)) break;
             if (c->fft_needed && n >= c->fft_cap) break;
diff --git a/kiwi_amd/csrc/kiwi_common.hpp b/kiwi_amd/csrc/kiwi_common.hpp
--- a/kiwi_amd/csrc/kiwi_common.hpp
+++ b/kiwi_amd/csrc/kiwi_common.hpp
@@ -83,6 +83,16 @@
 };
 
 constexpr int kCoefLine = 20;
+struct PlanSrc {
+    int   row[4];
+    int   o[4];
+    float w[4];
+    int   smax;
+    int   head;
+    float cl, sl;
+};
+static_assert(sizeof(PlanSrc) == 64, "PlanSrc layout");
+constexpr int kPlanStride = 256;
 template <int NG> __host__ __device__ constexpr int coef_wl(int a) { return 2 * a; }
 template <int NG> __host__ __device__ constexpr int coef_wr(int a) { return 2 * a + 1; }
 
diff --git a/kiwi_amd/csrc/kiwi_hip.hip b/kiwi_amd/csrc/kiwi_hip.hip
--- a/kiwi_amd/csrc/kiwi_hip.hip
+++ b/kiwi_amd/csrc/kiwi_hip.hip
@@ -188,10 +188,14 @@
     std::vector<kiwi_hip_ctx *> mates;
     int cpu_share = 1;
     std::vector<unsigned long long> struct_hash;
+    std::vector<int> ngroups;
     std::vector<unsigned char> group_lens;
     std::vector<int> first_shift;
     std::vector<float> src_ends;
     DevBuf<int> mate_d, mate4_d;
+    DevBuf<int> planofs_d;
+    DevBuf<int4> plan_d;
+    int multi_plan = 1;
     int duo = 4;
     std::vector<char> single_group;
     DevBuf<int> runfirst_d;
@@ -933,6 +937,12 @@
     return v;
 }
 
+size_t plan_bytes(const kiwi_hip_ctx *c, int s, size_t nrec)
+{
+    if (c->accum_mode != 0 || !c->duo || !c->multi_plan || !(c->db_simple && c->compact) || (size_t)s >= c->ngroups.size()) return 0;
+    return (size_t)c->ngroups[(size_t)s] * nrec * (kPlanStride / 2);
+}
+
 void run_chunk(kiwi_hip_ctx *c, int isrc0, int nsrc, int proc_which)
 {
     const int nrec = (int)c->recv.size();
@@ -1075,10 +1085,11 @@
                 }
             }
             bool duo = duo_maybe && !runs && !synrow && maxnc > 0;
-            bool any4 = false, any2 = false;
+            bool any4 = false, any2 = false, planned = false;
+            size_t plan_n4 = 0;
             if (duo) {
                 const size_t n4 = (size_t)(nsrc + 3) / 4, n2 = (size_t)(nsrc + 1) / 2;
-                pin_ensure(c->mate_pin, c->mate_pin_n, n4 + n2);
+                pin_ensure(c->mate_pin, c->mate_pin_n, 2 * (n4 + n2) + 2);
                 if (!c->mate_event) HIPCHECK(hipEventCreateWithFlags(&c->mate_event, hipEventDisableTiming));
                 else HIPCHECK(hipEventSynchronize(c->mate_event));
                 int *m4 = c->mate_pin, *m2 = c->mate_pin + n4;
@@ -1114,6 +1125,23 @@
                     c->mate_d.ensure(n2, &c->dev_bytes);
                     HIPCHECK(hipMemcpyAsync(c->mate4_d.p, m4, n4 * sizeof(int), hipMemcpyHostToDevice, c->stream));
                     HIPCHECK(hipMemcpyAsync(c->mate_d.p, m2, n2 * sizeof(int), hipMemcpyHostToDevice, c->stream));
+                    if (off4 && c->multi_plan) {
+                        int *po = c->mate_pin + n4 + n2;
+                        size_t np = 0;
+                        auto ngroups = [&](int a) { return (size_t)c->ngroups[(size_t)a]; };
+                        for (size_t k = 0; k < n4; k++) { po[k] = (int)np; if (m4[k]) np += ngroups(isrc0 + 4 * (int)k) * (size_t)nrec; }
+                        po[n4] = (int)np;
+                        plan_n4 = np;
+                        for (size_t k = 0; k < n2; k++) { po[n4 + 1 + k] = (int)(np - plan_n4); if (m2[k]) np += ngroups(isrc0 + 2 * (int)k) * (size_t)nrec; }
+                        po[n4 + 1 + n2] = (int)(np - plan_n4);
+                        if (np * (kPlanStride / 16) < ((size_t)1 << 31)) {
+                            c->planofs_d.ensure(n4 + n2 + 2, &c->dev_bytes);
+                            c->plan_d.ensure((np + 1) * (kPlanStride / 16), &c->dev_bytes);
+                            HIPCHECK(hipMemcpyAsync(c->planofs_d.p, po, (n4 + n2 + 2) * sizeof(int), hipMemcpyHostToDevice, c->stream));
+                            if (std::getenv("KIWI_HIP_POISON")) HIPCHECK(hipMemsetAsync(c->plan_d.p, 0x7f, (np + 1) * kPlanStride, c->stream));
+                            planned = true;
+                        }
+                    }
                     HIPCHECK(hipEventRecord(c->mate_event, c->stream));
                 }
             }
@@ -1136,8 +1164,16 @@
                 else exact::launch_cell(aa, cgrid, ntiles_c);
             }
             const int *m2p = any2 ? c->mate_d.p : (const int *)nullptr, *m4p = any4 ? c->mate4_d.p : (const int *)nullptr;
-            if (any4) { if (fusedar) fused::launch_multi(aa, qgrid, 4, ntiles_q, m4p, nullptr); else exact::launch_multi(aa, qgrid, 4, ntiles_q, m4p, nullptr); }
-            if (any2) { if (fusedar) fused::launch_multi(aa, dgrid, 2, ntiles_p, m2p, m4p); else exact::launch_multi(aa, dgrid, 2, ntiles_p, m2p, m4p); }
+            AccumArgs aa4 = aa, aa2 = aa;
+            if (planned) {
+                const size_t n4 = (size_t)(nsrc + 3) / 4;
+                aa4.plan = (const PlanSrc *)c->plan_d.p; aa4.plan_ofs = c->planofs_d.p;
+                aa2.plan = (const PlanSrc *)(c->plan_d.p + plan_n4 * (kPlanStride / 16)); aa2.plan_ofs = c->planofs_d.p + n4 + 1;
+                if (any4) { if (fusedar) fused::launch_multi_plan(aa4, 4, (int)qgrid.x, m4p, nullptr, (PlanSrc *)aa4.plan); else exact::launch_multi_plan(aa4, 4, (int)qgrid.x, m4p, nullptr, (PlanSrc *)aa4.plan); }
+                if (any2) { if (fusedar) fused::launch_multi_plan(aa2, 2, (int)dgrid.x, m2p, m4p, (PlanSrc *)aa2.plan); else exact::launch_multi_plan(aa2, 2, (int)dgrid.x, m2p, m4p, (PlanSrc *)aa2.plan); }
+            }
+            if (any4) { if (fusedar) fused::launch_multi(aa4, qgrid, 4, ntiles_q, m4p, nullptr); else exact::launch_multi(aa4, qgrid, 4, ntiles_q, m4p, nullptr); }
+            if (any2) { if (fusedar) fused::launch_multi(aa2, dgrid, 2, ntiles_p, m2p, m4p); else exact::launch_multi(aa2, dgrid, 2, ntiles_p, m2p, m4p); }
             const int pairsel = cell ? 1 : (duo ? 3 : 0);
             if (fusedar) fused::launch_grouped(aa, ggrid, T, ntiles, runs, pairsel, m2p, m4p);
             else         exact::launch_grouped(aa, ggrid, T, ntiles, runs, pairsel, m2p, m4p);
@@ -1297,7 +1333,7 @@
             const size_t nc = (size_t)(c->cent_ofs[s + n + 1] - c->cent_ofs[s + n]);
             const size_t syn_bytes = c->fuse_now ? (size_t)c->nmis * 64 * sizeof(double)
                                                              : c->syn_stride * sizeof(float) * ((proc_which ? 2 : 1) + (c->floating ? 1 : 0));
-            const size_t add = nc * nrec * (sizeof(GeoRec) + (c->accum_mode == 0 ? 512 + kCoefLine * sizeof(float) : 0)) + syn_bytes;
+            const size_t add = nc * nrec * (sizeof(GeoRec) + (c->accum_mode == 0 ? 512 + kCoefLine * sizeof(float) : 0)) + syn_bytes + plan_bytes(c, s + n, (size_t)nrec);
             if (n > 0 && (bytes + add > c->chunk_bytes_limit || n >= 65535)) break;
             if (c->fft_needed && n >= c->fft_cap) break;
             bytes += add; n++;
@@ -1369,6 +1405,7 @@
         if (const char *m = std::getenv("KIWI_HIP_ACCUM")) c->accum_mode = (std::strcmp(m, "direct") == 0) ? 1 : 0;
         if (const char *m = std::getenv("KIWI_HIP_FUSE")) c->fuse_enabled = std::atoi(m);
         if (const char *m = std::getenv("KIWI_HIP_DUO")) { const int v = std::atoi(m); c->duo = v >= 4 ? 4 : (v >= 1 ? 2 : 0); }
+        if (const char *m = std::getenv("KIWI_HIP_MULTI_PLAN")) c->multi_plan = std::atoi(m) ? 1 : 0;
         if (const char *m = std::getenv("KIWI_HIP_CELL")) c->cell_mode = std::atoi(m) ? 1 : 0;
         if (const char *m = std::getenv("KIWI_HIP_DEDUPE")) c->dedupe_enabled = std::atoi(m);
         if (const char *m = std::getenv("KIWI_HIP_FUSED_FFT")) c->fused_fft = std::atoi(m) != 0;
@@ -1870,6 +1907,7 @@
     c->geo_hash.assign((size_t)nsrc, 0ull);
     c->struct_hash.assign((size_t)nsrc, 0ull);
     c->group_lens.assign(ntot, 0);
+    c->ngroups.assign((size_t)nsrc, 0);
     c->first_shift.assign((size_t)nsrc, 0);
     c->src_ends.assign((size_t)nsrc * 6, 0.f);
     c->single_group.assign((size_t)nsrc, 0);
@@ -1909,6 +1947,7 @@
                 }
                 hs ^= (unsigned)len; hs *= 1099511628211ull;
                 c->group_lens[(size_t)cent_ofs[s] + k] = (unsigned char)len;
+                c->ngroups[(size_t)s]++;
                 k += len;
             }
             c->geo_hash[s] = h;
diff --git a/kiwi_amd/csrc/kiwi_linfit.hpp b/kiwi_amd/csrc/kiwi_linfit.hpp
--- a/kiwi_amd/csrc/kiwi_linfit.hpp
+++ b/kiwi_amd/csrc/kiwi_linfit.hpp
@@ -359,7 +359,7 @@
             size_t add = 0;
             for (int s = isrc0 + (g0 + ng) * K; s < isrc0 + (g0 + ng + 1) * K; s++) {
                 const size_t nc = (size_t)(c->cent_ofs[s + 1] - c->cent_ofs[s]);
-                add += nc * nrec * (sizeof(GeoRec) + (c->accum_mode == 0 ? 512 + kCoefLine * sizeof(float) : 0)) + c->syn_stride * sizeof(float) * 2;
+                add += nc * nrec * (sizeof(GeoRec) + (c->accum_mode == 0 ? 512 + kCoefLine * sizeof(float) : 0)) + plan_bytes(c, s, (size_t)nrec) + c->syn_stride * sizeof(float) * 2;
             }
             add += (size_t)nrec * (NN + (rb && rb->mode == 1 ? NN + 2 : 0)) * sizeof(double);
             if (cd) add += cand_bytes(*cd, nrec);
diff --git a/kiwi_amd/csrc/kiwi_linfit_timescan.hpp b/kiwi_amd/csrc/kiwi_linfit_timescan.hpp
--- a/kiwi_amd/csrc/kiwi_linfit_timescan.hpp
+++ b/kiwi_amd/csrc/kiwi_linfit_timescan.hpp
@@ -245,7 +245,7 @@
             size_t add = 0;
             for (int s = isrc0 + (g0 + ng) * K; s < isrc0 + (g0 + ng + 1) * K; s++) {
                 const size_t nc = (size_t)(c->cent_ofs[s + 1] - c->cent_ofs[s]);
-                add += nc * nrec * (sizeof(GeoRec) + (c->accum_mode == 0 ? 512 + kCoefLine * sizeof(float) : 0)) + c->syn_stride * sizeof(float);
+                add += nc * nrec * (sizeof(GeoRec) + (c->accum_mode == 0 ? 512 + kCoefLine * sizeof(float) : 0)) + plan_bytes(c, s, (size_t)nrec) + c->syn_stride * sizeof(float);
             }
             add += (size_t)nk * nrec * NN * sizeof(double);
             if (ng > 0 && (bytes + add > c->chunk_bytes_limit || (ng + 1) * K > 65535)) break;
diff --git a/kiwi_amd/csrc/kiwi_timescan.hpp b/kiwi_amd/csrc/kiwi_timescan.hpp
--- a/kiwi_amd/csrc/kiwi_timescan.hpp
+++ b/kiwi_amd/csrc/kiwi_timescan.hpp
@@ -336,7 +336,7 @@
         int n = 0;
         while (s + n < isrc0 + nsrc) {
             const size_t nc = (size_t)(c->cent_ofs[s + n + 1] - c->cent_ofs[s + n]);
-            const size_t add = nc * nrec * (sizeof(GeoRec) + (c->accum_mode == 0 ? 512 + kCoefLine * sizeof(float) : 0)) + c->syn_stride * sizeof(float) +
+            const size_t add = nc * nrec * (sizeof(GeoRec) + (c->accum_mode == 0 ? 512 + kCoefLine * sizeof(float) : 0)) + plan_bytes(c, s + n, (size_t)nrec) + c->syn_stride * sizeof(float) +
                                ((size_t)nk * nmis + nmis + nk + 1) * sizeof(float);
             if (n > 0 && (bytes + add > c->chunk_bytes_limit || n >= 65535)) break;
             if (c->fft_needed && n >= c->fft_cap) break;
```

Result: faster. 36640, median of 6 (+4.9%).
